# mgalardini/pyseer

Hardware: AMD Instinct MI355X
Metric: k-mer tests/sec at N=5000 samples (LMM), whole job (higher is better)
Workload: dtype int8 limbs x4 (exact int32 MFMA accumulation, fp64 recombination and statistics)

## Files before the change

### pyseer_amd/csrc/api.hip

```cpp
#include "common.h"
#include "route.h"
#include "host_pool.h"
#include <atomic>
#include <deque>
#include <mutex>
#include <condition_variable>
#include <functional>
#include <string>
#include <vector>
#include <thread>
#include <future>
#include <chrono>
#include <cmath>
#include <cstring>
#include <cstdlib>
#include <algorithm>

#include "lmm_params.h"
#include "vcf_kernels.h"
#include "vcf_reader.h"
#include "enet_params.h"
extern "C" {
hipError_t shk_sim_accumulate(hipStream_t st, const uint64_t *T, int64_t Vpad, int64_t V, int N, int NB64, double min_af, double max_af,
                              int af_on, uint64_t *keep, uint64_t *S, int NS, unsigned long long *Kacc);
hipError_t shk_sim_finish(hipStream_t st, const unsigned long long *Kacc, int NS, int N, double *K);
hipError_t shk_repack_bits(hipStream_t, const uint8_t *, int64_t, int64_t, int64_t, int, int, uint64_t *, uint8_t *);
hipError_t shk_lmm_linear(hipStream_t, int, const uint64_t *, int64_t, int, int, const double *, const double *,
                          const double *, const double *, const uint64_t *, const uint64_t *, int, const double *, LmmLinOut);
hipError_t shk_lmm_build_tab(hipStream_t, const double *, const double *, const double *, const double *, int, int, int, int, double *);
hipError_t shk_lmm_quadform(hipStream_t, int, const int8_t *, const uint64_t *, int64_t, int, int, int, double *, const int *, int, int64_t *);
hipError_t shk_lmm_refine(hipStream_t, int64_t, int64_t, int, int, int, int, const int8_t *, const uint64_t *, uint64_t *, double *, LmmLinOut,
                          const double *, LmmFinParams, double *, uint32_t *, LmmRefine);
hipError_t shk_af_compact(hipStream_t, int, int64_t, LmmLinOut, LmmFinParams, int *, int *, const uint64_t *, int64_t, uint64_t *,
                          int64_t, int, int, const double *, double *);
hipError_t shk_lmm_finalize(hipStream_t, int64_t, int64_t, int, LmmLinOut, const double *, LmmFinParams, double *, uint32_t *, LmmRefine);
hipError_t shk_spectral_bound(hipStream_t, const float *, int, int, double *, double *, int, double *, int *);
hipError_t shk_power_norm(hipStream_t, const float *, int, int, double *, double *, double *, int);
hipError_t shk_lmm_build_G(hipStream_t, const double *, const double *, int, int, int, int, int, int, double *, double *,
                           unsigned long long *, int8_t *, float *, double *, double *, double *, int);
hipError_t shk_dd_find(hipStream_t, const uint64_t *, int64_t, int64_t, int, uint64_t *, uint64_t, unsigned long long *, int *, int *, int *, int *);
hipError_t shk_af_rows(hipStream_t, int, const uint8_t *, int64_t, int64_t, int, double, double, int *, int *, int *);
hipError_t shk_pf_rows(hipStream_t, const uint8_t *, int64_t, int64_t, int, const uint64_t *, const uint64_t *, double, double, int, int, int,
                       double, int, int *, int *, int *, int *, int *, int *, double *, uint32_t *);
hipError_t shk_dd_gather(hipStream_t, const uint8_t *, int64_t, int64_t, const int *, const int *, uint8_t *);
hipError_t shk_dd_scatter(hipStream_t, int64_t, int64_t, int, const int *, const int *, const double *, const uint32_t *, double *, uint32_t *);
hipError_t shk_job_select(hipStream_t, const uint32_t *, const double *, int64_t, int, int, int, int *, long long *, long long *, int32_t *, uint32_t *, double *, int64_t, int32_t *);
int64_t sh_format_records(const char *, const int64_t *, const int32_t *, int, const int32_t *, int64_t, const double *const *, int, const double *, int64_t, int,
                          const uint8_t *, const int32_t *, const char *const *, int, const uint32_t *, const char **);
int64_t format_records_samples(const char *, const int64_t *, const int32_t *, int, const int32_t *, int64_t, const double *const *, int, const double *, int64_t, int,
                               const uint8_t *, const int32_t *, const char *const *, int, const uint32_t *, const char **, const uint8_t *, int64_t, const char *,
                               const int64_t *, const int32_t *);
hipError_t shk_job_patterns(hipStream_t, const uint64_t *, int64_t, int64_t, int, const uint32_t *, int *, long long *, uint32_t *, char *, char *);
#define JOB_ROWS_PER_BLOCK_HOST 1024
hipError_t shk_enet_store(hipStream_t, const uint8_t *, const uint8_t *, const uint8_t *, int64_t, int, int, uint64_t *);
hipError_t shk_enet_gather(hipStream_t, const uint64_t *, const int64_t *, int64_t, int, uint64_t *);
hipError_t shk_enet_ingest_count(hipStream_t, const uint64_t *, int64_t, int, int, int, int, int32_t *, int32_t *, int32_t *, int32_t *, int32_t *);
hipError_t shk_enet_ingest_scatter(hipStream_t, const uint64_t *, int64_t, int, int, const int32_t *, const int32_t *, uint64_t *);
hipError_t shk_enet_moments(hipStream_t, const uint64_t *, int64_t, int, int, const double *, double, double *);
hipError_t shk_enet_grad(hipStream_t, const uint64_t *, int64_t, int, const double *, int64_t, int, double *, int64_t);
size_t shk_enet_cd_lds_bytes(int, int);
hipError_t shk_enet_cd(hipStream_t, const struct EnetCdArgs *, int);
hipError_t shk_enet_predict(hipStream_t, const uint64_t *, const uint64_t *, const double *, const uint8_t *, int64_t, int, int, double *);
}
#include "glm_api.inc"

static thread_local std::string g_err;
static int fail(int code, const std::string &msg) { g_err = msg; return code; }
#define HIPCHK(x) do { hipError_t e_ = (x); if (e_ != hipSuccess) return fail(SH_EHIP, std::string(#x) + ": " + hipGetErrorString(e_)); } while (0)

#include <execinfo.h>
#include <signal.h>
static void sh_abort_backtrace(int sig)
{
    void *frames[64];
    const int n = backtrace(frames, 64);
    const char msg[] = "[seerhip] fatal signal; native backtrace of the signalled thread:\n";
    (void)!write(2, msg, sizeof(msg) - 1);
    backtrace_symbols_fd(frames, n, 2);
    signal(sig, SIG_DFL);
    raise(sig);
}
namespace { struct ShBacktraceInit { ShBacktraceInit() { if (sh_debug("backtrace")) { signal(SIGABRT, sh_abort_backtrace); signal(SIGSEGV, sh_abort_backtrace); signal(SIGBUS, sh_abort_backtrace); } } } sh_backtrace_init; }

template <typename T> static hipError_t dmalloc(T **p, size_t n)
{
    const hipError_t e = hipMalloc(reinterpret_cast<void **>(p), n * sizeof(T));
    if (e == hipSuccess && n && sh_debug("poison")) {
        const hipError_t m = hipMemset(*p, 0xFF, n * sizeof(T));
        return m != hipSuccess ? m : hipStreamSynchronize(nullptr);
    }
    return e;
}

struct sh_lanes;
struct EnetState;
struct PredictState;
struct GlmSetupArgs { std::vector<double> y, W; int q = 0, continuous = 0, force_firth = 0; double null_llf = 0, null_firth = 0, pret = 1, lrtt = 1;
                      std::string route; };
struct sh_ctx {
    int device = 0, N = 0;
    hipStream_t stream = nullptr;
    int *h_rb = nullptr;
    sh_lanes *lanes = nullptr; int n_lanes = 3; bool is_lane = false; GlmSetupArgs glm_args;
    double min_af = 0.0, max_af = 1.0; int af_on = 0;
    int NT = 0, Np = 0, NB64 = 0, NB64p = 0;
    bool lmm_ready = false;
    int k = 0, D = 0, L = 5, DP = 0;
    LmmFinParams fin{};
    double *d_vv = nullptr, *d_mdiag = nullptr, *d_yc = nullptr, *d_Qb = nullptr, *d_tab = nullptr;
    uint64_t *d_y1 = nullptr, *d_y0 = nullptr;
    int8_t *d_G = nullptr;
    double quant_scale = 0.0;
    size_t g_bytes = 0, tab_doubles = 0;
    int64_t macs_issued = 0;
    int E = 0;
    bool complement = false;
    double err_norm_ulp = 0.0, err_norm_est_ulp = 0.0, lmm_tol = 1e-8, trace_M = 0.0; int err_norm_squarings = 0;
    uint8_t *d_flip = nullptr; uint64_t *d_T3 = nullptr; double *d_q3 = nullptr; int *d_rlist = nullptr, *d_rcount = nullptr;
    unsigned long long *d_bmax = nullptr; int64_t cap_ref = 0;
    int qf_split = 1;
    int qf_variant = 4;
    GlmState glm;
    int64_t capV = 0;
    uint64_t *d_T = nullptr;
    int *d_t11 = nullptr, *d_t01 = nullptr, *d_m = nullptr;
    double *d_xky = nullptr, *d_dg = nullptr, *d_rss = nullptr, *d_s1 = nullptr, *d_q1 = nullptr, *d_q = nullptr;
    uint64_t *d_T2 = nullptr; double *d_q2 = nullptr; int *d_keep = nullptr, *d_nkeep = nullptr; int64_t cap_keep = 0;
    int af_compact = 1; int64_t last_kept = -1;
    int *h_nkeep = nullptr; hipEvent_t keep_ev = nullptr; bool keep_pending = false; int64_t keep_V = 0; double filtered_hint = 0.0;
    int timing = 0;
    int lin_tab = 1;
    std::vector<std::pair<hipEvent_t, hipEvent_t>> tev;
    int dedup = 0; int64_t dd_cap = 0, dd_capV = 0, dd_last_unique = -1;
    uint64_t *dd_h = nullptr; unsigned long long *dd_keys = nullptr; int *dd_idx = nullptr, *dd_rep = nullptr, *dd_slot = nullptr, *dd_n = nullptr;
    uint8_t *dd_bits = nullptr; double *dd_out = nullptr; uint32_t *dd_flags = nullptr; int64_t dd_cap_bits = 0, dd_cap_out = 0, dd_cap_flags = 0;
    int *af_rep = nullptr, *af_slot = nullptr, *af_cnt = nullptr, *h_af_cnt = nullptr; int64_t af_capV = 0;
    int *af_m = nullptr;
    uint8_t *af_bits = nullptr; double *af_out = nullptr; uint32_t *af_flags = nullptr; int64_t af_cap_bits = 0, af_cap_out = 0, af_cap_flags = 0;
    hipEvent_t af_ev = nullptr; bool af_pending = false; int64_t af_pending_V = 0; double af_hint = 0.0; int64_t af_last_rows = -1; unsigned af_tick = 0;
    unsigned long long *sim_K = nullptr; uint64_t *sim_S = nullptr, *sim_keep = nullptr; double *sim_out = nullptr; int64_t sim_capV = 0; int NS = 0;
    hipStream_t copy_stream = nullptr; hipEvent_t ev_h2d[2] = {nullptr, nullptr}, ev_done[2] = {nullptr, nullptr};
    uint8_t *hb_bits[2] = {nullptr, nullptr}; double *hb_out[2] = {nullptr, nullptr}; uint32_t *hb_flags[2] = {nullptr, nullptr};
    int64_t hb_cap_bits = 0, hb_cap_out = 0, hb_cap_flags = 0;
    uint8_t *hp_bits[2] = {nullptr, nullptr}; int64_t hp_cap = 0;
    struct HostPending { bool valid = false; int b = 0, q = 0; int64_t s = 0, n = 0; double *outs[5] = {nullptr, nullptr, nullptr, nullptr, nullptr};
                         double *betas = nullptr; uint32_t *flags = nullptr; } pend;
    uint64_t hb_seq = 0;
    const uint8_t *next_bits = nullptr; int64_t next_row_bytes = 0, next_V = 0;
    const uint8_t *pre_bits = nullptr; int64_t pre_row_bytes = 0, pre_n = 0; int pre_set = -1;
    int64_t cap_bits = 0, cap_out = 0, cap_flags = 0;
    uint8_t *d_bits = nullptr; double *d_out = nullptr; uint32_t *d_flags = nullptr;
    EnetState *enet = nullptr;
    PredictState *predict = nullptr;
};

__global__ void k_readback4(const int *__restrict__ a, const int *__restrict__ b, const int *__restrict__ c2, const int *__restrict__ d, int *__restrict__ out)
{
    if (threadIdx.x == 0) { out[0] = *a; if (b) out[1] = *b; if (c2) out[2] = *c2; if (d) out[3] = *d; __threadfence_system(); }
}
static hipError_t readback_launch(hipStream_t st, const int *a, const int *b, const int *c2, const int *d, int *host_mapped)
{
    hipLaunchKernelGGL(k_readback4, dim3(1), dim3(64), 0, st, a, b, c2, d, host_mapped);
    return hipGetLastError();
}
static int ensure_rb(sh_ctx *c);
static int readback_sync(sh_ctx *c, hipStream_t st, const int *a, const int *b, const int *c2, const int *d, int *dst);

static void lanes_destroy(sh_ctx *c);
static void enet_free(sh_ctx *c);
static void predict_free(sh_ctx *c);
static int lanes_wait(sh_ctx *c);
static void lanes_set_timing(sh_ctx *c, int on);
static int lanes_add_timing(sh_ctx *c, double *total_ms, int64_t *launches);
static void free_ws(sh_ctx *c)
{
    hipFree(c->d_T); hipFree(c->d_t11); hipFree(c->d_t01); hipFree(c->d_m); hipFree(c->d_xky); hipFree(c->d_dg);
    hipFree(c->d_rss); hipFree(c->d_s1); hipFree(c->d_q1); hipFree(c->d_q);
    c->d_T = nullptr; c->d_t11 = c->d_t01 = c->d_m = nullptr;
    c->d_xky = c->d_dg = c->d_rss = c->d_s1 = c->d_q1 = c->d_q = nullptr; c->capV = 0;
    hipFree(c->d_T2); hipFree(c->d_q2); hipFree(c->d_keep); hipFree(c->d_nkeep);
    c->d_T2 = nullptr; c->d_q2 = nullptr; c->d_keep = c->d_nkeep = nullptr; c->cap_keep = 0;
    hipFree(c->d_flip); hipFree(c->d_T3); hipFree(c->d_q3); hipFree(c->d_rlist);
    c->d_flip = nullptr; c->d_T3 = nullptr; c->d_q3 = nullptr; c->d_rlist = nullptr; c->cap_ref = 0;
}

static int ensure_rb(sh_ctx *c)
{
    if (!c->h_rb) HIPCHK(hipHostMalloc((void **)&c->h_rb, 16 * sizeof(int), hipHostMallocMapped));
    return SH_OK;
}
static int readback_sync(sh_ctx *c, hipStream_t st, const int *a, const int *b, const int *c2, const int *d, int *dst)
{
    int rc = ensure_rb(c); if (rc) return rc;
    HIPCHK(readback_launch(st, a, b, c2, d, c->h_rb));
    HIPCHK(hipStreamSynchronize(st));
    dst[0] = c->h_rb[0]; if (b) dst[1] = c->h_rb[1]; if (c2) dst[2] = c->h_rb[2]; if (d) dst[3] = c->h_rb[3];
    return SH_OK;
}

static int ensure_ws(sh_ctx *c, int64_t Vpad)
{
    if (Vpad <= c->capV) return SH_OK;
    free_ws(c);
    HIPCHK(dmalloc(&c->d_T, (size_t)Vpad * c->NB64p));
    HIPCHK(dmalloc(&c->d_t11, Vpad)); HIPCHK(dmalloc(&c->d_t01, Vpad)); HIPCHK(dmalloc(&c->d_m, Vpad));
    HIPCHK(dmalloc(&c->d_xky, Vpad)); HIPCHK(dmalloc(&c->d_dg, Vpad)); HIPCHK(dmalloc(&c->d_rss, Vpad));
    HIPCHK(dmalloc(&c->d_s1, Vpad)); HIPCHK(dmalloc(&c->d_q1, Vpad)); HIPCHK(dmalloc(&c->d_q, Vpad * 8));
    c->capV = Vpad;
    return SH_OK;
}

static int ensure_staging(sh_ctx *c, int64_t bits_bytes, int64_t out_doubles, int64_t V)
{
    if (bits_bytes > c->cap_bits) { hipFree(c->d_bits); c->d_bits = nullptr; HIPCHK(hipMalloc((void **)&c->d_bits, bits_bytes)); c->cap_bits = bits_bytes; }
    if (out_doubles > c->cap_out) { hipFree(c->d_out); c->d_out = nullptr; HIPCHK(dmalloc(&c->d_out, out_doubles)); c->cap_out = out_doubles; }
    if (V > c->cap_flags) { hipFree(c->d_flags); c->d_flags = nullptr; HIPCHK(dmalloc(&c->d_flags, V)); c->cap_flags = V; }
    return SH_OK;
}

static void parallel_copy(uint8_t *dst, const uint8_t *src, size_t n)
{
    shost::CpuScope cs(shost::ST_STAGE_COPY);
    const size_t piece = (size_t)4 << 20, np = (n + piece - 1) / piece;
    if (np <= 1) { std::memcpy(dst, src, n); return; }
    const std::function<void(int64_t)> cp = [&](int64_t i) { const size_t lo = (size_t)i * piece, hi = std::min(n, lo + piece); std::memcpy(dst + lo, src + lo, hi - lo); };
    shost::pool().run((int64_t)np, 1, cp, shost::ST_STAGE_COPY, shost::per_stream_cpus(2));
}

__global__ void k_betas_rows(const double *__restrict__ src, double *__restrict__ dst, int64_t n, int q)
{
    const int64_t i = (int64_t)blockIdx.x * blockDim.x + threadIdx.x;
    if (i >= n * q) return;
    const int64_t v = i / q; const int j = (int)(i - v * q);
    dst[i] = src[(size_t)j * n + v];
}

static void forget_announced(sh_ctx *c) { c->next_bits = nullptr; c->pre_bits = nullptr; c->pre_set = -1; }

static int drain_pending(sh_ctx *c)
{
    if (!c->pend.valid) return SH_OK;
    HIPCHK(hipSetDevice(c->device));
    const sh_ctx::HostPending p = c->pend;
    c->pend.valid = false;
    const int b = p.b;
    const int64_t s = p.s, n = p.n;
    HIPCHK(hipStreamWaitEvent(c->copy_stream, c->ev_done[b], 0));
    for (int a = 0; a < 5; ++a)
        HIPCHK(hipMemcpyAsync(p.outs[a] + s, c->hb_out[b] + (size_t)a * n, sizeof(double) * n, hipMemcpyDeviceToHost, c->copy_stream));
    if (p.q > 0)
        HIPCHK(hipMemcpyAsync(p.betas + (size_t)s * p.q, c->hb_out[b] + (size_t)(5 + p.q) * n, sizeof(double) * p.q * n, hipMemcpyDeviceToHost, c->copy_stream));
    HIPCHK(hipMemcpyAsync(p.flags + s, c->hb_flags[b], sizeof(uint32_t) * n, hipMemcpyDeviceToHost, c->copy_stream));
    HIPCHK(hipStreamSynchronize(c->copy_stream));
    return SH_OK;
}

template <typename F>
static int host_batch(sh_ctx *c, const uint8_t *bits, int64_t row_bytes, int64_t V, int nrow, double *const *outs, double *betas,
                      int q, uint32_t *flags, bool async, F inner_dev)
{
    const double t_entry = std::chrono::duration<double, std::milli>(std::chrono::steady_clock::now().time_since_epoch()).count();
    HIPCHK(hipSetDevice(c->device));
    const int64_t CH = 1 << 18;
    const int64_t cap = std::min(CH, V);
    if (!c->copy_stream) {
        HIPCHK(hipStreamCreateWithFlags(&c->copy_stream, hipStreamNonBlocking));
        for (int b = 0; b < 2; ++b) { HIPCHK(hipEventCreateWithFlags(&c->ev_h2d[b], hipEventDisableTiming)); HIPCHK(hipEventCreateWithFlags(&c->ev_done[b], hipEventDisableTiming)); }
    }
    if (cap * row_bytes > c->hb_cap_bits || cap * (nrow + q) > c->hb_cap_out || cap > c->hb_cap_flags) {
        int rc = drain_pending(c); if (rc) return rc;
        const int64_t nb = std::max(cap * row_bytes, c->hb_cap_bits), no = std::max(cap * (nrow + q), c->hb_cap_out), nf = std::max(cap, c->hb_cap_flags);
        for (int b = 0; b < 2; ++b) {
            hipFree(c->hb_bits[b]); hipFree(c->hb_out[b]); hipFree(c->hb_flags[b]);
            c->hb_bits[b] = nullptr; c->hb_out[b] = nullptr; c->hb_flags[b] = nullptr;
            HIPCHK(hipMalloc((void **)&c->hb_bits[b], nb)); HIPCHK(dmalloc(&c->hb_out[b], no)); HIPCHK(dmalloc(&c->hb_flags[b], nf));
        }
        c->hb_cap_bits = nb; c->hb_cap_out = no; c->hb_cap_flags = nf;
        c->pre_bits = nullptr; c->pre_set = -1;
    }
    if (cap * row_bytes > c->hp_cap) {
        int rc = drain_pending(c); if (rc) return rc;
        for (int b = 0; b < 2; ++b) { if (c->hp_bits[b]) hipHostFree(c->hp_bits[b]); c->hp_bits[b] = nullptr; HIPCHK(hipHostMalloc((void **)&c->hp_bits[b], cap * row_bytes, hipHostMallocDefault)); }
        c->hp_cap = cap * row_bytes;
        c->pre_bits = nullptr; c->pre_set = -1;
    }
    std::vector<int64_t> cut{0};
    for (int64_t step = 1 << 17; cut.back() < V; step = CH) cut.push_back(std::min(V, cut.back() + step));
    const int64_t nchunk = (int64_t)cut.size() - 1;
    const bool dbg = sh_debug("host");
    auto now = [] { return std::chrono::duration<double, std::milli>(std::chrono::steady_clock::now().time_since_epoch()).count(); };
    const uint8_t *const nb_bits = c->next_bits; const int64_t nb_rb = c->next_row_bytes, nb_V = c->next_V;
    c->next_bits = nullptr;
    const double t00 = now();
    auto upload = [&](int64_t i, int b) -> int {
        const int64_t s = cut[i], n = cut[i + 1] - s;
        parallel_copy(c->hp_bits[b], bits + s * row_bytes, (size_t)(n * row_bytes));
        HIPCHK(hipMemcpyAsync(c->hb_bits[b], c->hp_bits[b], n * row_bytes, hipMemcpyHostToDevice, c->copy_stream));
        HIPCHK(hipEventRecord(c->ev_h2d[b], c->copy_stream));
        return SH_OK;
    };
    for (int64_t i = 0; i < nchunk; ++i) {
        const int b = (int)(c->hb_seq++ & 1);
        const int64_t s = cut[i], n = cut[i + 1] - s;
        const double t0 = now();
        if (i == 0) {
            if (c->pend.valid && c->pend.b == b) { int rc = drain_pending(c); if (rc) return rc; }
            bool have = c->pre_bits == bits && c->pre_row_bytes == row_bytes && c->pre_n == n && c->pre_set == b;
            if (have) {
                const size_t nbytes = (size_t)(n * row_bytes), probe = std::min<size_t>(nbytes, 4096);
                have = std::memcmp(c->hp_bits[b], bits, probe) == 0 && std::memcmp(c->hp_bits[b] + nbytes - probe, bits + nbytes - probe, probe) == 0;
            }
            c->pre_bits = nullptr; c->pre_set = -1;
            if (!have) { int rc = upload(0, b); if (rc) return rc; }
        }
        const double t1 = now();
        HIPCHK(hipStreamWaitEvent(c->stream, c->ev_h2d[b], 0));
        std::string side_err;
        std::future<int> side = std::async(std::launch::async, [&]() -> int {
            if (hipSetDevice(c->device) != hipSuccess) { side_err = "hipSetDevice failed on the copy thread"; return SH_EHIP; }
            int rc = drain_pending(c);
            if (!rc && i + 1 < nchunk) rc = upload(i + 1, b ^ 1);
            else if (!rc && nb_bits && nb_bits != bits) {
                const int64_t n0 = std::min<int64_t>((int64_t)1 << 17, nb_V);
                if (n0 * nb_rb <= c->hp_cap && n0 * nb_rb <= c->hb_cap_bits) {
                    parallel_copy(c->hp_bits[b ^ 1], nb_bits, (size_t)(n0 * nb_rb));
                    if (hipMemcpyAsync(c->hb_bits[b ^ 1], c->hp_bits[b ^ 1], n0 * nb_rb, hipMemcpyHostToDevice, c->copy_stream) != hipSuccess ||
                        hipEventRecord(c->ev_h2d[b ^ 1], c->copy_stream) != hipSuccess) { g_err = "prefetch upload failed"; rc = SH_EHIP; }
                    else { c->pre_bits = nb_bits; c->pre_row_bytes = nb_rb; c->pre_n = n0; c->pre_set = b ^ 1; }
                }
            }
            if (rc) side_err = g_err;
            return rc;
        });
        int rc = inner_dev(c->hb_bits[b], n, c->hb_out[b], c->hb_flags[b]);
        if (!rc && q > 0) {
            hipLaunchKernelGGL(k_betas_rows, dim3((unsigned)((n * q + 255) / 256)), dim3(256), 0, c->stream, c->hb_out[b] + (size_t)5 * n,
                               c->hb_out[b] + (size_t)(5 + q) * n, n, q);
            if (hipGetLastError() != hipSuccess) rc = fail(SH_EHIP, "k_betas_rows launch failed");
        }
        if (!rc && hipEventRecord(c->ev_done[b], c->stream) != hipSuccess) rc = fail(SH_EHIP, "hipEventRecord failed");
        const double t2 = now();
        const int rc_side = side.get();
        if (rc) { c->pend.valid = false; return rc; }
        if (rc_side) { c->pend.valid = false; return fail(rc_side, side_err); }
        c->pend.valid = true; c->pend.b = b; c->pend.q = q; c->pend.s = s; c->pend.n = n; c->pend.betas = betas; c->pend.flags = flags;
        for (int a = 0; a < 5; ++a) c->pend.outs[a] = outs[a];
        if (dbg) fprintf(stderr, "[host_batch] chunk %lld n=%lld: first upload %.2f ms, kernels queued (fixed effects: run) %.2f ms, wait for the copy thread %.2f ms, t=%.2f\n", (long long)i, (long long)n, t1 - t0, t2 - t1, now() - t2, now() - t00);
    }
    const int rc_end = async ? SH_OK : drain_pending(c);
    if (dbg) fprintf(stderr, "[host_batch] call of %lld variants: %.2f ms in all (%.2f ms before the first chunk)\n", (long long)V, now() - t_entry, t00 - t_entry);
    return rc_end;
}

static int lmm_batch_dev_inner(sh_ctx *c, const void *d_bits, int64_t row_bytes, int64_t V, void *d_out, void *d_flags);
static int glm_batch_dev_inner(sh_ctx *c, const void *d_bits, int64_t row_bytes, int64_t V, void *d_out, void *d_flags);

template <typename F>
static int dedup_wrap(sh_ctx *c, const void *d_bits, int64_t row_bytes, int64_t V, void *d_out, void *d_flags, int nrow, F inner)
{
    HIPCHK(hipSetDevice(c->device));
    hipStream_t st = c->stream;
    const int64_t Vpad = (V + 511) / 512 * 512;
    int rc = ensure_ws(c, Vpad); if (rc) return rc;
    if (V > c->dd_capV) {
        hipFree(c->dd_h); hipFree(c->dd_keys); hipFree(c->dd_idx); hipFree(c->dd_rep); hipFree(c->dd_slot); hipFree(c->dd_n);
        c->dd_h = nullptr; c->dd_keys = nullptr; c->dd_idx = c->dd_rep = c->dd_slot = c->dd_n = nullptr;
        uint64_t cap = 1024; while (cap < (uint64_t)V * 2) cap <<= 1;
        HIPCHK(dmalloc(&c->dd_h, V)); HIPCHK(dmalloc(&c->dd_keys, cap)); HIPCHK(dmalloc(&c->dd_idx, cap));
        HIPCHK(dmalloc(&c->dd_rep, V)); HIPCHK(dmalloc(&c->dd_slot, V)); HIPCHK(dmalloc(&c->dd_n, 1));
        c->dd_cap = (int64_t)cap; c->dd_capV = V;
    }
    if (V * row_bytes > c->dd_cap_bits) { hipFree(c->dd_bits); c->dd_bits = nullptr; HIPCHK(hipMalloc((void **)&c->dd_bits, V * row_bytes)); c->dd_cap_bits = V * row_bytes; }
    if (V * nrow > c->dd_cap_out) { hipFree(c->dd_out); c->dd_out = nullptr; HIPCHK(dmalloc(&c->dd_out, V * nrow)); c->dd_cap_out = V * nrow; }
    if (V > c->dd_cap_flags) { hipFree(c->dd_flags); c->dd_flags = nullptr; HIPCHK(dmalloc(&c->dd_flags, V)); c->dd_cap_flags = V; }
    HIPCHK(shk_repack_bits(st, (const uint8_t *)d_bits, row_bytes, V, Vpad, c->N, c->NB64p, c->d_T, nullptr));
    HIPCHK(shk_dd_find(st, c->d_T, Vpad, V, c->NB64, c->dd_h, (uint64_t)c->dd_cap, c->dd_keys, c->dd_idx, c->dd_rep, c->dd_slot, c->dd_n));
    int nu = 0;
    { const int rcb = readback_sync(c, st, c->dd_n, nullptr, nullptr, nullptr, &nu); if (rcb) return rcb; }
    c->dd_last_unique = nu;
    HIPCHK(shk_dd_gather(st, (const uint8_t *)d_bits, row_bytes, V, c->dd_rep, c->dd_slot, c->dd_bits));
    rc = inner(c->dd_bits, (int64_t)nu, c->dd_out, c->dd_flags); if (rc) return rc;
    HIPCHK(shk_dd_scatter(st, V, nu, nrow, c->dd_rep, c->dd_slot, c->dd_out, c->dd_flags, (double *)d_out, (uint32_t *)d_flags));
    return SH_OK;
}

struct PrefilterRows { const uint64_t *y1 = nullptr, *y0 = nullptr; int n1 = 0, n0 = 0; double pret = 1.0; };
template <typename F>
static int af_wrap(sh_ctx *c, const void *d_bits, int64_t row_bytes, int64_t V, void *d_out, void *d_flags, int nrow, F inner,
                   PrefilterRows pf = PrefilterRows())
{
    c->af_last_rows = -1;
    const bool use_pf = pf.y1 != nullptr && pf.pret < 1.0;
    if (!((c->af_on || use_pf) && c->af_compact) || (V < 1024 && c->af_compact != 2)) return inner(d_bits, V, d_out, d_flags);
    HIPCHK(hipSetDevice(c->device));
    hipStream_t st = c->stream;
    if (V > c->af_capV) {
        hipFree(c->af_rep); hipFree(c->af_slot); hipFree(c->af_m); c->af_rep = c->af_slot = c->af_m = nullptr;
        HIPCHK(dmalloc(&c->af_rep, V)); HIPCHK(dmalloc(&c->af_slot, V)); HIPCHK(dmalloc(&c->af_m, 3 * V)); c->af_capV = V;
    }
    if (!c->af_cnt) {
        HIPCHK(dmalloc(&c->af_cnt, 2)); HIPCHK(hipHostMalloc((void **)&c->h_af_cnt, 2 * sizeof(int)));
        HIPCHK(hipEventCreateWithFlags(&c->af_ev, hipEventDisableTiming));
    }
    if (c->af_pending && hipEventQuery(c->af_ev) == hipSuccess) {
        c->af_hint = 1.0 - (double)c->h_af_cnt[0] / (double)c->af_pending_V; c->af_pending = false;
    }
    bool compact = false; int nk = 0, R = 0;
    if (!c->af_pending && (c->af_hint >= 0.10 || c->af_compact == 2 || (c->af_tick++ & 3) == 0)) {
        HIPCHK(hipMemsetD32Async((hipDeviceptr_t)c->af_cnt, 0, 1, st));
        HIPCHK(hipMemsetD32Async((hipDeviceptr_t)(c->af_cnt + 1), 2147483647, 1, st));
        if (use_pf)
            HIPCHK(shk_pf_rows(st, (const uint8_t *)d_bits, row_bytes, V, c->N, pf.y1, pf.y0, c->min_af, c->max_af, c->af_on, pf.n1, pf.n0, pf.pret, nrow,
                               c->af_m, c->af_m + c->af_capV, c->af_m + 2 * c->af_capV, c->af_rep, c->af_slot, c->af_cnt, (double *)d_out,
                               (uint32_t *)d_flags));
        else
            HIPCHK(shk_af_rows(st, 0, (const uint8_t *)d_bits, row_bytes, V, c->N, c->min_af, c->max_af, c->af_rep, c->af_slot, c->af_cnt));
        HIPCHK(readback_launch(st, c->af_cnt, c->af_cnt + 1, nullptr, nullptr, c->h_af_cnt));
        if (c->af_hint >= 0.10 || c->af_compact == 2) {
            HIPCHK(hipStreamSynchronize(st));
            nk = c->h_af_cnt[0]; R = c->h_af_cnt[1];
            c->af_hint = 1.0 - (double)nk / (double)V;
            compact = (int64_t)nk * 100 <= V * 90 || (c->af_compact == 2 && (int64_t)nk * 100 <= V * 97);
        } else {
            HIPCHK(hipEventRecord(c->af_ev, st)); c->af_pending = true; c->af_pending_V = V;
        }
    }
    if (!compact) return inner(d_bits, V, d_out, d_flags);
    const int64_t nu = (int64_t)nk + (R != 2147483647 ? 1 : 0);
    if (nu == 0) { c->af_last_rows = 0; return SH_OK; }
    if (nu * row_bytes > c->af_cap_bits) { hipFree(c->af_bits); c->af_bits = nullptr; HIPCHK(hipMalloc((void **)&c->af_bits, nu * row_bytes)); c->af_cap_bits = nu * row_bytes; }
    if (nu * nrow > c->af_cap_out) { hipFree(c->af_out); c->af_out = nullptr; HIPCHK(dmalloc(&c->af_out, nu * nrow)); c->af_cap_out = nu * nrow; }
    if (nu > c->af_cap_flags) { hipFree(c->af_flags); c->af_flags = nullptr; HIPCHK(dmalloc(&c->af_flags, nu)); c->af_cap_flags = nu; }
    HIPCHK(shk_af_rows(st, 1, nullptr, 0, V, 0, 0, 0, c->af_rep, c->af_slot, c->af_cnt));
    HIPCHK(shk_dd_gather(st, (const uint8_t *)d_bits, row_bytes, V, c->af_rep, c->af_slot, c->af_bits));
    c->af_last_rows = nu;
    int rc = inner(c->af_bits, nu, c->af_out, c->af_flags); if (rc) return rc;
    HIPCHK(shk_dd_scatter(st, V, nu, nrow, c->af_rep, c->af_slot, c->af_out, c->af_flags, (double *)d_out, (uint32_t *)d_flags));
    return SH_OK;
}

extern "C" {

int sh_abi_version(void) { return SH_ABI_VERSION; }
const char *sh_last_error(void) { return g_err.c_str(); }

int sh_device_count(void)
{
    int n = 0;
    if (hipGetDeviceCount(&n) != hipSuccess) return 0;
    return n;
}

__global__ void k_noop() {}

static std::atomic<int> g_wait_mode{0};
static std::atomic<uint64_t> g_wait_applied{0};
static void apply_wait_mode(int device)
{
    if (g_wait_mode.load() != 1 || device < 0 || device >= 64) return;
    const uint64_t bit = 1ull << device;
    if (g_wait_applied.fetch_or(bit) & bit) return;
    if (hipSetDeviceFlags(hipDeviceScheduleBlockingSync) != hipSuccess) (void)hipGetLastError();
}
void sh_set_wait_mode(int sleeping) { g_wait_mode.store(sleeping ? 1 : 0); }

int sh_warmup(int device)
{
    int n = 0;
    if (hipGetDeviceCount(&n) != hipSuccess || device < 0 || device >= n) return fail(SH_ENODEV, "no such HIP device");
    HIPCHK(hipSetDevice(device));
    apply_wait_mode(device);
    hipLaunchKernelGGL(k_noop, dim3(1), dim3(64), 0, 0);
    HIPCHK(hipGetLastError());
    HIPCHK(hipDeviceSynchronize());
    return SH_OK;
}

sh_ctx *sh_create(int device, int n_samples)
{
    int n = 0;
    if (const std::string bad = sh_route_unknown(); !bad.empty()) { g_err = "SEERHIP_ROUTE: unknown item '" + bad + "' (keys: csrc/route.h)"; return nullptr; }
    if (hipGetDeviceCount(&n) != hipSuccess || n <= 0) { g_err = "no HIP device: libseerhip has no CPU fallback"; return nullptr; }
    if (device < 0 || device >= n) { g_err = "bad device index"; return nullptr; }
    if (n_samples < 2) { g_err = "n_samples must be >= 2"; return nullptr; }
    hipDeviceProp_t prop;
    if (hipGetDeviceProperties(&prop, device) != hipSuccess) { g_err = "hipGetDeviceProperties failed"; return nullptr; }
    if (std::string(prop.gcnArchName).find("gfx950") == std::string::npos) {
        g_err = std::string("device is ") + prop.gcnArchName + ", libseerhip is built for gfx950 only"; return nullptr;
    }
    if (hipSetDevice(device) != hipSuccess) { g_err = "hipSetDevice failed"; return nullptr; }
    apply_wait_mode(device);
    sh_ctx *c = new sh_ctx();
    c->device = device; c->N = n_samples;
    if (const char *qv = sh_route("qf")) c->qf_variant = std::atoi(qv);
    if (const char *lv = sh_route("lanes")) c->n_lanes = std::max(1, std::min(8, std::atoi(lv)));
    if (const char *ac = sh_route("afcompact")) c->af_compact = std::atoi(ac);
    c->NT = (n_samples + 255) / 256; c->Np = c->NT * 256;
    c->NB64 = (n_samples + 63) / 64; c->NB64p = c->NT * 4;
    return c;
}

void sh_destroy(sh_ctx *c)
{
    if (!c) return;
    hipSetDevice(c->device);
    lanes_destroy(c);
    enet_free(c);
    predict_free(c);
    free_ws(c);
    if (c->h_nkeep) hipHostFree(c->h_nkeep);
    if (c->h_rb) hipHostFree(c->h_rb);
    if (c->h_af_cnt) hipHostFree(c->h_af_cnt);
    if (c->af_ev) hipEventDestroy(c->af_ev);
    hipFree(c->af_rep); hipFree(c->af_slot); hipFree(c->af_m); hipFree(c->af_cnt); hipFree(c->af_bits); hipFree(c->af_out); hipFree(c->af_flags);
    if (c->keep_ev) hipEventDestroy(c->keep_ev);
    hipFree(c->d_vv); hipFree(c->d_mdiag); hipFree(c->d_yc); hipFree(c->d_Qb); hipFree(c->d_y1); hipFree(c->d_y0); hipFree(c->d_tab);
    hipFree(c->d_G); hipFree(c->d_bits); hipFree(c->d_out); hipFree(c->d_flags); hipFree(c->d_rcount); hipFree(c->d_bmax);
    for (int b = 0; b < 2; ++b) { hipFree(c->hb_bits[b]); hipFree(c->hb_out[b]); hipFree(c->hb_flags[b]); if (c->ev_h2d[b]) hipEventDestroy(c->ev_h2d[b]); if (c->ev_done[b]) hipEventDestroy(c->ev_done[b]); }
    if (c->copy_stream) hipStreamDestroy(c->copy_stream);
    for (int b = 0; b < 2; ++b) if (c->hp_bits[b]) hipHostFree(c->hp_bits[b]);
    for (auto &p : c->tev) { hipEventDestroy(p.first); hipEventDestroy(p.second); }
    hipFree(c->dd_h); hipFree(c->dd_keys); hipFree(c->dd_idx); hipFree(c->dd_rep); hipFree(c->dd_slot); hipFree(c->dd_n); hipFree(c->dd_bits); hipFree(c->dd_out); hipFree(c->dd_flags);
    hipFree(c->sim_K); hipFree(c->sim_S); hipFree(c->sim_keep); hipFree(c->sim_out);
    glm_free(&c->glm);
    delete c;
}

int sh_set_stream(sh_ctx *c, void *s) { if (!c) return fail(SH_EINVAL, "null ctx"); forget_announced(c); c->stream = (hipStream_t)s; return SH_OK; }

int sh_synchronize(sh_ctx *c)
{
    if (!c) return fail(SH_EINVAL, "null ctx");
    HIPCHK(hipSetDevice(c->device));
    HIPCHK(hipStreamSynchronize(c->stream));
    return SH_OK;
}

int sh_set_timing(sh_ctx *c, int on)
{
    if (!c) return fail(SH_EINVAL, "null ctx");
    for (auto &p : c->tev) { hipEventDestroy(p.first); hipEventDestroy(p.second); }
    c->tev.clear(); c->timing = on;
    if (c->lanes) { const int rc = lanes_wait(c); if (rc) return rc; lanes_set_timing(c, on); }
    return SH_OK;
}

int sh_get_timing(sh_ctx *c, double *total_ms, int64_t *launches)
{
    if (!c) return fail(SH_EINVAL, "null ctx");
    HIPCHK(hipSetDevice(c->device));
    double tot = 0;
    for (auto &p : c->tev) { HIPCHK(hipEventSynchronize(p.second)); float ms = 0; HIPCHK(hipEventElapsedTime(&ms, p.first, p.second)); tot += ms; }
    int64_t nl = (int64_t)c->tev.size();
    if (c->lanes) { const int rc = lanes_wait(c); if (rc) return rc; const int r2 = lanes_add_timing(c, &tot, &nl); if (r2) return r2; }
    if (total_ms) *total_ms = tot;
    if (launches) *launches = nl;
    return SH_OK;
}

int sh_set_dedup(sh_ctx *c, int on) { if (!c) return fail(SH_EINVAL, "null ctx"); c->dedup = on; return SH_OK; }

int sh_dedup_info(sh_ctx *c, int64_t *unique_last_batch)
{
    if (!c) return fail(SH_EINVAL, "null ctx");
    if (unique_last_batch) *unique_last_batch = c->dd_last_unique;
    return SH_OK;
}

int sh_set_af_filter(sh_ctx *c, double min_af, double max_af)
{
    if (!c) return fail(SH_EINVAL, "null ctx");
    c->min_af = min_af; c->max_af = max_af; c->af_on = !(min_af <= 0.0 && max_af >= 1.0);
    return SH_OK;
}

static double spectral_bound_value(double f2, const int *e, int nsq)
{
    if (!(f2 > 0.0)) return 0.0;
    double lg = std::log2(f2) / std::ldexp(1.0, nsq + 1);
    for (int k = 0; k < nsq; ++k) lg -= (double)e[k] / std::ldexp(1.0, k);
    return std::exp2(lg);
}

int sh_lmm_setup(sh_ctx *c, const double *U, const double *S, int k, const double *y, const double *C, int D,
                 double h2, int continuous, double pret, double lrtt, int n_limbs)
{
    if (!c || !U || !S || !y || !C) return fail(SH_EINVAL, "null argument");
    if (k < 1 || D < 1) return fail(SH_ESHAPE, "k and D must be >= 1");
    if (h2 < 0.0 || h2 >= 1.0 || std::isnan(h2)) return fail(SH_EH2, "h2 outside [0,1): reference returns no 'beta' (KeyError)");
    { const int rc0 = drain_pending(c); if (rc0) return rc0; }
    forget_announced(c);
    if (n_limbs == 0) {
        const char *fe = sh_route("lmm_limbs");
        if (fe && std::atoi(fe) > 0) n_limbs = std::atoi(fe);
        else {
            const int rc4 = sh_lmm_setup(c, U, S, k, y, C, D, h2, continuous, pret, lrtt, 4);
            if (rc4 != SH_OK) return rc4;
            const double typ = c->trace_M > 0 ? c->fin.err_norm * (0.5 * c->N) / (0.25 * c->trace_M) : 0.0;
            if (c->E > 0 && typ <= 0.25 * c->lmm_tol) return SH_OK;
            n_limbs = 5;
        }
    }
    if (n_limbs < 3 || n_limbs > 7) return fail(SH_EINVAL, "n_limbs must be 3..7");
    if (c->N > 262143) return fail(SH_EINVAL, "more than 262143 samples: the int32 partial sums of k_lmm_quadform_i8 could overflow");
    HIPCHK(hipSetDevice(c->device));
    const int N = c->N, Np = c->Np;
    const int kp = (k + 3) & ~3;
    c->lmm_ready = false; c->macs_issued = 0;

    std::vector<double> Qb((size_t)N * D, 0.0);
    int r = 0;
    for (int d = 0; d < D; ++d) {
        const int src = (d == 0) ? D - 1 : d - 1;
        std::vector<double> col(N);
        double n0 = 0;
        for (int i = 0; i < N; ++i) { col[i] = C[(size_t)i * D + src]; n0 += col[i] * col[i]; }
        for (int pass = 0; pass < 2; ++pass)
            for (int e = 0; e < r; ++e) {
                double dot = 0; for (int i = 0; i < N; ++i) dot += Qb[(size_t)i * D + e] * col[i];
                for (int i = 0; i < N; ++i) col[i] -= dot * Qb[(size_t)i * D + e];
            }
        double n1 = 0; for (int i = 0; i < N; ++i) n1 += col[i] * col[i];
        if (!(n1 > 1e-24 * n0) || n0 == 0) continue;
        const double inv = 1.0 / std::sqrt(n1);
        for (int i = 0; i < N; ++i) Qb[(size_t)i * D + r] = col[i] * inv;
        ++r;
    }
    if (r < 1) return fail(SH_EINVAL, "covariate matrix has rank 0");
    bool ones_in_span;
    {
        std::vector<double> one(N, 1.0);
        for (int e = 0; e < r; ++e) { double dot = 0; for (int i = 0; i < N; ++i) dot += Qb[(size_t)i * D + e] * one[i]; for (int i = 0; i < N; ++i) one[i] -= dot * Qb[(size_t)i * D + e]; }
        double res = 0; for (int i = 0; i < N; ++i) res += one[i] * one[i];
        ones_in_span = res <= 1e-20 * (double)N;
    }
    bool intercept_only = (r == 1);
    if (intercept_only) { const double q0 = Qb[0]; for (int i = 0; i < N; ++i) if (std::fabs(Qb[(size_t)i * D] - q0) > 1e-12 * std::fabs(q0)) intercept_only = false; }
    int DP = 0;
    if (!intercept_only) { DP = 4; while (DP < r) DP *= 2; if (DP > 32) return fail(SH_EINVAL, "more than 32 independent covariates are not supported"); }

    std::vector<double> yt(N);
    {
        std::vector<double> cy(r, 0.0);
        for (int e = 0; e < r; ++e) { double s = 0; for (int i = 0; i < N; ++i) s += Qb[(size_t)i * D + e] * y[i]; cy[e] = s; }
        double mean = 0;
        for (int i = 0; i < N; ++i) { double s = y[i]; for (int e = 0; e < r; ++e) s -= Qb[(size_t)i * D + e] * cy[e]; yt[i] = s; mean += s; }
        mean /= N; double q = 0; for (int i = 0; i < N; ++i) q += (yt[i] - mean) * (yt[i] - mean);
        if (std::sqrt(q / N) <= 1e-10) std::fill(yt.begin(), yt.end(), 0.0);
    }
    std::vector<double> Sd(k), uy(k, 0.0), sgn(kp, 0.0);
    for (int rr = 0; rr < k; ++rr) Sd[rr] = h2 * S[rr] + (1.0 - h2);
    std::vector<double> W((size_t)Np * kp, 0.0);
    {
        std::vector<double> QtU((size_t)r * k, 0.0);
        for (int i = 0; i < N; ++i) {
            const double *u = U + (size_t)i * k;
            for (int e = 0; e < r; ++e) { const double q = Qb[(size_t)i * D + e]; double *o = &QtU[(size_t)e * k]; for (int rr = 0; rr < k; ++rr) o[rr] += q * u[rr]; }
        }
        for (int i = 0; i < N; ++i) {
            const double *u = U + (size_t)i * k; double *w = &W[(size_t)i * kp];
            for (int rr = 0; rr < k; ++rr) w[rr] = u[rr];
            for (int e = 0; e < r; ++e) { const double q = Qb[(size_t)i * D + e]; const double *o = &QtU[(size_t)e * k]; for (int rr = 0; rr < k; ++rr) w[rr] -= q * o[rr]; }
            const double yi = yt[i];
            if (yi != 0.0) for (int rr = 0; rr < k; ++rr) uy[rr] += w[rr] * yi;
        }
    }
    double yKy = 0;
    std::vector<double> uys(k);
    for (int rr = 0; rr < k; ++rr) { yKy += uy[rr] * uy[rr] / Sd[rr]; uys[rr] = uy[rr] / Sd[rr]; sgn[rr] = Sd[rr] < 0 ? -1.0 : 1.0; }
    std::vector<double> vv(N);
    for (int i = 0; i < N; ++i) {
        double *w = &W[(size_t)i * kp]; double s = 0;
        for (int rr = 0; rr < k; ++rr) s += w[rr] * uys[rr];
        vv[i] = s;
        for (int rr = 0; rr < k; ++rr) w[rr] *= 1.0 / std::sqrt(std::fabs(Sd[rr]));
    }
    std::vector<uint64_t> y1(c->NB64p, 0), y0(c->NB64p, 0);
    int n1 = 0, n0 = 0; double ymean = 0;
    for (int i = 0; i < N; ++i) { if (y[i] == 1.0) { y1[i >> 6] |= 1ull << (i & 63); ++n1; } else if (y[i] == 0.0) { y0[i >> 6] |= 1ull << (i & 63); ++n0; } ymean += y[i]; }
    ymean /= N;
    std::vector<double> yc(N); double ycs = 0, ycq = 0;
    for (int i = 0; i < N; ++i) { yc[i] = y[i] - ymean; ycs += yc[i]; ycq += yc[i] * yc[i]; }
    std::vector<double> Qbp;
    if (DP) { Qbp.assign((size_t)N * DP, 0.0); for (int i = 0; i < N; ++i) for (int e = 0; e < r; ++e) Qbp[(size_t)i * DP + e] = Qb[(size_t)i * D + e]; }

    hipFree(c->d_vv); hipFree(c->d_mdiag); hipFree(c->d_yc); hipFree(c->d_Qb); hipFree(c->d_y1); hipFree(c->d_y0); hipFree(c->d_G); hipFree(c->d_tab);
    c->d_vv = c->d_mdiag = c->d_yc = c->d_Qb = c->d_tab = nullptr; c->d_y1 = c->d_y0 = nullptr; c->d_G = nullptr;
    const int NT = c->NT, L = n_limbs;
    const int NR = 2 * NT;
    int E = std::min(2, 7 - L);
    const int Lt = L + E;
    const size_t gbytes = (size_t)Lt * NR * (NR + 1) * 8192;
    double *d_W = nullptr, *d_sgn = nullptr, *d_M = nullptr; unsigned long long *d_amax = nullptr;
    float *d_Ef = nullptr; double *d_px = nullptr, *d_py = nullptr, *d_nrm = nullptr;
    const int NPOW = 48;
    HIPCHK(dmalloc(&c->d_vv, N)); HIPCHK(dmalloc(&c->d_mdiag, N)); HIPCHK(dmalloc(&c->d_yc, N));
    HIPCHK(dmalloc(&c->d_y1, c->NB64p)); HIPCHK(dmalloc(&c->d_y0, c->NB64p));
    if (DP) HIPCHK(dmalloc(&c->d_Qb, (size_t)N * DP));
    HIPCHK(hipMalloc((void **)&c->d_G, gbytes + (256u << 10)));
    HIPCHK(dmalloc(&d_W, (size_t)Np * kp)); HIPCHK(dmalloc(&d_sgn, kp)); HIPCHK(dmalloc(&d_M, (size_t)Np * Np)); HIPCHK(dmalloc(&d_amax, 1));
    hipStream_t st = c->stream;
    HIPCHK(hipMemcpyAsync(d_W, W.data(), sizeof(double) * (size_t)Np * kp, hipMemcpyHostToDevice, st));
    HIPCHK(hipMemcpyAsync(d_sgn, sgn.data(), sizeof(double) * kp, hipMemcpyHostToDevice, st));
    HIPCHK(hipMemcpyAsync(c->d_vv, vv.data(), sizeof(double) * N, hipMemcpyHostToDevice, st));
    HIPCHK(hipMemcpyAsync(c->d_yc, yc.data(), sizeof(double) * N, hipMemcpyHostToDevice, st));
    HIPCHK(hipMemcpyAsync(c->d_y1, y1.data(), sizeof(uint64_t) * c->NB64p, hipMemcpyHostToDevice, st));
    HIPCHK(hipMemcpyAsync(c->d_y0, y0.data(), sizeof(uint64_t) * c->NB64p, hipMemcpyHostToDevice, st));
    if (DP) HIPCHK(hipMemcpyAsync(c->d_Qb, Qbp.data(), sizeof(double) * (size_t)N * DP, hipMemcpyHostToDevice, st));
    HIPCHK(hipMemsetAsync(d_M, 0, sizeof(double) * (size_t)Np * Np, st));
    HIPCHK(dmalloc(&d_Ef, (size_t)Np * Np)); HIPCHK(dmalloc(&d_px, Np)); HIPCHK(dmalloc(&d_py, Np)); HIPCHK(dmalloc(&d_nrm, NPOW));
    HIPCHK(shk_lmm_build_G(st, d_W, d_sgn, N, Np, kp, NR, Lt, E, d_M, c->d_mdiag, d_amax, c->d_G, d_Ef, d_px, d_py, d_nrm, NPOW));
    const int nsq = Np <= 16384 ? 5 : Np <= 32768 ? 4 : 3;
    double *d_X = nullptr, *d_work = nullptr; int *d_exps = nullptr;
    HIPCHK(dmalloc(&d_X, (size_t)Np * Np)); HIPCHK(dmalloc(&d_work, 2)); HIPCHK(dmalloc(&d_exps, 8));
    HIPCHK(shk_spectral_bound(st, d_Ef, N, Np, d_X, d_M, nsq, d_work, d_exps));
    double cert_f2 = 0.0; int cert_e[8] = {0, 0, 0, 0, 0, 0, 0, 0};
    HIPCHK(hipMemcpyAsync(&cert_f2, d_work + 1, sizeof(double), hipMemcpyDeviceToHost, st));
    HIPCHK(hipMemcpyAsync(cert_e, d_exps, sizeof(cert_e), hipMemcpyDeviceToHost, st));
    c->tab_doubles = (size_t)c->NB64 * 256 * (2 + 2 + 8); c->g_bytes = gbytes;
    HIPCHK(dmalloc(&c->d_tab, c->tab_doubles));
    HIPCHK(shk_lmm_build_tab(st, c->d_vv, c->d_mdiag, c->d_yc, c->d_Qb, DP, continuous, N, c->NB64, c->d_tab));
    unsigned long long amax_bits = 0;
    HIPCHK(hipMemcpyAsync(&amax_bits, d_amax, sizeof(amax_bits), hipMemcpyDeviceToHost, st));
    std::vector<double> nrm(NPOW, 0.0), mdiag_h(N, 0.0);
    HIPCHK(hipMemcpyAsync(nrm.data(), d_nrm, sizeof(double) * NPOW, hipMemcpyDeviceToHost, st));
    HIPCHK(hipMemcpyAsync(mdiag_h.data(), c->d_mdiag, sizeof(double) * N, hipMemcpyDeviceToHost, st));
    HIPCHK(hipStreamSynchronize(st));
    hipFree(d_W); hipFree(d_sgn); hipFree(d_M); hipFree(d_amax); hipFree(d_Ef); hipFree(d_px); hipFree(d_py); hipFree(d_nrm);
    hipFree(d_X); hipFree(d_work); hipFree(d_exps);
    double amax; std::memcpy(&amax, &amax_bits, sizeof(double));
    const double p256 = std::pow(256.0, L);
    c->quant_scale = amax > 0 ? 0.49 * p256 / amax : 0.0;
    c->err_norm_est_ulp = nrm[NPOW - 1];
    c->err_norm_squarings = nsq;
    c->err_norm_ulp = spectral_bound_value(cert_f2, cert_e, nsq) * (1.0 + 1e-6);
    if (!(c->err_norm_ulp >= c->err_norm_est_ulp * (1.0 - 1e-9)) || !std::isfinite(c->err_norm_ulp))
        return fail(SH_EHIP, "spectral-norm certificate below the power-iteration estimate");
    double sumv = 0; for (int i = 0; i < N; ++i) sumv += vv[i];
    c->trace_M = 0; for (int i = 0; i < N; ++i) c->trace_M += mdiag_h[i];

    c->k = k; c->D = D; c->L = L; c->DP = DP; c->E = E;
    c->complement = ones_in_span && !(sh_route("complement") && std::atoi(sh_route("complement")) == 0);
    if (const char *tv = sh_route("lmm_tol")) c->lmm_tol = std::atof(tv);
    LmmFinParams &P = c->fin;
    P.N = N; P.D = D; P.continuous = continuous; P.n1 = n1; P.n0 = n0; P.yc_sum = ycs; P.yc_sq = ycq;
    P.yKy = yKy; P.inv_scale = amax > 0 ? 1.0 / c->quant_scale : 0.0; P.pret = pret; P.lrtt = lrtt;
    P.sumv = sumv; P.err_norm = c->err_norm_ulp * P.inv_scale; P.tol = E > 0 ? c->lmm_tol : 0.0;
    P.inv_scale_low = P.inv_scale / std::pow(256.0, E);
    c->lmm_ready = true;
    return SH_OK;
}

int sh_lmm_info(sh_ctx *c, int *n_limbs, int64_t *macs, double *qscale)
{
    if (!c || !c->lmm_ready) return fail(SH_EINVAL, "sh_lmm_setup has not run");
    if (n_limbs) *n_limbs = c->L;
    if (macs) *macs = c->macs_issued > 0 ? c->macs_issued : (int64_t)c->L * (2 * c->NT) * (2 * c->NT + 1) * 128 * 64;
    if (qscale) *qscale = c->quant_scale;
    return SH_OK;
}

int sh_lmm_share(sh_ctx *dst, sh_ctx *src)
{
    if (!dst || !src || !src->lmm_ready) return fail(SH_EINVAL, "sh_lmm_share: the source context has no LMM set-up");
    if (dst == src) return SH_OK;
    if (dst->N != src->N) return fail(SH_ESHAPE, "sh_lmm_share: contexts of different sample counts");
    HIPCHK(hipSetDevice(src->device));
    HIPCHK(hipStreamSynchronize(src->stream));
    HIPCHK(hipSetDevice(dst->device));
    sh_ctx *c = dst;
    const int N = c->N;
    hipFree(c->d_vv); hipFree(c->d_mdiag); hipFree(c->d_yc); hipFree(c->d_Qb); hipFree(c->d_y1); hipFree(c->d_y0); hipFree(c->d_G); hipFree(c->d_tab);
    c->d_vv = c->d_mdiag = c->d_yc = c->d_Qb = c->d_tab = nullptr; c->d_y1 = c->d_y0 = nullptr; c->d_G = nullptr; c->lmm_ready = false;
    HIPCHK(dmalloc(&c->d_vv, N)); HIPCHK(dmalloc(&c->d_mdiag, N)); HIPCHK(dmalloc(&c->d_yc, N));
    HIPCHK(dmalloc(&c->d_y1, c->NB64p)); HIPCHK(dmalloc(&c->d_y0, c->NB64p));
    if (src->DP) HIPCHK(dmalloc(&c->d_Qb, (size_t)N * src->DP));
    HIPCHK(hipMalloc((void **)&c->d_G, src->g_bytes + (256u << 10))); HIPCHK(dmalloc(&c->d_tab, src->tab_doubles));
    auto cp = [&](void *d, const void *s_, size_t n) { return hipMemcpyPeerAsync(d, dst->device, s_, src->device, n, dst->stream); };
    HIPCHK(cp(c->d_vv, src->d_vv, sizeof(double) * N)); HIPCHK(cp(c->d_mdiag, src->d_mdiag, sizeof(double) * N));
    HIPCHK(cp(c->d_yc, src->d_yc, sizeof(double) * N));
    HIPCHK(cp(c->d_y1, src->d_y1, sizeof(uint64_t) * c->NB64p)); HIPCHK(cp(c->d_y0, src->d_y0, sizeof(uint64_t) * c->NB64p));
    if (src->DP) HIPCHK(cp(c->d_Qb, src->d_Qb, sizeof(double) * (size_t)N * src->DP));
    HIPCHK(cp(c->d_G, src->d_G, src->g_bytes)); HIPCHK(cp(c->d_tab, src->d_tab, sizeof(double) * src->tab_doubles));
    HIPCHK(hipStreamSynchronize(dst->stream));
    c->k = src->k; c->D = src->D; c->L = src->L; c->DP = src->DP; c->E = src->E; c->complement = src->complement;
    c->quant_scale = src->quant_scale; c->err_norm_ulp = src->err_norm_ulp; c->err_norm_est_ulp = src->err_norm_est_ulp; c->err_norm_squarings = src->err_norm_squarings; c->trace_M = src->trace_M; c->lmm_tol = src->lmm_tol;
    c->g_bytes = src->g_bytes; c->tab_doubles = src->tab_doubles; c->fin = src->fin;
    c->lmm_ready = true;
    return SH_OK;
}

int sh_set_lmm_tol(sh_ctx *c, double tol)
{
    if (!c) return fail(SH_EINVAL, "null ctx");
    if (!(tol >= 0.0)) return fail(SH_EINVAL, "tol must be >= 0 (0 = never refine)");
    c->lmm_tol = tol;
    if (c->lmm_ready) c->fin.tol = c->E > 0 ? tol : 0.0;
    return SH_OK;
}

int sh_lmm_bound(sh_ctx *c, double *err_norm_ulp, double *ulp, double *tol, int *extra_limbs, double *bound_typical,
                 double *bound_max_last, int64_t *refined_last)
{
    if (!c || !c->lmm_ready) return fail(SH_EINVAL, "sh_lmm_setup has not run");
    HIPCHK(hipSetDevice(c->device));
    if (err_norm_ulp) *err_norm_ulp = c->err_norm_ulp;
    if (ulp) *ulp = c->fin.inv_scale;
    if (tol) *tol = c->fin.tol;
    if (extra_limbs) *extra_limbs = c->E;
    if (bound_typical) *bound_typical = c->trace_M > 0 ? c->fin.err_norm * (0.5 * c->N) / (0.25 * c->trace_M) : 0.0;
    unsigned long long bm = 0; int nr = 0;
    if (c->d_bmax) {
        HIPCHK(hipMemcpyAsync(&bm, c->d_bmax, sizeof(bm), hipMemcpyDeviceToHost, c->stream));
        HIPCHK(hipMemcpyAsync(&nr, c->d_rcount, sizeof(nr), hipMemcpyDeviceToHost, c->stream));
        HIPCHK(hipStreamSynchronize(c->stream));
    }
    double b; std::memcpy(&b, &bm, sizeof(double));
    if (bound_max_last) *bound_max_last = b;
    if (refined_last) *refined_last = nr;
    return SH_OK;
}

int sh_lmm_bound_estimate(sh_ctx *c, double *power_iteration_ulp, int *squarings)
{
    if (!c || !c->lmm_ready) return fail(SH_EINVAL, "sh_lmm_setup has not run");
    if (power_iteration_ulp) *power_iteration_ulp = c->err_norm_est_ulp;
    if (squarings) *squarings = c->err_norm_squarings;
    return SH_OK;
}

int sh_spectral_bound_f32(sh_ctx *c, const float *A, int n, int squarings, double *upper, double *power_iteration)
{
    if (!c || !A || n < 1 || squarings < 1 || squarings > 6) return fail(SH_EINVAL, "bad argument");
    HIPCHK(hipSetDevice(c->device));
    const int Np = (n + 127) / 128 * 128, NPOW = 48;
    float *d_A = nullptr; double *d_X = nullptr, *d_Y = nullptr, *d_work = nullptr, *d_px = nullptr, *d_py = nullptr, *d_nrm = nullptr; int *d_exps = nullptr;
    HIPCHK(dmalloc(&d_A, (size_t)Np * Np)); HIPCHK(dmalloc(&d_X, (size_t)Np * Np)); HIPCHK(dmalloc(&d_Y, (size_t)Np * Np));
    HIPCHK(dmalloc(&d_work, 2)); HIPCHK(dmalloc(&d_exps, 8)); HIPCHK(dmalloc(&d_px, Np)); HIPCHK(dmalloc(&d_py, Np)); HIPCHK(dmalloc(&d_nrm, NPOW));
    hipStream_t st = c->stream;
    HIPCHK(hipMemsetAsync(d_A, 0, sizeof(float) * (size_t)Np * Np, st));
    HIPCHK(hipMemcpy2DAsync(d_A, sizeof(float) * Np, A, sizeof(float) * n, sizeof(float) * n, n, hipMemcpyHostToDevice, st));
    HIPCHK(shk_spectral_bound(st, d_A, n, Np, d_X, d_Y, squarings, d_work, d_exps));
    HIPCHK(shk_power_norm(st, d_A, n, Np, d_px, d_py, d_nrm, NPOW));
    double f2 = 0.0, nrm[48]; int e[8] = {0, 0, 0, 0, 0, 0, 0, 0};
    HIPCHK(hipMemcpyAsync(&f2, d_work + 1, sizeof(double), hipMemcpyDeviceToHost, st));
    HIPCHK(hipMemcpyAsync(e, d_exps, sizeof(e), hipMemcpyDeviceToHost, st));
    HIPCHK(hipMemcpyAsync(nrm, d_nrm, sizeof(nrm), hipMemcpyDeviceToHost, st));
    HIPCHK(hipStreamSynchronize(st));
    hipFree(d_A); hipFree(d_X); hipFree(d_Y); hipFree(d_work); hipFree(d_exps); hipFree(d_px); hipFree(d_py); hipFree(d_nrm);
    if (upper) *upper = spectral_bound_value(f2, e, squarings) * (1.0 + 1e-6);
    if (power_iteration) *power_iteration = nrm[NPOW - 1];
    return SH_OK;
}

int sh_lmm_batch_dev(sh_ctx *c, const void *d_bits, int64_t row_bytes, int64_t V, void *d_out, void *d_flags)
{
    if (!c || !c->lmm_ready) return fail(SH_EINVAL, "sh_lmm_setup has not run");
    if (V <= 0) return SH_OK;
    if (row_bytes * 8 < c->N) return fail(SH_ESHAPE, "row_bytes*8 < n_samples: shape mismatch between snps and Y");
    if (c->dedup)
        return dedup_wrap(c, d_bits, row_bytes, V, d_out, d_flags, 5,
                          [&](const void *b, int64_t n, void *o, void *f) { return lmm_batch_dev_inner(c, b, row_bytes, n, o, f); });
    return lmm_batch_dev_inner(c, d_bits, row_bytes, V, d_out, d_flags);
}

static int lmm_batch_dev_inner(sh_ctx *c, const void *d_bits, int64_t row_bytes, int64_t V, void *d_out, void *d_flags)
{
    if (V <= 0) return SH_OK;
    if (row_bytes * 8 < c->N) return fail(SH_ESHAPE, "row_bytes*8 < n_samples: shape mismatch between snps and Y");
    HIPCHK(hipSetDevice(c->device));
    const int64_t Vpad = (V + 511) / 512 * 512;
    int rc = ensure_ws(c, Vpad); if (rc) return rc;
    hipStream_t st = c->stream;
    if (Vpad > c->cap_ref || (c->E > 0 && !c->d_T3)) {
        hipFree(c->d_flip); hipFree(c->d_T3); hipFree(c->d_q3); hipFree(c->d_rlist);
        c->d_flip = nullptr; c->d_T3 = nullptr; c->d_q3 = nullptr; c->d_rlist = nullptr;
        HIPCHK(dmalloc(&c->d_flip, Vpad)); HIPCHK(dmalloc(&c->d_rlist, Vpad));
        if (c->E > 0) { HIPCHK(dmalloc(&c->d_T3, (size_t)Vpad * c->NB64p)); HIPCHK(dmalloc(&c->d_q3, Vpad * 2)); }
        c->cap_ref = Vpad;
    }
    if (!c->d_rcount) { HIPCHK(dmalloc(&c->d_rcount, 1)); HIPCHK(dmalloc(&c->d_bmax, 1)); }
    LmmLinOut lo{c->d_t11, c->d_t01, c->d_m, c->d_xky, c->d_dg, c->d_rss, c->d_s1, c->d_q1, c->complement ? c->d_flip : nullptr};
    HIPCHK(shk_repack_bits(st, (const uint8_t *)d_bits, row_bytes, V, Vpad, c->N, c->NB64p, c->d_T, c->complement ? c->d_flip : nullptr));
    HIPCHK(shk_lmm_linear(st, c->DP, c->d_T, Vpad, c->N, c->NB64, c->d_vv, c->d_mdiag, c->d_yc, c->d_Qb, c->d_y1, c->d_y0,
                          c->fin.continuous, c->lin_tab ? c->d_tab : nullptr, lo));
    hipEvent_t e0 = nullptr, e1 = nullptr;
    if (c->timing) { HIPCHK(hipEventCreate(&e0)); HIPCHK(hipEventCreate(&e1)); HIPCHK(hipEventRecord(e0, st)); }
    const int lsplit = c->qf_split ? c->L : 1;
    const int8_t *Gmain = c->d_G + (size_t)c->E * (2 * c->NT) * (2 * c->NT + 1) * 8192;
    int64_t nk = V;
    bool compact = false;
    LmmFinParams KP = c->fin; KP.min_af = c->min_af; KP.max_af = c->max_af; KP.af_on = c->af_on;
    if ((c->af_on || KP.pret < 1.0) && c->af_compact) {
        if (Vpad > c->cap_keep) {
            hipFree(c->d_T2); hipFree(c->d_q2); hipFree(c->d_keep); hipFree(c->d_nkeep);
            c->d_T2 = nullptr; c->d_q2 = nullptr; c->d_keep = c->d_nkeep = nullptr;
            HIPCHK(dmalloc(&c->d_T2, (size_t)Vpad * c->NB64p)); HIPCHK(dmalloc(&c->d_q2, Vpad * 8)); HIPCHK(dmalloc(&c->d_keep, Vpad));
            HIPCHK(dmalloc(&c->d_nkeep, 1)); c->cap_keep = Vpad;
        }
        if (!c->h_nkeep) { HIPCHK(hipHostMalloc((void **)&c->h_nkeep, sizeof(int))); HIPCHK(hipEventCreateWithFlags(&c->keep_ev, hipEventDisableTiming)); }
        if (c->keep_pending && hipEventQuery(c->keep_ev) == hipSuccess) {
            c->filtered_hint = 1.0 - (double)*c->h_nkeep / (double)c->keep_V; c->keep_pending = false;
        }
        if (!c->keep_pending) {
            HIPCHK(hipMemsetAsync(c->d_nkeep, 0, sizeof(int), st));
            HIPCHK(shk_af_compact(st, 0, V, lo, KP, c->d_keep, c->d_nkeep, nullptr, 0, nullptr, 0, 0, 0, nullptr, nullptr));
            HIPCHK(readback_launch(st, c->d_nkeep, nullptr, nullptr, nullptr, c->h_nkeep));
            if (c->filtered_hint >= 0.03 || c->af_compact == 2) {
                HIPCHK(hipStreamSynchronize(st));
                nk = *c->h_nkeep; c->filtered_hint = 1.0 - (double)nk / (double)V;
                compact = nk * 100 <= V * 97;
            } else {
                HIPCHK(hipEventRecord(c->keep_ev, st)); c->keep_pending = true; c->keep_V = V;
            }
        }
    }
    c->last_kept = compact ? nk : -1;
    if (compact && nk > 0) {
        const int64_t Vpad2 = (nk + 511) / 512 * 512;
        HIPCHK(shk_af_compact(st, 1, V, lo, KP, c->d_keep, nullptr, c->d_T, Vpad, c->d_T2, Vpad2, c->NB64p, (int)nk, nullptr, nullptr));
        HIPCHK(shk_lmm_quadform(st, c->qf_variant, Gmain, c->d_T2, Vpad2, 2 * c->NT, c->L, lsplit, c->d_q2, nullptr, c->N - (2 * c->NT - 1) * 128, &c->macs_issued));
        HIPCHK(shk_af_compact(st, 2, V, lo, KP, c->d_keep, nullptr, nullptr, Vpad, nullptr, Vpad2, lsplit, (int)nk, c->d_q2, c->d_q));
    } else if (!compact) {
        HIPCHK(shk_lmm_quadform(st, c->qf_variant, Gmain, c->d_T, Vpad, 2 * c->NT, c->L, lsplit, c->d_q, nullptr, c->N - (2 * c->NT - 1) * 128, &c->macs_issued));
    }
    if (c->timing) { HIPCHK(hipEventRecord(e1, st)); c->tev.emplace_back(e0, e1); }
    LmmFinParams P = c->fin; P.min_af = c->min_af; P.max_af = c->max_af; P.af_on = c->af_on;
    const bool refine = c->E > 0 && P.tol > 0.0;
    LmmRefine R{refine ? c->d_rlist : nullptr, c->d_rcount, c->d_bmax};
    HIPCHK(hipMemsetAsync(c->d_rcount, 0, sizeof(int), st));
    HIPCHK(hipMemsetAsync(c->d_bmax, 0, sizeof(unsigned long long), st));
    HIPCHK(shk_lmm_finalize(st, V, Vpad, lsplit, lo, c->d_q, P, (double *)d_out, (uint32_t *)d_flags, R));
    if (refine)
        HIPCHK(shk_lmm_refine(st, V, Vpad, lsplit, c->E, 2 * c->NT, c->NB64p, c->d_G, c->d_T, c->d_T3, c->d_q3, lo, c->d_q, P, (double *)d_out,
                              (uint32_t *)d_flags, R));
    return SH_OK;
}

static int lmm_batch_host(sh_ctx *c, const uint8_t *bits, int64_t row_bytes, int64_t V, double *prep, double *pvalue,
                          double *beta, double *bse, double *frac_h2, uint32_t *flags, bool async)
{
    if (!c || !c->lmm_ready) return fail(SH_EINVAL, "sh_lmm_setup has not run");
    if (!bits || !prep || !pvalue || !beta || !bse || !frac_h2 || !flags) return fail(SH_EINVAL, "null argument");
    if (V <= 0) { HIPCHK(hipSetDevice(c->device)); return drain_pending(c); }
    double *outs[5] = {prep, pvalue, beta, bse, frac_h2};
    return host_batch(c, bits, row_bytes, V, 5, outs, nullptr, 0, flags, async,
                      [&](const void *b, int64_t n, void *o, void *f) { return sh_lmm_batch_dev(c, b, row_bytes, n, o, f); });
}

int sh_lmm_batch(sh_ctx *c, const uint8_t *bits, int64_t row_bytes, int64_t V, double *prep, double *pvalue,
                 double *beta, double *bse, double *frac_h2, uint32_t *flags)
{
    return lmm_batch_host(c, bits, row_bytes, V, prep, pvalue, beta, bse, frac_h2, flags, false);
}

int sh_lmm_batch_async(sh_ctx *c, const uint8_t *bits, int64_t row_bytes, int64_t V, double *prep, double *pvalue,
                       double *beta, double *bse, double *frac_h2, uint32_t *flags)
{
    return lmm_batch_host(c, bits, row_bytes, V, prep, pvalue, beta, bse, frac_h2, flags, true);
}

int sh_prefetch_rows(sh_ctx *c, const uint8_t *bits, int64_t row_bytes, int64_t V)
{
    if (!c) return fail(SH_EINVAL, "null ctx");
    if (!bits || V <= 0 || row_bytes <= 0) { c->next_bits = nullptr; return SH_OK; }
    c->next_bits = bits; c->next_row_bytes = row_bytes; c->next_V = V;
    return SH_OK;
}

int sh_wait(sh_ctx *c)
{
    if (!c) return fail(SH_EINVAL, "null ctx");
    HIPCHK(hipSetDevice(c->device));
    const int rc = drain_pending(c);
    const int rl = lanes_wait(c);
    return rc ? rc : rl;
}

int sh_sim_begin(sh_ctx *c)
{
    if (!c) return fail(SH_EINVAL, "null ctx");
    HIPCHK(hipSetDevice(c->device));
    c->NS = (c->N + 127) / 128 * 128;
    if (!c->sim_K) HIPCHK(dmalloc(&c->sim_K, (size_t)c->NS * c->NS));
    HIPCHK(hipMemsetAsync(c->sim_K, 0, sizeof(unsigned long long) * (size_t)c->NS * c->NS, c->stream));
    return SH_OK;
}

int sh_sim_accumulate_dev(sh_ctx *c, const void *d_bits, int64_t row_bytes, int64_t V)
{
    if (!c || !c->sim_K) return fail(SH_EINVAL, "sh_sim_begin has not run");
    if (!d_bits) return fail(SH_EINVAL, "null argument");
    if (row_bytes * 8 < c->N) return fail(SH_ESHAPE, "row_bytes too small for n_samples");
    if (V <= 0) return SH_OK;
    if (V > ((int64_t)1 << 31)) return fail(SH_EINVAL, "at most 2^31 variants per call (32-bit partial counts)");
    HIPCHK(hipSetDevice(c->device));
    const int64_t Vpad = (V + 511) / 512 * 512;
    int rc = ensure_ws(c, Vpad); if (rc) return rc;
    if (Vpad > c->sim_capV) {
        hipFree(c->sim_S); hipFree(c->sim_keep); c->sim_S = nullptr; c->sim_keep = nullptr;
        const int64_t VWp = (Vpad / 64 + 15) / 16 * 16;
        HIPCHK(dmalloc(&c->sim_S, (size_t)VWp * c->NS)); HIPCHK(dmalloc(&c->sim_keep, (size_t)VWp));
        c->sim_capV = Vpad;
    }
    HIPCHK(shk_repack_bits(c->stream, (const uint8_t *)d_bits, row_bytes, V, Vpad, c->N, c->NB64p, c->d_T, nullptr));
    HIPCHK(shk_sim_accumulate(c->stream, c->d_T, Vpad, V, c->N, c->NB64, c->min_af, c->max_af, c->af_on, c->sim_keep, c->sim_S, c->NS, c->sim_K));
    return SH_OK;
}

int sh_sim_accumulate(sh_ctx *c, const uint8_t *bits, int64_t row_bytes, int64_t V)
{
    if (!c || !c->sim_K) return fail(SH_EINVAL, "sh_sim_begin has not run");
    if (!bits) return fail(SH_EINVAL, "null argument");
    HIPCHK(hipSetDevice(c->device));
    const int64_t CH = 1 << 20;
    for (int64_t s = 0; s < V; s += CH) {
        const int64_t n = std::min(CH, V - s);
        int rc = ensure_staging(c, n * row_bytes, 0, 0); if (rc) return rc;
        HIPCHK(hipMemcpyAsync(c->d_bits, bits + s * row_bytes, n * row_bytes, hipMemcpyHostToDevice, c->stream));
        rc = sh_sim_accumulate_dev(c, c->d_bits, row_bytes, n); if (rc) return rc;
        HIPCHK(hipStreamSynchronize(c->stream));
    }
    return SH_OK;
}

int sh_sim_finish(sh_ctx *c, double *K)
{
    if (!c || !c->sim_K) return fail(SH_EINVAL, "sh_sim_begin has not run");
    if (!K) return fail(SH_EINVAL, "null argument");
    HIPCHK(hipSetDevice(c->device));
    const size_t n = (size_t)c->N * c->N;
    if (!c->sim_out) HIPCHK(dmalloc(&c->sim_out, n));
    HIPCHK(shk_sim_finish(c->stream, c->sim_K, c->NS, c->N, c->sim_out));
    HIPCHK(hipMemcpyAsync(K, c->sim_out, sizeof(double) * n, hipMemcpyDeviceToHost, c->stream));
    HIPCHK(hipStreamSynchronize(c->stream));
    return SH_OK;
}

#include "glm_api_impl.inc"
#include "lanes_api.inc"
#include "job_api.inc"
#include "job_run.inc"
#include "vcf_api.inc"
#include "enet_api.inc"

}
```

### pyseer_amd/csrc/lmm_kernels.hip

```cpp
#include <utility>
#include "common.h"
#include "lmm_params.h"

typedef int v4i __attribute__((ext_vector_type(4)));
typedef int v16i __attribute__((ext_vector_type(16)));
typedef double v4d __attribute__((ext_vector_type(4)));


__global__ __launch_bounds__(256) void k_row_flip(const uint8_t *__restrict__ bits, int64_t row_bytes, int64_t V, int N, uint8_t *__restrict__ flip)
{
    const int64_t v = (int64_t)blockIdx.x * 4 + (threadIdx.x >> 6);
    const int lane = threadIdx.x & 63;
    if (v >= V) return;
    const uint8_t *p = bits + v * row_bytes;
    const int nb = N >> 3;
    int m = 0;
    for (int b = lane; b < nb; b += 64) m += __popc((unsigned)p[b]);
    if (lane == 0 && (N & 7)) m += __popc((unsigned)p[nb] & ((1u << (N & 7)) - 1u));
    for (int o = 32; o > 0; o >>= 1) m += __shfl_xor(m, o, 64);
    if (lane == 0) flip[v] = (2 * m > N) ? 1 : 0;
}

__global__ __launch_bounds__(256) void k_repack_bits_gather(const uint8_t *__restrict__ bits, int64_t row_bytes, int64_t V,
                                                            int64_t Vpad, int N, uint64_t *__restrict__ T, const uint8_t *__restrict__ flip)
{
    const int64_t v = (int64_t)blockIdx.x * 256 + threadIdx.x;
    const int sb = blockIdx.y;
    uint64_t w = 0;
    if (v < V) {
        const int64_t off = (int64_t)sb * 8;
        const uint8_t *p = bits + v * row_bytes + off;
        int64_t nbytes = row_bytes - off; if (nbytes > 8) nbytes = 8;
        if (nbytes == 8 && ((reinterpret_cast<uintptr_t>(p) & 7) == 0)) w = *reinterpret_cast<const uint64_t *>(p);
        else for (int b = 0; b < nbytes; b++) w |= (uint64_t)p[b] << (8 * b);
        if (flip && flip[v]) w = ~w;
        const int valid = N - sb * 64;
        if (valid <= 0) w = 0; else if (valid < 64) w &= ((1ull << valid) - 1ull);
    }
    T[(int64_t)sb * Vpad + v] = w;
}

__global__ __launch_bounds__(256) void k_repack_bits(const uint8_t *__restrict__ bits, int64_t row_bytes, int64_t V,
                                                     int64_t Vpad, int N, int NB64p, uint64_t *__restrict__ T, uint8_t *__restrict__ flip)
{
    extern __shared__ __attribute__((aligned(16))) uint8_t rp_rows[];
    __shared__ int rp_cnt[4][64];
    const int64_t v0 = (int64_t)blockIdx.x * 64;
    const int tid = threadIdx.x, lane = tid & 63, wave = tid >> 6;
    const int64_t nrows = min((int64_t)64, V - v0);
    const int64_t span = nrows > 0 ? nrows * row_bytes : 0;
    const uint8_t *src = bits + v0 * row_bytes;
    if ((reinterpret_cast<uintptr_t>(src) & 15) == 0) {
        const int64_t n16 = span >> 4;
        for (int64_t i = tid; i < n16; i += 256) reinterpret_cast<uint4 *>(rp_rows)[i] = reinterpret_cast<const uint4 *>(src)[i];
        for (int64_t i = (n16 << 4) + tid; i < span; i += 256) rp_rows[i] = src[i];
    } else {
        for (int64_t i = tid; i < span; i += 256) rp_rows[i] = src[i];
    }
    __syncthreads();
    auto word = [&](int sb) -> uint64_t {
        uint64_t w = 0;
        const int64_t off = (int64_t)sb * 8;
        if (lane < nrows && off < row_bytes) {
            const uint8_t *p = rp_rows + lane * row_bytes + off;
            int64_t nbytes = row_bytes - off; if (nbytes > 8) nbytes = 8;
            if (nbytes == 8 && ((row_bytes & 7) == 0)) w = *reinterpret_cast<const uint64_t *>(p);
            else for (int b = 0; b < nbytes; b++) w |= (uint64_t)p[b] << (8 * b);
            const int valid = N - sb * 64;
            if (valid <= 0) w = 0; else if (valid < 64) w &= ((1ull << valid) - 1ull);
        }
        return w;
    };
    bool fl = false;
    if (flip) {
        int m = 0;
        for (int sb = wave; sb < NB64p; sb += 4) m += __popcll(word(sb));
        rp_cnt[wave][lane] = m;
        __syncthreads();
        m = rp_cnt[0][lane] + rp_cnt[1][lane] + rp_cnt[2][lane] + rp_cnt[3][lane];
        fl = lane < nrows && 2 * m > N;
        if (wave == 0 && lane < nrows) flip[v0 + lane] = fl ? 1 : 0;
    }
    for (int sb = wave; sb < NB64p; sb += 4) {
        uint64_t w = word(sb);
        if (fl) {
            const int valid = N - sb * 64;
            w = ~w;
            if (valid <= 0) w = 0; else if (valid < 64) w &= ((1ull << valid) - 1ull);
        }
        T[(int64_t)sb * Vpad + v0 + lane] = w;
    }
}


template <int DP>
__global__ __launch_bounds__(256) void k_lmm_linear(const uint64_t *__restrict__ T, int64_t Vpad, int N, int NB64,
                                                    const double *__restrict__ vv, const double *__restrict__ mdiag,
                                                    const double *__restrict__ yc, const double *__restrict__ Qb,
                                                    const uint64_t *__restrict__ y1, const uint64_t *__restrict__ y0,
                                                    int continuous, LmmLinOut o)
{
    const int64_t v = (int64_t)blockIdx.x * 256 + threadIdx.x;
    double xky = 0, dg = 0, s1 = 0, q1 = 0;
    double c[DP > 0 ? DP : 1];
#pragma unroll
    for (int d = 0; d < DP; d++) c[d] = 0;
    int t11 = 0, t01 = 0, m = 0;
    for (int sb = 0; sb < NB64; sb++) {
        const uint64_t w = T[(int64_t)sb * Vpad + v];
        m += __popcll(w); t11 += __popcll(w & y1[sb]); t01 += __popcll(w & y0[sb]);
        const int nb = min(64, N - sb * 64);
        for (int b = 0; b < nb; b++) {
            const int i = sb * 64 + b;
            const double xd = (double)(unsigned)((w >> b) & 1ull);
            xky = fma(xd, vv[i], xky);
            dg = fma(xd, mdiag[i], dg);
            if (continuous) { const double t = yc[i]; s1 = fma(xd, t, s1); q1 = fma(xd, t * t, q1); }
#pragma unroll
            for (int d = 0; d < DP; d++) c[d] = fma(xd, Qb[(int64_t)i * DP + d], c[d]);
        }
    }
    double rss;
    if (DP > 0) {
        rss = 0;
        for (int sb = 0; sb < NB64; sb++) {
            const uint64_t w = T[(int64_t)sb * Vpad + v];
            const int nb = min(64, N - sb * 64);
            for (int b = 0; b < nb; b++) {
                const int i = sb * 64 + b;
                double r = (double)(unsigned)((w >> b) & 1ull);
#pragma unroll
                for (int d = 0; d < DP; d++) r = fma(-Qb[(int64_t)i * DP + d], c[d], r);
                rss = fma(r, r, rss);
            }
        }
    } else {
        rss = (double)m * (double)(N - m) / (double)N;
    }
    o.t11[v] = t11; o.t01[v] = t01; o.m[v] = m;
    o.xky[v] = xky; o.dg[v] = dg; o.rss[v] = rss; o.s1[v] = s1; o.q1[v] = q1;
}

__global__ __launch_bounds__(256) void k_lmm_build_tab(const double *__restrict__ vv, const double *__restrict__ mdiag, int N, int NB64,
                                                       double2 *__restrict__ tab)
{
    const int e = blockIdx.x * 256 + threadIdx.x;
    if (e >= NB64 * 256) return;
    const int value = e & 15, base = (e >> 4) * 4;
    double a = 0.0, b = 0.0;
    for (int k = 0; k < 4; ++k)
        if (((value >> k) & 1) && base + k < N) { a += vv[base + k]; b += mdiag[base + k]; }
    tab[e] = make_double2(a, b);
}

__global__ __launch_bounds__(256) void k_lmm_linear_tab(const uint64_t *__restrict__ T, int64_t Vpad, int N, int NB64,
                                                        const double2 *__restrict__ tab, const uint64_t *__restrict__ y1,
                                                        const uint64_t *__restrict__ y0, LmmLinOut o)
{
    __shared__ double2 lt[2][256];
    const int tid = threadIdx.x;
    const int64_t v = (int64_t)blockIdx.x * 256 + tid;
    double xky = 0, dg = 0;
    int t11 = 0, t01 = 0, m = 0;
    lt[0][tid] = tab[tid];
    for (int sb = 0; sb < NB64; sb++) {
        const double2 nxt = (sb + 1 < NB64) ? tab[(sb + 1) * 256 + tid] : make_double2(0.0, 0.0);
        const uint64_t w = T[(int64_t)sb * Vpad + v];
        __syncthreads();
        m += __popcll(w); t11 += __popcll(w & y1[sb]); t01 += __popcll(w & y0[sb]);
        const double2 *cur = lt[sb & 1];
        const uint32_t lo = (uint32_t)w, hi = (uint32_t)(w >> 32);
#pragma unroll
        for (int nib = 0; nib < 8; ++nib) {
            const double2 e0 = cur[nib * 16 + ((lo >> (4 * nib)) & 15u)];
            const double2 e1 = cur[(8 + nib) * 16 + ((hi >> (4 * nib)) & 15u)];
            xky += e0.x; dg += e0.y; xky += e1.x; dg += e1.y;
        }
        lt[(sb + 1) & 1][tid] = nxt;
    }
    o.t11[v] = t11; o.t01[v] = t01; o.m[v] = m;
    o.xky[v] = xky; o.dg[v] = dg; o.rss[v] = (double)m * (double)(N - m) / (double)N; o.s1[v] = 0.0; o.q1[v] = 0.0;
}

template <int NE>
__global__ __launch_bounds__(256) void k_lmm_build_tabn(const double *__restrict__ vv, const double *__restrict__ mdiag,
                                                        const double *__restrict__ yc, const double *__restrict__ Qb, int DP, int cont,
                                                        int N, int NB64, double *__restrict__ tab)
{
    const int e = blockIdx.x * 256 + threadIdx.x;
    if (e >= NB64 * 256) return;
    const int value = e & 15, base = (e >> 4) * 4;
    for (int c = 0; c < NE; ++c) {
        double a = 0.0;
        for (int k = 0; k < 4; ++k) {
            const int i = base + k;
            if (!((value >> k) & 1) || i >= N) continue;
            double x;
            if (c == 0) x = vv[i]; else if (c == 1) x = mdiag[i];
            else if (cont && c == 2) x = yc[i]; else if (cont && c == 3) x = yc[i] * yc[i];
            else x = Qb[(int64_t)i * DP + (c - 2 - 2 * cont)];
            a += x;
        }
        tab[(int64_t)e * NE + c] = a;
    }
}

template <int NE>
__global__ __launch_bounds__(256) void k_lmm_linear_tabn(const uint64_t *__restrict__ T, int64_t Vpad, int N, int NB64,
                                                         const double *__restrict__ tab, const uint64_t *__restrict__ y1,
                                                         const uint64_t *__restrict__ y0, const double *__restrict__ Qb, int DP,
                                                         int cont, LmmLinOut o)
{
    __shared__ __attribute__((aligned(16))) double lt[2][256 * NE];
    const int tid = threadIdx.x;
    const int64_t v = (int64_t)blockIdx.x * 256 + tid;
    double acc[NE];
#pragma unroll
    for (int c = 0; c < NE; ++c) acc[c] = 0.0;
    int t11 = 0, t01 = 0, m = 0;
#pragma unroll
    for (int c = 0; c < NE; ++c) lt[0][tid * NE + c] = tab[(int64_t)tid * NE + c];
    for (int sb = 0; sb < NB64; sb++) {
        double nxt[NE];
        const bool more = sb + 1 < NB64;
#pragma unroll
        for (int c = 0; c < NE; ++c) nxt[c] = more ? tab[((int64_t)(sb + 1) * 256 + tid) * NE + c] : 0.0;
        const uint64_t w = T[(int64_t)sb * Vpad + v];
        __syncthreads();
        m += __popcll(w); t11 += __popcll(w & y1[sb]); t01 += __popcll(w & y0[sb]);
        const double *cur = lt[sb & 1];
#pragma unroll 4
        for (int nib = 0; nib < 16; ++nib) {
            const double *e = cur + (nib * 16 + (int)((w >> (4 * nib)) & 15ull)) * NE;
#pragma unroll
            for (int c = 0; c < NE; ++c) acc[c] += e[c];
        }
#pragma unroll
        for (int c = 0; c < NE; ++c) lt[(sb + 1) & 1][tid * NE + c] = nxt[c];
    }
    const int c0 = 2 + 2 * cont;
    double rss;
    if (DP > 0) {
        double sc = 0.0;
        for (int d = 0; d < NE - c0; ++d) sc = fma(acc[c0 + d], acc[c0 + d], sc);
        rss = (double)m - sc;
        const bool susp = rss <= 1e-8 * fmax((double)m, 1.0);
        if (__any(susp)) {
            double ex = 0.0;
            for (int sb = 0; sb < NB64; sb++) {
                const uint64_t w = T[(int64_t)sb * Vpad + v];
                const int nb = min(64, N - sb * 64);
                for (int b = 0; b < nb; b++) {
                    const int i = sb * 64 + b;
                    double r = (double)(unsigned)((w >> b) & 1ull);
                    for (int d = 0; d < NE - c0; ++d) r = fma(-Qb[(int64_t)i * DP + d], acc[c0 + d], r);
                    ex = fma(r, r, ex);
                }
            }
            if (susp) rss = ex;
        }
    } else {
        rss = (double)m * (double)(N - m) / (double)N;
    }
    o.t11[v] = t11; o.t01[v] = t01; o.m[v] = m;
    o.xky[v] = acc[0]; o.dg[v] = acc[1]; o.rss[v] = rss;
    o.s1[v] = cont ? acc[2] : 0.0; o.q1[v] = cont ? acc[3] : 0.0;
}

template __global__ void k_lmm_linear<0>(const uint64_t *, int64_t, int, int, const double *, const double *, const double *, const double *, const uint64_t *, const uint64_t *, int, LmmLinOut);
template __global__ void k_lmm_linear<4>(const uint64_t *, int64_t, int, int, const double *, const double *, const double *, const double *, const uint64_t *, const uint64_t *, int, LmmLinOut);
template __global__ void k_lmm_linear<8>(const uint64_t *, int64_t, int, int, const double *, const double *, const double *, const double *, const uint64_t *, const uint64_t *, int, LmmLinOut);
template __global__ void k_lmm_linear<16>(const uint64_t *, int64_t, int, int, const double *, const double *, const double *, const double *, const uint64_t *, const uint64_t *, int, LmmLinOut);
template __global__ void k_lmm_linear<32>(const uint64_t *, int64_t, int, int, const double *, const double *, const double *, const double *, const uint64_t *, const uint64_t *, int, LmmLinOut);

#define QF_TILE_BYTES 8192
#define QF_BN 512

__device__ __forceinline__ int qf_off(int row, int chunk) { return row * 64 + ((chunk ^ ((row >> 2) & 3)) << 4); }

__device__ __forceinline__ uint4 qf_expand16(uint32_t bits16)
{
    uint4 r;
    r.x = (((bits16) & 0xFu) * 0x00204081u) & 0x01010101u;
    r.y = (((bits16 >> 4) & 0xFu) * 0x00204081u) & 0x01010101u;
    r.z = (((bits16 >> 8) & 0xFu) * 0x00204081u) & 0x01010101u;
    r.w = (((bits16 >> 12) & 0xFu) * 0x00204081u) & 0x01010101u;
    return r;
}

#ifndef QF_G_AUX
#define QF_G_AUX 0
#endif
#ifndef QF_JT
#define QF_JT 2
#endif
#define QF_WAVES (16 / QF_JT)
#define QF_DMA_PER_WAVE (24 / QF_WAVES)
#ifndef QF_DIAG_TRIM
#define QF_DIAG_TRIM 0
#endif
#ifndef QF_NST
#define QF_NST 5
#endif
#define QF_AHEAD (QF_NST - 1)
#define QF_STAGE_BYTES (2 * QF_TILE_BYTES + 2 * QF_BN * 8)

__device__ __forceinline__ void qf_dma_stage(const int8_t *gsrc, const uint64_t *tsrc, int64_t Vpad, char *slot, int wave, int lane)
{
#pragma unroll
    for (int j = 0; j < 16 / QF_WAVES; ++j) {
        const int piece = wave * (16 / QF_WAVES) + j;
        __builtin_amdgcn_global_load_lds((const __attribute__((address_space(1))) void *)(gsrc + piece * 1024 + lane * 16),
                                         (__attribute__((address_space(3))) void *)(slot + piece * 1024), 16, 0, QF_G_AUX);
    }
#pragma unroll
    for (int j = 0; j < 8 / QF_WAVES; ++j) {
        const int pb = wave * (8 / QF_WAVES) + j;
        const uint64_t *src = tsrc + (int64_t)(pb >> 2) * Vpad + (pb & 3) * 128 + lane * 2;
        __builtin_amdgcn_global_load_lds((const __attribute__((address_space(1))) void *)src,
                                         (__attribute__((address_space(3))) void *)(slot + 2 * QF_TILE_BYTES + pb * 1024), 16, 0, 0);
    }
}

template <int N> __device__ __forceinline__ void qf_wait_vm() { asm volatile("s_waitcnt vmcnt(%0)" ::"n"(N) : "memory"); }

template <int ABL>
__global__ __launch_bounds__(64 * QF_WAVES, QF_JT == 2 ? 2 : 1) void k_lmm_quadform_i8(const int8_t *__restrict__ G, const uint64_t *__restrict__ T,
                                                            int64_t Vpad, int NR, int L, int lsplit, double *__restrict__ qout,
                                                            const int *__restrict__ nlimit)
{
    extern __shared__ __attribute__((aligned(16))) char smem[];
    const int tid = threadIdx.x, lane = tid & 63, wave = tid >> 6;
    const int l31 = lane & 31, lh = lane >> 5;
    const int ntiles = (int)(Vpad / QF_BN);
    int tile, lgrp;
    if ((ntiles & 7) == 0) { const int xcd = blockIdx.x & 7, w = blockIdx.x >> 3; tile = (w / lsplit) * 8 + xcd; lgrp = w % lsplit; }
    else { tile = blockIdx.x / lsplit; lgrp = blockIdx.x % lsplit; }
    const int nl = (L - lgrp + lsplit - 1) / lsplit;
    const int64_t v0 = (int64_t)tile * QF_BN;
    if (nlimit && v0 >= (int64_t)*nlimit) return;
    const bool big = NR * 128 > 65535;
    const int64_t TL = (int64_t)NR * (NR + 1);
    const int total = nl * (NR * (NR + 1) / 2);
    int aoff[4][2];
#pragma unroll
    for (int it = 0; it < 4; ++it) { aoff[it][0] = qf_off(it * 32 + l31, lh); aoff[it][1] = qf_off(it * 32 + l31, 2 + lh); }
    const int boff = 2 * QF_TILE_BYTES + (wave * (32 * QF_JT) + l31) * 8;

    double tot[QF_JT];
#pragma unroll
    for (int jt = 0; jt < QF_JT; ++jt) tot[jt] = 0.0;
    v16i acc[4][QF_JT];
    int pI = 0, pl = 0, pst = 0, pslot = 0;
    int cI = 0, cl = 0, cst = 0;
    double scale0 = 1.0, step = 1.0;
    for (int i = 0; i < lgrp; ++i) scale0 *= 256.0;
    for (int i = 0; i < lsplit; ++i) step *= 256.0;
    double scale_l = scale0;

    auto fetch = [&]() {
        const int8_t *g = G + ((int64_t)(lgrp + pl * lsplit) * TL + (int64_t)pI * (pI + 1) + 2 * pst) * QF_TILE_BYTES;
        const uint64_t *t = T + (int64_t)(2 * pst) * Vpad + v0;
        if (ABL & 8) { g = G; t = T + v0; }
        if (!(ABL & 1)) qf_dma_stage(g, t, Vpad, smem + pslot * QF_STAGE_BYTES, wave, lane);
        if (++pslot == QF_NST) pslot = 0;
        if (++pst == pI + 1) { pst = 0; if (++pl == nl) { pl = 0; ++pI; } }
    };

#pragma unroll 1
    for (int s = 0; s < QF_AHEAD && s < total; ++s) fetch();

    auto sync_refill = [&](int s) {
        const int newer = max(0, min(total - 2 - s, QF_AHEAD - 2));
        if (!(ABL & 1)) {
            if (newer >= 3) qf_wait_vm<3 * QF_DMA_PER_WAVE>(); else if (newer == 2) qf_wait_vm<2 * QF_DMA_PER_WAVE>();
            else if (newer == 1) qf_wait_vm<QF_DMA_PER_WAVE>(); else qf_wait_vm<0>();
        }
        if (!(ABL & 16)) __builtin_amdgcn_s_barrier();
        __builtin_amdgcn_sched_barrier(0);
        if (s + QF_AHEAD < total) fetch();
    };
    auto read_bits = [&](const char *base, uint64_t (&w)[2][QF_JT]) {
#pragma unroll
        for (int jt = 0; jt < QF_JT; ++jt) {
            w[0][jt] = *reinterpret_cast<const uint64_t *>(base + boff + 256 * jt);
            w[1][jt] = *reinterpret_cast<const uint64_t *>(base + boff + QF_BN * 8 + 256 * jt);
        }
    };
    auto expand = [&](const uint64_t (&w)[2][QF_JT], int sub, v4i (&b)[QF_JT]) {
        const int tl = sub >> 1, kh = sub & 1;
#pragma unroll
        for (int jt = 0; jt < QF_JT; ++jt) {
            const uint32_t h = lh ? (uint32_t)(w[tl][jt] >> 32) : (uint32_t)w[tl][jt];
            uint4 e;
            if (ABL & 4) e = make_uint4(h, kh, jt, 1);
            else e = make_uint4((h >> (4 * kh)) & 0x01010101u, (h >> (4 * kh + 1)) & 0x01010101u,
                                (h >> (4 * kh + 2)) & 0x01010101u, (h >> (4 * kh + 3)) & 0x01010101u);
            b[jt] = (v4i){(int)e.x, (int)e.y, (int)e.z, (int)e.w};
        }
    };

    uint64_t wb[2][QF_JT], wbn[2][QF_JT];
    v4i a_cur[4], a_nxt[4], b_cur[QF_JT], b_nxt[QF_JT];
    sync_refill(0);
    read_bits(smem, wb);
#pragma unroll
    for (int it = 0; it < 4; ++it) a_cur[it] = (ABL & 2) ? (v4i){it, lane, 0, 1} : *reinterpret_cast<const v4i *>(smem + aoff[it][0]);
    expand(wb, 0, b_cur);

    int slot = 0;
#pragma unroll 1
    for (int s = 0; s < total; ++s) {
        if (s > 0) sync_refill(s);
        if ((ABL & 256) ? s == 0 : cst == 0) {
#pragma unroll
            for (int it = 0; it < 4; ++it)
#pragma unroll
                for (int jt = 0; jt < QF_JT; ++jt)
#pragma unroll
                    for (int r = 0; r < 16; ++r) acc[it][jt][r] = 0;
        }
        const char *a_base = smem + slot * QF_STAGE_BYTES;
        const char *n_base = smem + (slot + 1 == QF_NST ? 0 : slot + 1) * QF_STAGE_BYTES;
        const bool diag = (cst == cI);
        __builtin_amdgcn_sched_barrier(0);
#pragma unroll
        for (int sub = 0; sub < 4; ++sub) {
            if (sub < 3) {
                const int nt = (sub + 1) >> 1, nk = (sub + 1) & 1;
#pragma unroll
                for (int it = 0; it < 4; ++it)
                    a_nxt[it] = (ABL & 2) ? (v4i){it, lane, nt, nk}
                                          : *reinterpret_cast<const v4i *>(a_base + nt * QF_TILE_BYTES + aoff[it][nk]);
                if (sub == 2) read_bits(n_base, wbn);
            } else {
#pragma unroll
                for (int it = 0; it < 4; ++it)
                    a_nxt[it] = (ABL & 2) ? (v4i){it, lane, s, 1} : *reinterpret_cast<const v4i *>(n_base + aoff[it][0]);
            }
#pragma unroll
            for (int it = 0; it < 4; ++it) {
                if (QF_DIAG_TRIM && sub >= 2 && it < 2 && diag) continue;
#pragma unroll
                for (int jt = 0; jt < QF_JT; ++jt)
                    acc[it][jt] = __builtin_amdgcn_mfma_i32_32x32x32_i8(a_cur[it], b_cur[jt], acc[it][jt], 0, 0, 0);
            }
            if (sub < 3) expand(wb, sub + 1, b_nxt); else expand(wbn, 0, b_nxt);
            __builtin_amdgcn_sched_barrier(0);
#pragma unroll
            for (int it = 0; it < 4; ++it) a_cur[it] = a_nxt[it];
#pragma unroll
            for (int jt = 0; jt < QF_JT; ++jt) b_cur[jt] = b_nxt[jt];
        }
        if (++slot == QF_NST) slot = 0;
        if (++cst == cI + 1) {
#pragma unroll
            for (int jt = 0; jt < QF_JT; ++jt) {
                int part[4];
                if (ABL & 128) { tot[jt] += (double)(acc[0][jt][0] + acc[1][jt][1] + acc[2][jt][2] + acc[3][jt][3]); continue; }
#pragma unroll
                for (int it = 0; it < 4; ++it) {
                    const uint32_t w = (uint32_t)(wb[it >> 1][jt] >> ((it & 1) * 32 + 4 * lh));
                    part[it] = 0;
                    if (!big) {
#pragma unroll
                        for (int r = 0; r < 16; ++r) {
                            const int row = (r & 3) + 8 * (r >> 2);
                            const int bit = (int)__builtin_amdgcn_ubfe(w, row, 1);
                            asm("v_mad_i32_i24 %0, %1, %2, %0" : "+v"(part[it]) : "v"(acc[it][jt][r]), "v"(bit));
                        }
                    } else {
#pragma unroll
                        for (int r = 0; r < 16; ++r) {
                            const int row = (r & 3) + 8 * (r >> 2);
                            part[it] += ((w >> row) & 1u) ? acc[it][jt][r] : 0;
                        }
                    }
                }
                tot[jt] = fma((double)((part[0] + part[1]) + (part[2] + part[3])), scale_l, tot[jt]);
            }
            cst = 0; scale_l *= step;
            if (++cl == nl) { cl = 0; scale_l = scale0; ++cI; }
        }
#pragma unroll
        for (int jt = 0; jt < QF_JT; ++jt) { wb[0][jt] = wbn[0][jt]; wb[1][jt] = wbn[1][jt]; }
    }
#pragma unroll
    for (int jt = 0; jt < QF_JT; ++jt) tot[jt] += __shfl_xor(tot[jt], 32, 64);
    if (lh == 0) {
        double *qo = qout + (int64_t)lgrp * Vpad + v0 + wave * (32 * QF_JT) + l31;
#pragma unroll
        for (int jt = 0; jt < QF_JT; ++jt) qo[32 * jt] = tot[jt];
    }
}

#include "lmm_quadform_wide.inc"


struct LinV { int m, t11, t01, mst; double xky, dg, rss, s1, q1; };
__device__ __forceinline__ LinV lin_load(const LmmLinOut &li, const LmmFinParams &P, int64_t v)
{
    LinV r;
    r.mst = li.m[v]; r.m = r.mst; r.t11 = li.t11[v]; r.t01 = li.t01[v];
    r.xky = li.xky[v]; r.dg = li.dg[v]; r.rss = li.rss[v]; r.s1 = li.s1[v]; r.q1 = li.q1[v];
    if (li.flip && li.flip[v]) {
        r.m = P.N - r.mst; r.t11 = P.n1 - r.t11; r.t01 = P.n0 - r.t01;
        r.xky = P.sumv - r.xky; r.s1 = P.yc_sum - r.s1; r.q1 = P.yc_sq - r.q1;
    }
    return r;
}

__device__ __forceinline__ double lmm_fin_one(int64_t v, int64_t V, int64_t Vpad, int nq, const LmmLinOut &li, const double *__restrict__ q,
                                              const LmmFinParams &P, double q_extra, bool refined, double *__restrict__ out,
                                              uint32_t *__restrict__ flags, bool *want_refine)
{
    const double nanv = NAN;
    double prep = nanv, pval = nanv, beta = nanv, bse = nanv, frac = nanv, bound = 0.0;
    uint32_t fl = 0;
    const LinV L = lin_load(li, P, v);
    const int m = L.m;
    bool go = true;
    *want_refine = false;
    if (P.af_on) {
        const double af = (double)m / (double)P.N;
        if (!(P.min_af <= af && af <= P.max_af)) { fl = SH_NOTE_AF_FILTER | SH_FLAG_PREFILTER; go = false; }
    }
    if (go) {
        bool bad = false;
        if (P.continuous) {
            const double n1 = (double)m, n0 = (double)(P.N - m);
            prep = sh_prefilter_welch(n1, L.s1, L.q1, n0, P.yc_sum - L.s1, P.yc_sq - L.q1);
        } else {
            prep = sh_prefilter_binary(L.t11, P.n1 - L.t11, L.t01, P.n0 - L.t01, &bad);
        }
        if (bad) fl |= SH_NOTE_BAD_CHISQ;
        if (prep >= P.pret || !isfinite(prep)) fl |= SH_NOTE_PRE_FILTER | SH_FLAG_PREFILTER;
    }
    if (go && !((fl & SH_FLAG_PREFILTER) && P.pret < 1.0)) {
        const bool zeroed = sqrt(L.rss / (double)P.N) <= 1e-10;
        double qs = 0.0;
        for (int a = 0; a < nq; ++a) qs += q[(int64_t)a * Vpad + v];
        const double xKx = zeroed ? 0.0 : (L.dg + (qs * P.inv_scale + q_extra));
        const double xKy = zeroed ? 0.0 : L.xky;
        if (!zeroed && xKx > 0.0) {
            bound = (refined ? P.err_norm * (P.inv_scale_low / P.inv_scale) : P.err_norm) * (double)L.mst / xKx;
            if (!refined && P.tol > 0.0 && bound > P.tol) *want_refine = true;
        }
        double b = xKy / xKx;
        if (isnan(b) && xKy == 0.0) b = 0.0;
        const double veb = xKy * b, r2 = P.yKy - veb;
        const double var = r2 / ((double)(P.N - P.D) - 1.0) / xKx;
        const double chi2 = b * b / var;
        pval = sh_f_sf_1(chi2, (double)(P.N - (P.D + 1)));
        beta = b; bse = sqrt(var); frac = sqrt(veb / P.yKy);
        if (!(fl & SH_FLAG_PREFILTER)) {
            if (pval >= P.lrtt || !isfinite(pval)) fl |= SH_NOTE_LRT_FILTER | SH_FLAG_FILTER;
        }
    }
    out[v] = prep; out[V + v] = pval; out[2 * V + v] = beta; out[3 * V + v] = bse; out[4 * V + v] = frac;
    flags[v] = fl;
    return bound;
}

__device__ __forceinline__ void lmm_bound_max(double bound, unsigned long long *bound_max)
{
    for (int o = 32; o > 0; o >>= 1) bound = fmax(bound, __shfl_xor(bound, o, 64));
    if ((threadIdx.x & 63) == 0 && bound > 0.0 && bound_max) atomicMax(bound_max, (unsigned long long)__double_as_longlong(bound));
}

__global__ __launch_bounds__(256) void k_lmm_finalize(int64_t V, int64_t Vpad, int nq, LmmLinOut li, const double *__restrict__ q,
                                                      LmmFinParams P, double *__restrict__ out, uint32_t *__restrict__ flags, LmmRefine R)
{
    const int64_t v = (int64_t)blockIdx.x * 256 + threadIdx.x;
    const int lane = threadIdx.x & 63;
    bool ref = false;
    double bound = 0.0;
    if (v < V) bound = lmm_fin_one(v, V, Vpad, nq, li, q, P, 0.0, false, out, flags, &ref);
    const unsigned long long rm = __ballot(ref);
    if (rm && R.list) {
        int base = 0;
        if (lane == 0) base = atomicAdd(R.count, __popcll(rm));
        base = __shfl(base, 0);
        if (ref) R.list[base + __popcll(rm & ((1ull << lane) - 1ull))] = (int)v;
    }
    lmm_bound_max((ref && R.list) ? 0.0 : bound, R.bound_max);
}

__global__ __launch_bounds__(256) void k_lmm_refine_fix(int64_t V, int64_t Vpad, int nq, int nq3, LmmLinOut li, const double *__restrict__ q,
                                                        const double *__restrict__ q3, LmmFinParams P, double *__restrict__ out,
                                                        uint32_t *__restrict__ flags, LmmRefine R)
{
    const int n = *R.count;
    for (int64_t j0 = (int64_t)blockIdx.x * 256; j0 < n; j0 += (int64_t)gridDim.x * 256) {
        const int64_t j = j0 + threadIdx.x;
        double bound = 0.0;
        if (j < n) {
            const int64_t v = R.list[j];
            double qe = 0.0;
            for (int a = 0; a < nq3; ++a) qe += q3[(int64_t)a * Vpad + j];
            bool dummy;
            bound = lmm_fin_one(v, V, Vpad, nq, li, q, P, qe * P.inv_scale_low, true, out, flags, &dummy);
        }
        lmm_bound_max(bound, R.bound_max);
    }
}

__global__ __launch_bounds__(256) void k_gather_T_list(const uint64_t *__restrict__ T, int64_t Vpad, uint64_t *__restrict__ T3, LmmRefine R)
{
    const int n = *R.count;
    const int64_t npad = ((int64_t)n + 511) / 512 * 512;
    const int64_t sb = blockIdx.y;
    for (int64_t j = (int64_t)blockIdx.x * 256 + threadIdx.x; j < npad; j += (int64_t)gridDim.x * 256)
        T3[sb * Vpad + j] = j < n ? T[sb * Vpad + R.list[j]] : 0ull;
}

__global__ __launch_bounds__(256) void k_af_keep(int64_t V, LmmLinOut li, LmmFinParams P, int *__restrict__ idx, int *__restrict__ n)
{
    const int64_t v = (int64_t)blockIdx.x * 256 + threadIdx.x;
    const int lane = threadIdx.x & 63;
    bool keep = false;
    if (v < V) {
        const LinV L = lin_load(li, P, v);
        const int m = L.m;
        keep = true;
        if (P.af_on) { const double af = (double)m / (double)P.N; keep = (P.min_af <= af && af <= P.max_af); }
        if (keep && P.pret < 1.0) {
            bool bad = false; double prep;
            if (P.continuous) prep = sh_prefilter_welch((double)m, L.s1, L.q1, (double)(P.N - m), P.yc_sum - L.s1, P.yc_sq - L.q1);
            else prep = sh_prefilter_binary(L.t11, P.n1 - L.t11, L.t01, P.n0 - L.t01, &bad);
            keep = !(prep >= P.pret || !isfinite(prep));
        }
    }
    const unsigned long long km = __ballot(keep);
    int base = 0;
    if (lane == 0 && km) base = atomicAdd(n, __popcll(km));
    base = __shfl(base, 0);
    if (keep) idx[base + __popcll(km & ((1ull << lane) - 1ull))] = (int)v;
}

__global__ __launch_bounds__(256) void k_gather_T(const uint64_t *__restrict__ T, int64_t Vpad, uint64_t *__restrict__ T2, int64_t Vpad2,
                                                  const int *__restrict__ idx, int nk)
{
    const int64_t j = (int64_t)blockIdx.x * 256 + threadIdx.x;
    if (j >= Vpad2) return;
    const int64_t sb = blockIdx.y;
    T2[sb * Vpad2 + j] = j < nk ? T[sb * Vpad + idx[j]] : 0ull;
}

__global__ __launch_bounds__(256) void k_scatter_q(const double *__restrict__ q2, int64_t Vpad2, double *__restrict__ q, int64_t Vpad,
                                                   const int *__restrict__ idx, int nk)
{
    const int64_t j = (int64_t)blockIdx.x * 256 + threadIdx.x;
    if (j >= nk) return;
    q[(int64_t)blockIdx.y * Vpad + idx[j]] = q2[(int64_t)blockIdx.y * Vpad2 + j];
}

extern "C" hipError_t shk_af_compact(hipStream_t st, int which, int64_t V, LmmLinOut li, LmmFinParams P, int *idx, int *n,
                                     const uint64_t *T, int64_t Vpad, uint64_t *T2, int64_t Vpad2, int rows, int nk,
                                     const double *q2, double *q)
{
    if (which == 0) hipLaunchKernelGGL(k_af_keep, dim3((unsigned)((V + 255) / 256)), dim3(256), 0, st, V, li, P, idx, n);
    else if (which == 1) hipLaunchKernelGGL(k_gather_T, dim3((unsigned)((Vpad2 + 255) / 256), (unsigned)rows), dim3(256), 0, st, T, Vpad, T2, Vpad2, idx, nk);
    else hipLaunchKernelGGL(k_scatter_q, dim3((unsigned)((nk + 255) / 256), (unsigned)rows), dim3(256), 0, st, q2, Vpad2, q, Vpad, idx, nk);
    return hipGetLastError();
}


__global__ __launch_bounds__(256) void k_syrk_f64(const double *__restrict__ W, const double *__restrict__ sgn,
                                                  int Np, int kp, double *__restrict__ M, int mirror = 0)
{
    int t = blockIdx.x, bi = 0;
    while ((bi + 1) * (bi + 2) / 2 <= t) ++bi;
    const int bj = t - bi * (bi + 1) / 2;
    const int lane = threadIdx.x & 63, wave = threadIdx.x >> 6;
    const int i0 = bi * 128 + (wave >> 1) * 64, j0 = bj * 128 + (wave & 1) * 64;
    const int lr = lane & 15, lk = lane >> 4;
    v4d acc[4][4];
#pragma unroll
    for (int a = 0; a < 4; ++a)
#pragma unroll
        for (int b = 0; b < 4; ++b) acc[a][b] = (v4d){0, 0, 0, 0};
    const double *Ai = W + (int64_t)(i0 + lr) * kp + lk;
    const double *Bj = W + (int64_t)(j0 + lr) * kp + lk;
    for (int kk = 0; kk < kp; kk += 4) {
        const double sg = sgn ? sgn[kk + lk] : 1.0;
        double a[4], b[4];
#pragma unroll
        for (int x = 0; x < 4; ++x) { a[x] = Ai[(int64_t)x * 16 * kp + kk] * sg; b[x] = Bj[(int64_t)x * 16 * kp + kk]; }
#pragma unroll
        for (int x = 0; x < 4; ++x)
#pragma unroll
            for (int y = 0; y < 4; ++y)
                acc[x][y] = __builtin_amdgcn_mfma_f64_16x16x4f64(a[x], b[y], acc[x][y], 0, 0, 0);
    }
#pragma unroll
    for (int x = 0; x < 4; ++x)
#pragma unroll
        for (int y = 0; y < 4; ++y)
#pragma unroll
            for (int r = 0; r < 4; ++r) {
                M[(int64_t)(i0 + x * 16 + lk + 4 * r) * Np + (j0 + y * 16 + lr)] = acc[x][y][r];
                if (mirror && bi != bj) M[(int64_t)(j0 + y * 16 + lr) * Np + (i0 + x * 16 + lk + 4 * r)] = acc[x][y][r];
            }
}

__global__ __launch_bounds__(256) void k_lower_absmax(const double *__restrict__ M, int N, int Np,
                                                      unsigned long long *__restrict__ amax)
{
    const int i = blockIdx.x;
    double mx = 0;
    for (int j = threadIdx.x; j < i; j += 256) mx = fmax(mx, fabs(2.0 * M[(int64_t)i * Np + j]));
    for (int o = 32; o > 0; o >>= 1) mx = fmax(mx, __shfl_xor(mx, o, 64));
    if ((threadIdx.x & 63) == 0 && mx > 0) atomicMax(amax, (unsigned long long)__double_as_longlong(mx));
}

__global__ void k_extract_diag(const double *__restrict__ M, int N, int Np, double *__restrict__ mdiag)
{
    const int i = blockIdx.x * blockDim.x + threadIdx.x;
    if (i < N) mdiag[i] = M[(int64_t)i * Np + i];
}

__global__ __launch_bounds__(128) void k_lmm_quantize(const double *__restrict__ M, int N, int Np, int NR, int Lt, int E,
                                                      const unsigned long long *__restrict__ amax_bits,
                                                      int8_t *__restrict__ G, float *__restrict__ Ef)
{
    int t = blockIdx.x, I = 0;
    while ((I + 1) * (I + 2) <= t) ++I;
    const int ks = t - I * (I + 1);
    const int r = threadIdx.x;
    const int i = I * 128 + r;
    const double amax = __longlong_as_double((long long)*amax_bits);
    double p256 = 1.0;
    for (int l = 0; l < Lt; ++l) p256 *= 256.0;
    const double scale = amax > 0 ? 0.49 * p256 / amax : 0.0;
    const int64_t TL = (int64_t)NR * (NR + 1);
    for (int ch = 0; ch < 4; ++ch) {
        long long qv[16];
        double fr[16];
        int jj[16];
#pragma unroll
        for (int c = 0; c < 16; ++c) {
            const int j = ks * 64 + 32 * (ch & 1) + 8 * (c & 3) + 4 * (ch >> 1) + (c >> 2);
            double g = 0.0;
            if (i < N && j < i) g = 2.0 * M[(int64_t)i * Np + j];
            const double gs = g * scale;
            qv[c] = llrint(gs); fr[c] = gs - (double)qv[c]; jj[c] = j;
        }
        for (int l = 0; l < Lt; ++l) {
            if (l == E && Ef) {
#pragma unroll
                for (int c = 0; c < 16; ++c) {
                    const int j = jj[c];
                    if (i < N && j < i) {
                        const float e = (float)(fr[c] * 0.5);
                        Ef[(int64_t)i * Np + j] = e; Ef[(int64_t)j * Np + i] = e;
                    }
                }
            }
            uint32_t pk[4] = {0, 0, 0, 0};
#pragma unroll
            for (int c = 0; c < 16; ++c) {
                long long d = ((qv[c] + 128) & 255) - 128;
                qv[c] = (qv[c] - d) >> 8;
                if (l < E) fr[c] = (fr[c] + (double)d) * (1.0 / 256.0);
                pk[c >> 2] |= ((uint32_t)(d & 255)) << (8 * (c & 3));
            }
            uint4 o; o.x = pk[0]; o.y = pk[1]; o.z = pk[2]; o.w = pk[3];
            *reinterpret_cast<uint4 *>(G + ((int64_t)l * TL + t) * QF_TILE_BYTES + qf_off(r, ch)) = o;
        }
    }
}

__global__ __launch_bounds__(256) void k_symv_f32(const float *__restrict__ A, int N, int Np, const double *__restrict__ x, double *__restrict__ y)
{
    __shared__ double red[4];
    const int i = blockIdx.x;
    double s = 0.0;
    for (int j = threadIdx.x; j < N; j += 256) s = fma((double)A[(int64_t)i * Np + j], x[j], s);
    for (int o = 32; o > 0; o >>= 1) s += __shfl_xor(s, o, 64);
    if ((threadIdx.x & 63) == 0) red[threadIdx.x >> 6] = s;
    __syncthreads();
    if (threadIdx.x == 0) y[i] = (red[0] + red[1]) + (red[2] + red[3]);
}

__global__ __launch_bounds__(256) void k_f32_to_f64_sq(const float *__restrict__ A, int N, int Np, double *__restrict__ X)
{
    const int64_t i = (int64_t)blockIdx.x * 256 + threadIdx.x;
    if (i >= (int64_t)Np * Np) return;
    const int r = (int)(i / Np), c = (int)(i % Np);
    X[i] = (r < N && c < N) ? (double)A[i] : 0.0;
}

__global__ __launch_bounds__(256) void k_frob2(const double *__restrict__ X, int64_t n, double *__restrict__ out)
{
    __shared__ double red[4];
    double s = 0.0;
    for (int64_t i = (int64_t)blockIdx.x * 256 + threadIdx.x; i < n; i += (int64_t)gridDim.x * 256) s = fma(X[i], X[i], s);
    for (int o = 32; o > 0; o >>= 1) s += __shfl_xor(s, o, 64);
    if ((threadIdx.x & 63) == 0) red[threadIdx.x >> 6] = s;
    __syncthreads();
    if (threadIdx.x == 0) atomicAdd(out, (red[0] + red[1]) + (red[2] + red[3]));
}

__global__ __launch_bounds__(256) void k_scale_pow2(double *__restrict__ X, int64_t n, const double *__restrict__ frob2, int *__restrict__ exps, int step)
{
    int e2; (void)frexp(sqrt(*frob2), &e2);
    const int e = -(e2 - 1);
    if (blockIdx.x == 0 && threadIdx.x == 0) exps[step] = e;
    for (int64_t i = (int64_t)blockIdx.x * 256 + threadIdx.x; i < n; i += (int64_t)gridDim.x * 256) X[i] = ldexp(X[i], e);
}

__global__ __launch_bounds__(1024) void k_pow_norm(const double *__restrict__ y, double *__restrict__ x, int N, double *__restrict__ nrm, int it)
{
    __shared__ double red[16];
    __shared__ double tot;
    double s = 0.0;
    for (int j = threadIdx.x; j < N; j += 1024) s = fma(y[j], y[j], s);
    for (int o = 32; o > 0; o >>= 1) s += __shfl_xor(s, o, 64);
    if ((threadIdx.x & 63) == 0) red[threadIdx.x >> 6] = s;
    __syncthreads();
    if (threadIdx.x == 0) { double t = 0; for (int w = 0; w < 16; ++w) t += red[w]; tot = sqrt(t); nrm[it] = tot; }
    __syncthreads();
    const double inv = tot > 0.0 ? 1.0 / tot : 0.0;
    for (int j = threadIdx.x; j < N; j += 1024) x[j] = y[j] * inv;
}

__global__ void k_pow_init(double *__restrict__ x, int N)
{
    const int i = blockIdx.x * blockDim.x + threadIdx.x;
    if (i < N) { unsigned h = (unsigned)i * 2654435761u; h ^= h >> 15; h *= 2246822519u; h ^= h >> 13; x[i] = ((double)(h & 0xFFFF) - 32767.5) / 32768.0; }
}

extern "C" {

hipError_t shk_repack_bits(hipStream_t st, const uint8_t *bits, int64_t row_bytes, int64_t V, int64_t Vpad, int N,
                           int NB64, uint64_t *T, uint8_t *flip)
{
    const size_t lds = (size_t)64 * row_bytes;
    if (lds > 64 * 1024) {
        if (Vpad & 255) return hipErrorInvalidValue;
        if (flip) hipLaunchKernelGGL(k_row_flip, dim3((unsigned)((V + 3) / 4)), dim3(256), 0, st, bits, row_bytes, V, N, flip);
        hipLaunchKernelGGL(k_repack_bits_gather, dim3((unsigned)(Vpad / 256), (unsigned)NB64), dim3(256), 0, st, bits, row_bytes, V, Vpad, N, T, flip);
        return hipGetLastError();
    }
    static bool attr_set = false;
    if (!attr_set) { (void)hipFuncSetAttribute(reinterpret_cast<const void *>(k_repack_bits), hipFuncAttributeMaxDynamicSharedMemorySize, 64 * 1024); attr_set = true; }
    hipLaunchKernelGGL(k_repack_bits, dim3((unsigned)(Vpad / 64)), dim3(256), lds, st, bits, row_bytes, V, Vpad, N, NB64, T, flip);
    return hipGetLastError();
}

static int lin_tab_ne(int DP, int continuous) { return (DP == 0 || DP == 4 || DP == 8) ? 2 + 2 * (continuous ? 1 : 0) + DP : 0; }

hipError_t shk_lmm_build_tab(hipStream_t st, const double *vv, const double *mdiag, const double *yc, const double *Qb, int DP,
                             int continuous, int N, int NB64, double *tab)
{
    const dim3 g((unsigned)NB64), b(256);
    const int cont = continuous ? 1 : 0;
    switch (lin_tab_ne(DP, continuous)) {
    case 2: hipLaunchKernelGGL(k_lmm_build_tab, g, b, 0, st, vv, mdiag, N, NB64, reinterpret_cast<double2 *>(tab)); break;
    case 4: hipLaunchKernelGGL(k_lmm_build_tabn<4>, g, b, 0, st, vv, mdiag, yc, Qb, DP, cont, N, NB64, tab); break;
    case 6: hipLaunchKernelGGL(k_lmm_build_tabn<6>, g, b, 0, st, vv, mdiag, yc, Qb, DP, cont, N, NB64, tab); break;
    case 8: hipLaunchKernelGGL(k_lmm_build_tabn<8>, g, b, 0, st, vv, mdiag, yc, Qb, DP, cont, N, NB64, tab); break;
    case 10: hipLaunchKernelGGL(k_lmm_build_tabn<10>, g, b, 0, st, vv, mdiag, yc, Qb, DP, cont, N, NB64, tab); break;
    case 12: hipLaunchKernelGGL(k_lmm_build_tabn<12>, g, b, 0, st, vv, mdiag, yc, Qb, DP, cont, N, NB64, tab); break;
    default: return hipSuccess;
    }
    return hipGetLastError();
}

hipError_t shk_lmm_linear(hipStream_t st, int DP, const uint64_t *T, int64_t Vpad, int N, int NB64, const double *vv,
                          const double *mdiag, const double *yc, const double *Qb, const uint64_t *y1,
                          const uint64_t *y0, int continuous, const double *tab, LmmLinOut o)
{
    dim3 grid((unsigned)(Vpad / 256)), blk(256);
    const int cont = continuous ? 1 : 0;
    if (tab) {
        switch (lin_tab_ne(DP, continuous)) {
        case 2: hipLaunchKernelGGL(k_lmm_linear_tab, grid, blk, 0, st, T, Vpad, N, NB64, reinterpret_cast<const double2 *>(tab), y1, y0, o); return hipGetLastError();
        case 4: hipLaunchKernelGGL(k_lmm_linear_tabn<4>, grid, blk, 0, st, T, Vpad, N, NB64, tab, y1, y0, Qb, DP, cont, o); return hipGetLastError();
        case 6: hipLaunchKernelGGL(k_lmm_linear_tabn<6>, grid, blk, 0, st, T, Vpad, N, NB64, tab, y1, y0, Qb, DP, cont, o); return hipGetLastError();
        case 8: hipLaunchKernelGGL(k_lmm_linear_tabn<8>, grid, blk, 0, st, T, Vpad, N, NB64, tab, y1, y0, Qb, DP, cont, o); return hipGetLastError();
        case 10: hipLaunchKernelGGL(k_lmm_linear_tabn<10>, grid, blk, 0, st, T, Vpad, N, NB64, tab, y1, y0, Qb, DP, cont, o); return hipGetLastError();
        case 12: hipLaunchKernelGGL(k_lmm_linear_tabn<12>, grid, blk, 0, st, T, Vpad, N, NB64, tab, y1, y0, Qb, DP, cont, o); return hipGetLastError();
        default: break;
        }
    }
    switch (DP) {
    case 0: hipLaunchKernelGGL(k_lmm_linear<0>, grid, blk, 0, st, T, Vpad, N, NB64, vv, mdiag, yc, Qb, y1, y0, continuous, o); break;
    case 4: hipLaunchKernelGGL(k_lmm_linear<4>, grid, blk, 0, st, T, Vpad, N, NB64, vv, mdiag, yc, Qb, y1, y0, continuous, o); break;
    case 8: hipLaunchKernelGGL(k_lmm_linear<8>, grid, blk, 0, st, T, Vpad, N, NB64, vv, mdiag, yc, Qb, y1, y0, continuous, o); break;
    case 16: hipLaunchKernelGGL(k_lmm_linear<16>, grid, blk, 0, st, T, Vpad, N, NB64, vv, mdiag, yc, Qb, y1, y0, continuous, o); break;
    case 32: hipLaunchKernelGGL(k_lmm_linear<32>, grid, blk, 0, st, T, Vpad, N, NB64, vv, mdiag, yc, Qb, y1, y0, continuous, o); break;
    default: return hipErrorInvalidValue;
    }
    return hipGetLastError();
}

hipError_t shk_lmm_quadform(hipStream_t st, int variant, const int8_t *G, const uint64_t *T, int64_t Vpad, int NR, int L, int lsplit, double *q,
                            const int *nlimit, int rows_last, int64_t *macs_per_variant)
{
    const bool wide_ok = lsplit == L && NR >= 4 && (uint64_t)NR * 2 * (uint64_t)Vpad * 8 < (1ull << 32) && (uint64_t)(L + 1) * NR * (NR + 1) * QF_TILE_BYTES < (1ull << 32);
    const bool wide_var = variant == 4 || variant == 6 || variant == 7 || variant == 8 || variant == 9 || variant == 50 || variant == 441 || variant == 162 || variant == 35;
    if (wide_var && !wide_ok) variant = 0;
    const bool refine_wide = true;
    if (variant == 64 && wide_ok && refine_wide) variant = 464;
    const bool wide = (wide_var && wide_ok) || variant == 464;
    const int nit_last = !wide ? 4 : rows_last <= 0 ? 0 : rows_last <= 32 ? 1 : rows_last <= 64 ? 2 : 4;
    if (macs_per_variant)
        *macs_per_variant = (int64_t)L * ((int64_t)(NR - 1) * NR * 128 * 64 + (int64_t)2 * NR * 32 * nit_last * 64);
    const dim3 g((unsigned)(Vpad / QF_BN * lsplit)), b(wide ? 256 : 64 * QF_WAVES);
    const size_t lds = QF_NST * QF_STAGE_BYTES;
    static bool attr_set = false;
    if (!attr_set) {
        (void)hipFuncSetAttribute(reinterpret_cast<const void *>(k_lmm_quadform_i8<0>), hipFuncAttributeMaxDynamicSharedMemorySize, (int)lds);
        (void)hipFuncSetAttribute(reinterpret_cast<const void *>(k_lmm_quadform_i8<1>), hipFuncAttributeMaxDynamicSharedMemorySize, (int)lds);
        (void)hipFuncSetAttribute(reinterpret_cast<const void *>(k_lmm_quadform_i8<2>), hipFuncAttributeMaxDynamicSharedMemorySize, (int)lds);
        (void)hipFuncSetAttribute(reinterpret_cast<const void *>(k_lmm_quadform_i8<4>), hipFuncAttributeMaxDynamicSharedMemorySize, (int)lds);
        (void)hipFuncSetAttribute(reinterpret_cast<const void *>(k_lmm_quadform_i8<7>), hipFuncAttributeMaxDynamicSharedMemorySize, (int)lds);
        (void)hipFuncSetAttribute(reinterpret_cast<const void *>(k_lmm_quadform_i8<8>), hipFuncAttributeMaxDynamicSharedMemorySize, (int)lds);
        (void)hipFuncSetAttribute(reinterpret_cast<const void *>(k_lmm_quadform_i8<16>), hipFuncAttributeMaxDynamicSharedMemorySize, (int)lds);
        (void)hipFuncSetAttribute(reinterpret_cast<const void *>(k_lmm_quadform_i8<23>), hipFuncAttributeMaxDynamicSharedMemorySize, (int)lds);
        (void)hipFuncSetAttribute(reinterpret_cast<const void *>(k_lmm_quadform_i8<64>), hipFuncAttributeMaxDynamicSharedMemorySize, (int)lds);
        (void)hipFuncSetAttribute(reinterpret_cast<const void *>(k_lmm_quadform_i8<128>), hipFuncAttributeMaxDynamicSharedMemorySize, (int)lds);
        (void)hipFuncSetAttribute(reinterpret_cast<const void *>(k_lmm_quadform_i8<256>), hipFuncAttributeMaxDynamicSharedMemorySize, (int)lds);
        (void)hipFuncSetAttribute(reinterpret_cast<const void *>(k_lmm_quadform_i8<384>), hipFuncAttributeMaxDynamicSharedMemorySize, (int)lds);
        (void)hipFuncSetAttribute(reinterpret_cast<const void *>(k_lmm_quadform_i8<407>), hipFuncAttributeMaxDynamicSharedMemorySize, (int)lds);
        (void)hipFuncSetAttribute(reinterpret_cast<const void *>(k_lmm_quadform_i8w<0>), hipFuncAttributeMaxDynamicSharedMemorySize, (int)lds);
        (void)hipFuncSetAttribute(reinterpret_cast<const void *>(k_lmm_quadform_i8w<0, 3>), hipFuncAttributeMaxDynamicSharedMemorySize, (int)lds);
        (void)hipFuncSetAttribute(reinterpret_cast<const void *>(k_lmm_quadform_i8w<0, 0, 1>), hipFuncAttributeMaxDynamicSharedMemorySize, (int)lds);
        (void)hipFuncSetAttribute(reinterpret_cast<const void *>(k_lmm_quadform_i8w<0, 0, 2>), hipFuncAttributeMaxDynamicSharedMemorySize, (int)lds);
        (void)hipFuncSetAttribute(reinterpret_cast<const void *>(k_lmm_quadform_i8w<16, 0, 1>), hipFuncAttributeMaxDynamicSharedMemorySize, (int)lds);
        (void)hipFuncSetAttribute(reinterpret_cast<const void *>(k_lmm_quadform_i8w<1, 0, 1>), hipFuncAttributeMaxDynamicSharedMemorySize, (int)lds);
        (void)hipFuncSetAttribute(reinterpret_cast<const void *>(k_lmm_quadform_i8w<16>), hipFuncAttributeMaxDynamicSharedMemorySize, (int)lds);
        (void)hipFuncSetAttribute(reinterpret_cast<const void *>(k_lmm_quadform_i8w<1>), hipFuncAttributeMaxDynamicSharedMemorySize, (int)lds);
        (void)hipFuncSetAttribute(reinterpret_cast<const void *>(k_lmm_quadform_i8w<128>), hipFuncAttributeMaxDynamicSharedMemorySize, (int)lds);
        (void)hipFuncSetAttribute(reinterpret_cast<const void *>(k_lmm_quadform_i8w<407>), hipFuncAttributeMaxDynamicSharedMemorySize, (int)lds);
        attr_set = true;
    }
    switch (variant) {
    case 31: hipLaunchKernelGGL(k_lmm_quadform_i8<1>, g, b, lds, st, G, T, Vpad, NR, L, lsplit, q, nlimit); break;
    case 32: hipLaunchKernelGGL(k_lmm_quadform_i8<2>, g, b, lds, st, G, T, Vpad, NR, L, lsplit, q, nlimit); break;
    case 34: hipLaunchKernelGGL(k_lmm_quadform_i8<4>, g, b, lds, st, G, T, Vpad, NR, L, lsplit, q, nlimit); break;
    case 53: hipLaunchKernelGGL(k_lmm_quadform_i8<23>, g, b, lds, st, G, T, Vpad, NR, L, lsplit, q, nlimit); break;
    case 46: hipLaunchKernelGGL(k_lmm_quadform_i8<16>, g, b, lds, st, G, T, Vpad, NR, L, lsplit, q, nlimit); break;
    case 38: hipLaunchKernelGGL(k_lmm_quadform_i8<8>, g, b, lds, st, G, T, Vpad, NR, L, lsplit, q, nlimit); break;
    case 37: hipLaunchKernelGGL(k_lmm_quadform_i8<7>, g, b, lds, st, G, T, Vpad, NR, L, lsplit, q, nlimit); break;
    case 64: hipLaunchKernelGGL(k_lmm_quadform_i8<64>, g, b, lds, st, G, T, Vpad, NR, L, lsplit, q, nlimit); break;
    case 158: hipLaunchKernelGGL(k_lmm_quadform_i8<128>, g, b, lds, st, G, T, Vpad, NR, L, lsplit, q, nlimit); break;
    case 286: hipLaunchKernelGGL(k_lmm_quadform_i8<256>, g, b, lds, st, G, T, Vpad, NR, L, lsplit, q, nlimit); break;
    case 414: hipLaunchKernelGGL(k_lmm_quadform_i8<384>, g, b, lds, st, G, T, Vpad, NR, L, lsplit, q, nlimit); break;
    case 464: hipLaunchKernelGGL((k_lmm_quadform_i8w<0, 3>), g, b, lds, st, G, T, Vpad, NR, L, lsplit, q, nlimit, nit_last); break;
    case 4: hipLaunchKernelGGL(k_lmm_quadform_i8w<0>, g, b, lds, st, G, T, Vpad, NR, L, lsplit, q, nlimit, nit_last); break;
    case 6: hipLaunchKernelGGL((k_lmm_quadform_i8w<0, 0, 1>), g, b, lds, st, G, T, Vpad, NR, L, lsplit, q, nlimit, nit_last); break;
    case 7: hipLaunchKernelGGL((k_lmm_quadform_i8w<0, 0, 2>), g, b, lds, st, G, T, Vpad, NR, L, lsplit, q, nlimit, nit_last); break;
    case 8: hipLaunchKernelGGL((k_lmm_quadform_i8w<16, 0, 1>), g, b, lds, st, G, T, Vpad, NR, L, lsplit, q, nlimit, nit_last); break;
    case 9: hipLaunchKernelGGL((k_lmm_quadform_i8w<1, 0, 1>), g, b, lds, st, G, T, Vpad, NR, L, lsplit, q, nlimit, nit_last); break;
    case 50: hipLaunchKernelGGL(k_lmm_quadform_i8w<16>, g, b, lds, st, G, T, Vpad, NR, L, lsplit, q, nlimit, nit_last); break;
    case 35: hipLaunchKernelGGL(k_lmm_quadform_i8w<1>, g, b, lds, st, G, T, Vpad, NR, L, lsplit, q, nlimit, nit_last); break;
    case 162: hipLaunchKernelGGL(k_lmm_quadform_i8w<128>, g, b, lds, st, G, T, Vpad, NR, L, lsplit, q, nlimit, nit_last); break;
    case 441: hipLaunchKernelGGL(k_lmm_quadform_i8w<407>, g, b, lds, st, G, T, Vpad, NR, L, lsplit, q, nlimit, nit_last); break;
    case 437: hipLaunchKernelGGL(k_lmm_quadform_i8<407>, g, b, lds, st, G, T, Vpad, NR, L, lsplit, q, nlimit); break;
    default: hipLaunchKernelGGL(k_lmm_quadform_i8<0>, g, b, lds, st, G, T, Vpad, NR, L, lsplit, q, nlimit); break;
    }
    return hipGetLastError();
}

hipError_t shk_lmm_finalize(hipStream_t st, int64_t V, int64_t Vpad, int nq, LmmLinOut li, const double *q, LmmFinParams P, double *out,
                            uint32_t *flags, LmmRefine R)
{
    hipLaunchKernelGGL(k_lmm_finalize, dim3((unsigned)((V + 255) / 256)), dim3(256), 0, st, V, Vpad, nq, li, q, P, out, flags, R);
    return hipGetLastError();
}

hipError_t shk_lmm_refine(hipStream_t st, int64_t V, int64_t Vpad, int nq, int E, int NR, int NB64p, const int8_t *Glow, const uint64_t *T,
                          uint64_t *T3, double *q3, LmmLinOut li, const double *q, LmmFinParams P, double *out, uint32_t *flags, LmmRefine R)
{
    hipLaunchKernelGGL(k_gather_T_list, dim3(64, (unsigned)NB64p), dim3(256), 0, st, T, Vpad, T3, R);
    hipError_t e = shk_lmm_quadform(st, 64, Glow, T3, Vpad, NR, E, E, q3, R.count, 128, nullptr);
    if (e != hipSuccess) return e;
    hipLaunchKernelGGL(k_lmm_refine_fix, dim3(64), dim3(256), 0, st, V, Vpad, nq, E, li, q, q3, P, out, flags, R);
    return hipGetLastError();
}

hipError_t shk_lmm_build_G(hipStream_t st, const double *W, const double *sgn, int N, int Np, int kp, int NR, int Lt, int E,
                           double *M, double *mdiag, unsigned long long *amax, int8_t *G, float *Ef, double *px, double *py, double *nrm, int npow)
{
    const int nb = Np / 128;
    (void)hipMemsetAsync(amax, 0, sizeof(unsigned long long), st);
    hipLaunchKernelGGL(k_syrk_f64, dim3((unsigned)(nb * (nb + 1) / 2)), dim3(256), 0, st, W, sgn, Np, kp, M);
    hipLaunchKernelGGL(k_lower_absmax, dim3((unsigned)N), dim3(256), 0, st, M, N, Np, amax);
    hipLaunchKernelGGL(k_extract_diag, dim3((unsigned)((N + 255) / 256)), dim3(256), 0, st, M, N, Np, mdiag);
    if (Ef) (void)hipMemsetAsync(Ef, 0, sizeof(float) * (size_t)Np * Np, st);
    hipLaunchKernelGGL(k_lmm_quantize, dim3((unsigned)(NR * (NR + 1))), dim3(128), 0, st, M, N, Np, NR, Lt, E, amax, G, Ef);
    if (Ef) {
        hipLaunchKernelGGL(k_pow_init, dim3((unsigned)((N + 255) / 256)), dim3(256), 0, st, px, N);
        for (int it = 0; it < npow; ++it) {
            hipLaunchKernelGGL(k_symv_f32, dim3((unsigned)N), dim3(256), 0, st, Ef, N, Np, px, py);
            hipLaunchKernelGGL(k_pow_norm, dim3(1), dim3(1024), 0, st, py, px, N, nrm, it);
        }
    }
    return hipGetLastError();
}

hipError_t shk_power_norm(hipStream_t st, const float *A, int N, int Np, double *px, double *py, double *nrm, int npow)
{
    hipLaunchKernelGGL(k_pow_init, dim3((unsigned)((N + 255) / 256)), dim3(256), 0, st, px, N);
    for (int it = 0; it < npow; ++it) {
        hipLaunchKernelGGL(k_symv_f32, dim3((unsigned)N), dim3(256), 0, st, A, N, Np, px, py);
        hipLaunchKernelGGL(k_pow_norm, dim3(1), dim3(1024), 0, st, py, px, N, nrm, it);
    }
    return hipGetLastError();
}

hipError_t shk_spectral_bound(hipStream_t st, const float *A, int N, int Np, double *X, double *Y, int nsq, double *work, int *exps)
{
    const int nb = Np / 128;
    const int64_t n2 = (int64_t)Np * Np;
    hipLaunchKernelGGL(k_f32_to_f64_sq, dim3((unsigned)((n2 + 255) / 256)), dim3(256), 0, st, A, N, Np, X);
    double *cur = X, *nxt = Y;
    for (int k = 0; k <= nsq; ++k) {
        (void)hipMemsetAsync(work, 0, sizeof(double), st);
        hipLaunchKernelGGL(k_frob2, dim3(1024), dim3(256), 0, st, cur, n2, work);
        if (k == nsq) break;
        hipLaunchKernelGGL(k_scale_pow2, dim3(1024), dim3(256), 0, st, cur, n2, work, exps, k);
        hipLaunchKernelGGL(k_syrk_f64, dim3((unsigned)(nb * (nb + 1) / 2)), dim3(256), 0, st, cur, (const double *)nullptr, Np, Np, nxt, 1);
        std::swap(cur, nxt);
    }
    (void)hipMemcpyAsync(work + 1, work, sizeof(double), hipMemcpyDeviceToDevice, st);
    return hipGetLastError();
}

}
```

### pyseer_amd/csrc/lmm_params.h

```cpp
#pragma once

struct LmmLinOut {
    int *t11, *t01, *m;
    double *xky, *dg, *rss, *s1, *q1;
    const unsigned char *flip;
};

struct LmmFinParams {
    int N, D, continuous;
    int n1, n0;
    double yc_sum, yc_sq;
    double yKy, inv_scale;
    double pret, lrtt;
    double min_af, max_af; int af_on;
    double sumv;
    double err_norm;
    double tol;
    double inv_scale_low;
};

struct LmmRefine {
    int *list, *count;
    unsigned long long *bound_max;
};
```

### pyseer_amd/csrc/lmm_quadform_wide.inc

```
#define QW_ALL_AGPRS "a0","a1","a2","a3","a4","a5","a6","a7","a8","a9","a10","a11","a12","a13","a14","a15","a16","a17","a18","a19","a20","a21","a22","a23","a24","a25","a26","a27","a28","a29","a30","a31","a32","a33","a34","a35","a36","a37","a38","a39","a40","a41","a42","a43","a44","a45","a46","a47","a48","a49","a50","a51","a52","a53","a54","a55","a56","a57","a58","a59","a60","a61","a62","a63","a64","a65","a66","a67","a68","a69","a70","a71","a72","a73","a74","a75","a76","a77","a78","a79","a80","a81","a82","a83","a84","a85","a86","a87","a88","a89","a90","a91","a92","a93","a94","a95","a96","a97","a98","a99","a100","a101","a102","a103","a104","a105","a106","a107","a108","a109","a110","a111","a112","a113","a114","a115","a116","a117","a118","a119","a120","a121","a122","a123","a124","a125","a126","a127","a128","a129","a130","a131","a132","a133","a134","a135","a136","a137","a138","a139","a140","a141","a142","a143","a144","a145","a146","a147","a148","a149","a150","a151","a152","a153","a154","a155","a156","a157","a158","a159","a160","a161","a162","a163","a164","a165","a166","a167","a168","a169","a170","a171","a172","a173","a174","a175","a176","a177","a178","a179","a180","a181","a182","a183","a184","a185","a186","a187","a188","a189","a190","a191","a192","a193","a194","a195","a196","a197","a198","a199","a200","a201","a202","a203","a204","a205","a206","a207","a208","a209","a210","a211","a212","a213","a214","a215","a216","a217","a218","a219","a220","a221","a222","a223","a224","a225","a226","a227","a228","a229","a230","a231","a232","a233","a234","a235","a236","a237","a238","a239","a240","a241","a242","a243","a244","a245","a246","a247","a248","a249","a250","a251","a252","a253","a254","a255"

typedef int v2i_t __attribute__((ext_vector_type(2)));

#define QW_SREGS "s84", "s85", "s86", "s87", "s88", "s89", "s90", "s91", "s92", "s93", "s94", "s95", "s96", "s97", "s98", "s99", "scc"

__device__ __forceinline__ void qw_read_bits(v2i_t (&H)[2][2], int h_addr)
{
    asm volatile("ds_read2st64_b32 %0, %4 offset1:1\n\tds_read2st64_b32 %1, %4 offset0:2 offset1:3\n\t"
                 "ds_read2st64_b32 %2, %4 offset0:16 offset1:17\n\tds_read2st64_b32 %3, %4 offset0:18 offset1:19"
                 : "+v"(H[0][0]), "+v"(H[0][1]), "+v"(H[1][0]), "+v"(H[1][1]) : "v"(h_addr) : "memory");
}

#include "lmm_quadform_wide_substeps.inc"

template <int ABL, int DM = 0, int PROF = 0>
__global__ __launch_bounds__(256, 1) void k_lmm_quadform_i8w(const int8_t *__restrict__ G, const uint64_t *__restrict__ T,
                                                              int64_t Vpad, int NR, int L, int lsplit, double *__restrict__ qout,
                                                              const int *__restrict__ nlimit, int nit_last)
{
    constexpr int JT = 4, DMA_PER_WAVE = 6;
    extern __shared__ __attribute__((aligned(16))) char smem[];
    const int tid = threadIdx.x, lane = tid & 63;
    const int wave = __builtin_amdgcn_readfirstlane(tid >> 6);
    const int l31 = lane & 31, lh = lane >> 5;
    const int ntiles = (int)(Vpad / QF_BN);
    int tile, lgrp;
    if ((ntiles & 7) == 0) { const int xcd = blockIdx.x & 7, w = blockIdx.x >> 3; tile = (w / lsplit) * 8 + xcd; lgrp = w % lsplit; }
    else { tile = blockIdx.x / lsplit; lgrp = blockIdx.x % lsplit; }
    const int nl = (L - lgrp + lsplit - 1) / lsplit;
    const int64_t v0 = (int64_t)tile * QF_BN;
    if (nlimit && v0 >= (int64_t)*nlimit) return;
    asm volatile("" ::: QW_ALL_AGPRS);
    const int64_t TL = (int64_t)NR * (NR + 1);
    const uint32_t smem_base = (uint32_t)(uintptr_t)smem;
    const int aoff0 = qf_off(l31, lh), aoff1 = qf_off(l31, 2 + lh);
    const int boff = 2 * QF_TILE_BYTES + (wave * (32 * JT) + l31) * 8;
    auto make_rsrc = [](const void *p) -> v4i {
        const uint64_t a = (uint64_t)(uintptr_t)p;
        return (v4i){__builtin_amdgcn_readfirstlane((int)(uint32_t)a), __builtin_amdgcn_readfirstlane((int)(uint32_t)((a >> 32) & 0xffffu)), -1, 0x00020000};
    };
    const v4i rsG = make_rsrc(G), rsT = make_rsrc(T + v0);
    uint32_t gvoff[4], tvoff[2];
#pragma unroll
    for (int j = 0; j < 4; ++j) gvoff[j] = (uint32_t)((wave * 4 + j) * 1024 + lane * 16);
#pragma unroll
    for (int j = 0; j < 2; ++j) { const int pb = wave * 2 + j; tvoff[j] = (uint32_t)(((int64_t)(pb >> 2) * Vpad + (pb & 3) * 128 + lane * 2) * 8); }

    double tot[JT];
#pragma unroll
    for (int jt = 0; jt < JT; ++jt) tot[jt] = 0.0;
    double scale0 = 1.0;
    for (int i = 0; i < lgrp; ++i) scale0 *= 256.0;

    uint32_t gso = (uint32_t)((int64_t)lgrp * TL * QF_TILE_BYTES), tso = 0, prem = 1, plen = 2;
    const uint32_t tinc = (uint32_t)(2 * Vpad * 8);
    auto dma1 = [&](uint32_t lds_dst, uint32_t voff, const v4i &rs, uint32_t so) {
        if (!(ABL & 1)) asm volatile("s_mov_b32 m0, %0\n\ts_nop 0\n\tbuffer_load_dwordx4 %1, %2, %3 offen lds" ::"s"(lds_dst), "v"(voff), "s"(rs), "s"(so) : "memory");
    };
#pragma unroll 1
    for (int s = 0; s < QF_AHEAD; ++s) {
        const uint32_t dslot = smem_base + s * QF_STAGE_BYTES;
#pragma unroll
        for (int j = 0; j < 4; ++j) dma1(dslot + (wave * 4 + j) * 1024, gvoff[j], rsG, gso);
#pragma unroll
        for (int j = 0; j < 2; ++j) dma1(dslot + 2 * QF_TILE_BYTES + (wave * 2 + j) * 1024, tvoff[j], rsT, tso);
        gso += 2 * QF_TILE_BYTES; tso += tinc;
        if (--prem == 0) { tso = 0; prem = plen; ++plen; }
    }
    if (!(ABL & 1)) qf_wait_vm<(QF_AHEAD - 2) * DMA_PER_WAVE>();
    __builtin_amdgcn_s_barrier();

    v4i AP[4], AQ[4], BP[4], BQ[4];
    v2i_t HC[2][2], HN[2][2];
#pragma unroll
    for (int it = 0; it < 4; ++it) { AP[it] = (v4i){0, 0, 0, 0}; AQ[it] = (v4i){0, 0, 0, 0}; }
#pragma unroll
    for (int a = 0; a < 2; ++a)
#pragma unroll
        for (int b = 0; b < 2; ++b) { HC[a][b] = (v2i_t){0, 0}; HN[a][b] = (v2i_t){0, 0}; }
    {
        const int a0 = (int)smem_base + aoff0;
#pragma unroll
        for (int it = 0; it < 4; ++it) asm volatile("ds_read_b128 %0, %1 offset:%c2" : "+v"(AP[it]) : "v"(a0), "i"(it * 2048) : "memory");
        qw_read_bits(HC, (int)smem_base + boff + 4 * lh);
        asm volatile("s_waitcnt lgkmcnt(0)" : "+v"(AP[0]), "+v"(AP[1]), "+v"(AP[2]), "+v"(AP[3]), "+v"(HC[0][0]), "+v"(HC[0][1]), "+v"(HC[1][0]), "+v"(HC[1][1]));
#pragma unroll
        for (int jt = 0; jt < JT; ++jt) {
            const uint32_t h = (uint32_t)HC[0][jt >> 1][jt & 1];
            BP[jt] = (v4i){(int)(h & 0x01010101u), (int)((h >> 1) & 0x01010101u), (int)((h >> 2) & 0x01010101u), (int)((h >> 3) & 0x01010101u)};
        }
    }

    const int boffl = boff + 4 * lh;
    int a0c = (int)smem_base + aoff0, a1c = (int)smem_base + aoff1;
    int a0n = a0c + QF_STAGE_BYTES, a1n = a1c + QF_STAGE_BYTES, hbn = (int)smem_base + QF_STAGE_BYTES + boffl;
    asm volatile("s_mov_b32 s84, %0\n\ts_mov_b32 s85, %1\n\ts_add_u32 s86, %1, 0x6000\n\ts_mov_b32 s87, %1\n\t"
                 "s_add_u32 s88, %2, %3\n\ts_add_u32 s89, %2, %4\n\ts_mov_b32 s90, %5\n\ts_mov_b32 s91, %6\n\ts_mov_b32 s92, %7\n\ts_mov_b32 s93, %8\n\t"
                 "s_add_u32 s94, %1, %9\n\ts_mov_b32 s95, %1\n\ts_mov_b32 s96, %3\n\ts_mov_b32 s97, %4\n\ts_mov_b32 s98, 0x01010101\n\ts_mov_b32 s99, 0x6000"
                 ::"s"(prem), "s"(smem_base), "s"(smem_base + QF_AHEAD * QF_STAGE_BYTES), "s"(wave * 4096), "s"(2 * QF_TILE_BYTES + wave * 2048), "s"(gso),
                   "s"(tso), "s"(plen), "s"(tinc), "s"(QF_NST * QF_STAGE_BYTES) : QW_SREGS);
    uint64_t pt_wait = 0, pt_sub[4] = {0, 0, 0, 0}, pt_epi = 0, pt_tail = 0, pt0 = 0, pt1 = 0;
#define QW_STAMP(ACCU) if (PROF) { pt1 = __builtin_amdgcn_s_memtime(); ACCU += pt1 - pt0; pt0 = pt1; }
    if (PROF) pt0 = __builtin_amdgcn_s_memtime();

    auto stage = [&](auto zc, auto nc) {
        constexpr bool Z = decltype(zc)::value; constexpr int NIT = decltype(nc)::value;
#define QW_H(HH, TLX, JTX) ((uint32_t)HH[TLX][(JTX) >> 1][(JTX) & 1])
#define QW_BIND(AF, BF, RF, TLX, HH, ADDR, OFFV)                                                                                          \
        v4i(&A)[4] = AF; v4i(&B)[4] = BF; v4i(&R)[4] = RF; int N[4][4];                                                                    \
        const uint32_t H0 = QW_H(HH, TLX, 0), H1 = QW_H(HH, TLX, 1), H2 = QW_H(HH, TLX, 2), H3 = QW_H(HH, TLX, 3);                            \
        const int AA = ADDR; constexpr int OFF = OFFV;
#define QW_NEXT(BN) _Pragma("unroll") for (int it = 0; it < 4; ++it) BN[it] = (v4i){N[it][0], N[it][1], N[it][2], N[it][3]};
        const uint32_t(&GV)[4] = gvoff; const uint32_t(&TV)[2] = tvoff; const v4i &RSG = rsG, &RST = rsT;
        {
            QW_BIND(AP, BP, AQ, 0, HC, a1c, 0)
            if (NIT == 4) {
                if (Z) { if (ABL & 1) QW_SUB0Z_NODMA(); else if (ABL & 16) QW_SUB0Z_NOBAR(); else QW_SUB0Z(); }
                else { if (ABL & 1) QW_SUB0_NODMA(); else if (ABL & 16) QW_SUB0_NOBAR(); else QW_SUB0(); }
            } else if (NIT == 2) {
                if (Z) { if (ABL & 1) QW_SUB0Z_NODMA_N2(); else if (ABL & 16) QW_SUB0Z_NOBAR_N2(); else QW_SUB0Z_N2(); }
                else { if (ABL & 1) QW_SUB0_NODMA_N2(); else if (ABL & 16) QW_SUB0_NOBAR_N2(); else QW_SUB0_N2(); }
            } else {
                if (Z) { if (ABL & 1) QW_SUB0Z_NODMA_N1(); else if (ABL & 16) QW_SUB0Z_NOBAR_N1(); else QW_SUB0Z_N1(); }
                else { if (ABL & 1) QW_SUB0_NODMA_N1(); else if (ABL & 16) QW_SUB0_NOBAR_N1(); else QW_SUB0_N1(); }
            }
            QW_NEXT(BQ)
        }
        QW_STAMP(pt_sub[0])
        {
            QW_BIND(AQ, BQ, AP, 1, HC, a0c, 8192)
            if (NIT == 4) { if (ABL & 1) QW_SUB1_NODMA(); else QW_SUB1(); }
            else if (NIT == 2) { if (ABL & 1) QW_SUB1_NODMA_N2(); else QW_SUB1_N2(); }
            else { if (ABL & 1) QW_SUB1_NODMA_N1(); else QW_SUB1_N1(); }
            QW_NEXT(BP)
        }
        QW_STAMP(pt_sub[1])
        int a0n_n, a1n_n, hbn_n;
        {
            QW_BIND(AP, BP, AQ, 1, HC, a1c, 8192)
            const int HB = hbn, Y1 = aoff0; int X0;
            if (NIT == 4) QW_SUB2(); else if (NIT == 2) QW_SUB2_N2(); else QW_SUB2_N1();
            a0n_n = X0;
            QW_NEXT(BQ)
        }
        QW_STAMP(pt_sub[2])
        {
            QW_BIND(AQ, BQ, AP, 0, HN, a0n, 0)
            const int Y2 = aoff1, Y3 = boffl; int X1, X2;
            if (NIT == 4) QW_SUB3(); else if (NIT == 2) QW_SUB3_N2(); else QW_SUB3_N1();
            a1n_n = X1; hbn_n = X2;
            QW_NEXT(BP)
        }
#undef QW_H
        QW_STAMP(pt_sub[3])
        a0c = a0n; a1c = a1n; a0n = a0n_n; a1n = a1n_n; hbn = hbn_n;
    };

    auto segment = [&](auto nc, int cI, double scale_l) {
        constexpr int NIT = decltype(nc)::value;
        if (ABL & 256) { if (cI == 0) stage(std::true_type{}, nc); else stage(std::false_type{}, nc); }
        else stage(std::true_type{}, nc);
#pragma unroll 1
        for (int k = 1; k <= cI; ++k) stage(std::false_type{}, nc);
            v4i W[2][2];
#pragma unroll
        for (int a = 0; a < 2; ++a)
#pragma unroll
            for (int b = 0; b < 2; ++b) W[a][b] = (v4i){0, 0, 0, 0};
        int wa;
        asm volatile("s_cmp_eq_u32 s85, s95\n\ts_cselect_b32 s87, s94, s85\n\ts_sub_u32 s87, s87, s99\n\tv_add_u32 %0, s87, %1" : "=v"(wa) : "v"(boff) : QW_SREGS);
        asm volatile("ds_read2_b64 %[w0], %[p0] offset1:32\n\tds_read2_b64 %[w1], %[p0] offset0:64 offset1:96\n\t"
                     "ds_read2_b64 %[w2], %[p1] offset1:32\n\tds_read2_b64 %[w3], %[p1] offset0:64 offset1:96\n\t"
                     "s_waitcnt lgkmcnt(0)\n\ts_nop 7"
                     : [w0] "+v"(W[0][0]), [w1] "+v"(W[0][1]), [w2] "+v"(W[1][0]), [w3] "+v"(W[1][1]),
                       "+v"(AP[0]), "+v"(AP[1]), "+v"(AP[2]), "+v"(AP[3])
                     : [p0] "v"(wa), [p1] "v"(wa + QF_BN * 8) : "memory");
        if (ABL & 128) {
            int t0; asm volatile("v_accvgpr_read_b32 %0, a0" : "=v"(t0)); tot[0] += (double)(t0 + W[0][0][0]);
        } else {
#pragma unroll
            for (int jt = 0; jt < JT; ++jt) {
                int part[4] = {0, 0, 0, 0};
                uint32_t w[4];
#pragma unroll
                for (int it = 0; it < 4; ++it)
                    w[it] = (uint32_t)W[it >> 1][jt >> 1][(jt & 1) * 2 + (it & 1)] >> (4 * lh);
#pragma unroll
                for (int r = 0; r < 16; ++r) {
                    const int row = (r & 3) + 8 * (r >> 2);
                    int t0, t1, t2, t3, b0, b1, b2, b3;
                    if (NIT == 4)
                        asm volatile("v_accvgpr_read_b32 %[t0], a%c[i0]\n\tv_accvgpr_read_b32 %[t1], a%c[i1]\n\t"
                                         "v_accvgpr_read_b32 %[t2], a%c[i2]\n\tv_accvgpr_read_b32 %[t3], a%c[i3]\n\t"
                                         "v_bfe_u32 %[b0], %[w0], %c[row], 1\n\tv_bfe_u32 %[b1], %[w1], %c[row], 1\n\t"
                                         "v_bfe_u32 %[b2], %[w2], %c[row], 1\n\tv_bfe_u32 %[b3], %[w3], %c[row], 1\n\t"
                                         "v_mad_i32_i24 %[p0], %[t0], %[b0], %[p0]\n\tv_mad_i32_i24 %[p1], %[t1], %[b1], %[p1]\n\t"
                                         "v_mad_i32_i24 %[p2], %[t2], %[b2], %[p2]\n\tv_mad_i32_i24 %[p3], %[t3], %[b3], %[p3]"
                                         : [p0] "+v"(part[0]), [p1] "+v"(part[1]), [p2] "+v"(part[2]), [p3] "+v"(part[3]), [t0] "=&v"(t0), [t1] "=&v"(t1),
                                           [t2] "=&v"(t2), [t3] "=&v"(t3), [b0] "=&v"(b0), [b1] "=&v"(b1), [b2] "=&v"(b2), [b3] "=&v"(b3)
                                         : [w0] "v"(w[0]), [w1] "v"(w[1]), [w2] "v"(w[2]), [w3] "v"(w[3]), [row] "i"(row), [i0] "i"((0 * 4 + jt) * 16 + r),
                                           [i1] "i"((1 * 4 + jt) * 16 + r), [i2] "i"((2 * 4 + jt) * 16 + r), [i3] "i"((3 * 4 + jt) * 16 + r));
                    else {
#pragma unroll
                        for (int it = 0; it < NIT; ++it) {
                            int t, bb;
                            if (it == 0) asm volatile("v_accvgpr_read_b32 %[t], a%c[i]\n\tv_bfe_u32 %[b], %[w], %c[row], 1\n\tv_mad_i32_i24 %[p], %[t], %[b], %[p]"
                                                      : [p] "+v"(part[0]), [t] "=&v"(t), [b] "=&v"(bb) : [w] "v"(w[0]), [row] "i"(row), [i] "i"((0 * 4 + jt) * 16 + r));
                            else asm volatile("v_accvgpr_read_b32 %[t], a%c[i]\n\tv_bfe_u32 %[b], %[w], %c[row], 1\n\tv_mad_i32_i24 %[p], %[t], %[b], %[p]"
                                              : [p] "+v"(part[1]), [t] "=&v"(t), [b] "=&v"(bb) : [w] "v"(w[1]), [row] "i"(row), [i] "i"((1 * 4 + jt) * 16 + r));
                        }
                    }
                }
                tot[jt] = fma((double)((part[0] + part[1]) + (part[2] + part[3])), scale_l, tot[jt]);
            }
        }
        QW_STAMP(pt_epi)
    };
    const int NRfull = (nit_last == 4) ? NR : NR - 1;
#pragma unroll 1
    for (int cI = 0; cI < NRfull; ++cI) segment(std::integral_constant<int, 4>{}, cI, scale0);
    if (nit_last == 2) segment(std::integral_constant<int, 2>{}, NR - 1, scale0);
    else if (nit_last == 1) segment(std::integral_constant<int, 1>{}, NR - 1, scale0);
    const int total = nl * (NR * (NR + 1) / 2);
    asm volatile("s_waitcnt vmcnt(0) lgkmcnt(0)" ::: "memory");
    if (PROF && blockIdx.x == 0 && tid == 0)
        printf("wide prof (block 0, wave 0): stages %d  wait %llu  sub0 %llu  sub1 %llu  sub2 %llu  sub3 %llu  tail %llu  epilogue %llu  (cycles)\n", total,
               (unsigned long long)pt_wait, (unsigned long long)pt_sub[0], (unsigned long long)pt_sub[1], (unsigned long long)pt_sub[2],
               (unsigned long long)pt_sub[3], (unsigned long long)pt_tail, (unsigned long long)pt_epi);
#pragma unroll
    for (int jt = 0; jt < JT; ++jt) tot[jt] += __shfl_xor(tot[jt], 32, 64);
    if (lh == 0) {
        double *qo = qout + (int64_t)lgrp * Vpad + v0 + wave * (32 * JT) + l31;
#pragma unroll
        for (int jt = 0; jt < JT; ++jt) qo[32 * jt] = tot[jt];
    }
}
```

### pyseer_amd/csrc/route.h

```cpp
#pragma once
#include <cstdlib>
#include <cstring>
#include <string>

static inline const char *const *sh_route_keys()
{
    static const char *const keys[] = {"chord", "chord_n32", "chord_enter", "bitdot", "first_bordered", "pk", "warm", "fin_rounds", "ll_first", "newton",
                                       "firth_last", "firth_first32", "afcompact", "complement", "reader_slab", "reader_pad", "reader_chunk", "reader_workers", "reader_depth", "reader_helpers", "reader_target",
                                       "firth_literal", "firth_strict", "firth_fast", "firth_w", "lmm_limbs", "lmm_tol", "qf", "lanes", "reader", "reader_threads", "wait", "job", "dma", "procs", "dma_window", nullptr};
    return keys;
}
static inline const char *&sh_route_override() { static thread_local const char *p = nullptr; return p; }
static inline const char *sh_route_string() { const char *o = sh_route_override(); return o ? o : std::getenv("SEERHIP_ROUTE"); }
static inline const char *sh_route(const char *key)
{
    const char *e = sh_route_string();
    if (!e) return nullptr;
    static thread_local std::string val;
    const size_t kl = std::strlen(key);
    for (const char *p = e; *p;) {
        const char *end = std::strchr(p, ','); if (!end) end = p + std::strlen(p);
        const char *eq = (const char *)std::memchr(p, '=', (size_t)(end - p));
        if (eq && (size_t)(eq - p) == kl && std::memcmp(p, key, kl) == 0) { val.assign(eq + 1, end); return val.c_str(); }
        p = *end ? end + 1 : end;
    }
    return nullptr;
}
static inline std::string sh_route_unknown()
{
    const char *e = sh_route_string();
    if (!e) return std::string();
    for (const char *p = e; *p;) {
        const char *end = std::strchr(p, ','); if (!end) end = p + std::strlen(p);
        const char *eq = (const char *)std::memchr(p, '=', (size_t)(end - p));
        bool ok = false;
        if (eq) for (const char *const *k = sh_route_keys(); *k; ++k) if (std::strlen(*k) == (size_t)(eq - p) && std::memcmp(*k, p, (size_t)(eq - p)) == 0) ok = true;
        if (!ok && end > p) return std::string(p, end);
        p = *end ? end + 1 : end;
    }
    return std::string();
}

static inline bool sh_debug(const char *item)
{
    const char *e = std::getenv("SEERHIP_DEBUG");
    if (!e) return false;
    const size_t kl = std::strlen(item);
    for (const char *p = e; *p;) {
        const char *end = std::strchr(p, ','); if (!end) end = p + std::strlen(p);
        if ((size_t)(end - p) == kl && std::memcmp(p, item, kl) == 0) return true;
        p = *end ? end + 1 : end;
    }
    return false;
}
```

Baseline: 34.40 million.

## Handle ragged sample tail with a packed multi-limb MFMA kernel

When N leaves only a few rows (up to 8) beyond a multiple of 128, the wide quadform kernel now stops at the last full segment. A new kernel handles the leftover rows for all limbs at once, packing each limb's few rows into a shared 32-row MFMA tile. This avoids running a partial 32-row segment per limb that is mostly padding. The cost is a second kernel launch, a small extra device image built once at setup, and a read-modify-write of q with per-limb scaling.

After: 34.88 million, median of 6. 1.01x the previous value.

```diff
diff --git a/pyseer_amd/csrc/api.hip b/pyseer_amd/csrc/api.hip
--- a/pyseer_amd/csrc/api.hip
+++ b/pyseer_amd/csrc/api.hip
@@ -28,7 +28,8 @@
 hipError_t shk_lmm_linear(hipStream_t, int, const uint64_t *, int64_t, int, int, const double *, const double *,
                           const double *, const double *, const uint64_t *, const uint64_t *, int, const double *, LmmLinOut);
 hipError_t shk_lmm_build_tab(hipStream_t, const double *, const double *, const double *, const double *, int, int, int, int, double *);
-hipError_t shk_lmm_quadform(hipStream_t, int, const int8_t *, const uint64_t *, int64_t, int, int, int, double *, const int *, int, int64_t *);
+hipError_t shk_lmm_quadform(hipStream_t, int, const int8_t *, const uint64_t *, int64_t, int, int, int, double *, const int *, int, int64_t *, const int8_t *);
+hipError_t shk_lmm_ragged_image(hipStream_t, const int8_t *, int, int, int, int8_t *);
 hipError_t shk_lmm_refine(hipStream_t, int64_t, int64_t, int, int, int, int, const int8_t *, const uint64_t *, uint64_t *, double *, LmmLinOut,
                           const double *, LmmFinParams, double *, uint32_t *, LmmRefine);
 hipError_t shk_af_compact(hipStream_t, int, int64_t, LmmLinOut, LmmFinParams, int *, int *, const uint64_t *, int64_t, uint64_t *,
@@ -110,6 +111,8 @@
     double *d_vv = nullptr, *d_mdiag = nullptr, *d_yc = nullptr, *d_Qb = nullptr, *d_tab = nullptr;
     uint64_t *d_y1 = nullptr, *d_y0 = nullptr;
     int8_t *d_G = nullptr;
+    int8_t *d_ragA = nullptr; size_t rag_bytes = 0;
+    int ragged = 1;
     double quant_scale = 0.0;
     size_t g_bytes = 0, tab_doubles = 0;
     int64_t macs_issued = 0;
@@ -493,6 +496,7 @@
     sh_ctx *c = new sh_ctx();
     c->device = device; c->N = n_samples;
     if (const char *qv = sh_route("qf")) c->qf_variant = std::atoi(qv);
+    if (const char *rv = sh_route("ragged")) c->ragged = std::atoi(rv);
     if (const char *lv = sh_route("lanes")) c->n_lanes = std::max(1, std::min(8, std::atoi(lv)));
     if (const char *ac = sh_route("afcompact")) c->af_compact = std::atoi(ac);
     c->NT = (n_samples + 255) / 256; c->Np = c->NT * 256;
@@ -515,7 +519,7 @@
     hipFree(c->af_rep); hipFree(c->af_slot); hipFree(c->af_m); hipFree(c->af_cnt); hipFree(c->af_bits); hipFree(c->af_out); hipFree(c->af_flags);
     if (c->keep_ev) hipEventDestroy(c->keep_ev);
     hipFree(c->d_vv); hipFree(c->d_mdiag); hipFree(c->d_yc); hipFree(c->d_Qb); hipFree(c->d_y1); hipFree(c->d_y0); hipFree(c->d_tab);
-    hipFree(c->d_G); hipFree(c->d_bits); hipFree(c->d_out); hipFree(c->d_flags); hipFree(c->d_rcount); hipFree(c->d_bmax);
+    hipFree(c->d_G); hipFree(c->d_ragA); hipFree(c->d_bits); hipFree(c->d_out); hipFree(c->d_flags); hipFree(c->d_rcount); hipFree(c->d_bmax);
     for (int b = 0; b < 2; ++b) { hipFree(c->hb_bits[b]); hipFree(c->hb_out[b]); hipFree(c->hb_flags[b]); if (c->ev_h2d[b]) hipEventDestroy(c->ev_h2d[b]); if (c->ev_done[b]) hipEventDestroy(c->ev_done[b]); }
     if (c->copy_stream) hipStreamDestroy(c->copy_stream);
     for (int b = 0; b < 2; ++b) if (c->hp_bits[b]) hipHostFree(c->hp_bits[b]);
@@ -684,8 +688,8 @@
     std::vector<double> Qbp;
     if (DP) { Qbp.assign((size_t)N * DP, 0.0); for (int i = 0; i < N; ++i) for (int e = 0; e < r; ++e) Qbp[(size_t)i * DP + e] = Qb[(size_t)i * D + e]; }
 
-    hipFree(c->d_vv); hipFree(c->d_mdiag); hipFree(c->d_yc); hipFree(c->d_Qb); hipFree(c->d_y1); hipFree(c->d_y0); hipFree(c->d_G); hipFree(c->d_tab);
-    c->d_vv = c->d_mdiag = c->d_yc = c->d_Qb = c->d_tab = nullptr; c->d_y1 = c->d_y0 = nullptr; c->d_G = nullptr;
+    hipFree(c->d_vv); hipFree(c->d_mdiag); hipFree(c->d_yc); hipFree(c->d_Qb); hipFree(c->d_y1); hipFree(c->d_y0); hipFree(c->d_G); hipFree(c->d_tab); hipFree(c->d_ragA);
+    c->d_vv = c->d_mdiag = c->d_yc = c->d_Qb = c->d_tab = nullptr; c->d_y1 = c->d_y0 = nullptr; c->d_G = nullptr; c->d_ragA = nullptr; c->rag_bytes = 0;
     const int NT = c->NT, L = n_limbs;
     const int NR = 2 * NT;
     int E = std::min(2, 7 - L);
@@ -710,6 +714,11 @@
     HIPCHK(hipMemsetAsync(d_M, 0, sizeof(double) * (size_t)Np * Np, st));
     HIPCHK(dmalloc(&d_Ef, (size_t)Np * Np)); HIPCHK(dmalloc(&d_px, Np)); HIPCHK(dmalloc(&d_py, Np)); HIPCHK(dmalloc(&d_nrm, NPOW));
     HIPCHK(shk_lmm_build_G(st, d_W, d_sgn, N, Np, kp, NR, Lt, E, d_M, c->d_mdiag, d_amax, c->d_G, d_Ef, d_px, d_py, d_nrm, NPOW));
+    if (LmmRagged rg; c->ragged && lmm_ragged_shape(N, L, &rg)) {
+        c->rag_bytes = lmm_ragged_bytes(rg);
+        HIPCHK(hipMalloc((void **)&c->d_ragA, c->rag_bytes));
+        HIPCHK(shk_lmm_ragged_image(st, c->d_G + (size_t)E * NR * (NR + 1) * 8192, N, NR, L, c->d_ragA));
+    }
     const int nsq = Np <= 16384 ? 5 : Np <= 32768 ? 4 : 3;
     double *d_X = nullptr, *d_work = nullptr; int *d_exps = nullptr;
     HIPCHK(dmalloc(&d_X, (size_t)Np * Np)); HIPCHK(dmalloc(&d_work, 2)); HIPCHK(dmalloc(&d_exps, 8));
@@ -770,8 +779,8 @@
     HIPCHK(hipSetDevice(dst->device));
     sh_ctx *c = dst;
     const int N = c->N;
-    hipFree(c->d_vv); hipFree(c->d_mdiag); hipFree(c->d_yc); hipFree(c->d_Qb); hipFree(c->d_y1); hipFree(c->d_y0); hipFree(c->d_G); hipFree(c->d_tab);
-    c->d_vv = c->d_mdiag = c->d_yc = c->d_Qb = c->d_tab = nullptr; c->d_y1 = c->d_y0 = nullptr; c->d_G = nullptr; c->lmm_ready = false;
+    hipFree(c->d_vv); hipFree(c->d_mdiag); hipFree(c->d_yc); hipFree(c->d_Qb); hipFree(c->d_y1); hipFree(c->d_y0); hipFree(c->d_G); hipFree(c->d_tab); hipFree(c->d_ragA);
+    c->d_vv = c->d_mdiag = c->d_yc = c->d_Qb = c->d_tab = nullptr; c->d_y1 = c->d_y0 = nullptr; c->d_G = nullptr; c->d_ragA = nullptr; c->rag_bytes = 0; c->lmm_ready = false;
     HIPCHK(dmalloc(&c->d_vv, N)); HIPCHK(dmalloc(&c->d_mdiag, N)); HIPCHK(dmalloc(&c->d_yc, N));
     HIPCHK(dmalloc(&c->d_y1, c->NB64p)); HIPCHK(dmalloc(&c->d_y0, c->NB64p));
     if (src->DP) HIPCHK(dmalloc(&c->d_Qb, (size_t)N * src->DP));
@@ -782,6 +791,7 @@
     HIPCHK(cp(c->d_y1, src->d_y1, sizeof(uint64_t) * c->NB64p)); HIPCHK(cp(c->d_y0, src->d_y0, sizeof(uint64_t) * c->NB64p));
     if (src->DP) HIPCHK(cp(c->d_Qb, src->d_Qb, sizeof(double) * (size_t)N * src->DP));
     HIPCHK(cp(c->d_G, src->d_G, src->g_bytes)); HIPCHK(cp(c->d_tab, src->d_tab, sizeof(double) * src->tab_doubles));
+    if (src->d_ragA) { HIPCHK(hipMalloc((void **)&c->d_ragA, src->rag_bytes)); HIPCHK(cp(c->d_ragA, src->d_ragA, src->rag_bytes)); c->rag_bytes = src->rag_bytes; }
     HIPCHK(hipStreamSynchronize(dst->stream));
     c->k = src->k; c->D = src->D; c->L = src->L; c->DP = src->DP; c->E = src->E; c->complement = src->complement;
     c->quant_scale = src->quant_scale; c->err_norm_ulp = src->err_norm_ulp; c->err_norm_est_ulp = src->err_norm_est_ulp; c->err_norm_squarings = src->err_norm_squarings; c->trace_M = src->trace_M; c->lmm_tol = src->lmm_tol;
@@ -919,10 +929,10 @@
     if (compact && nk > 0) {
         const int64_t Vpad2 = (nk + 511) / 512 * 512;
         HIPCHK(shk_af_compact(st, 1, V, lo, KP, c->d_keep, nullptr, c->d_T, Vpad, c->d_T2, Vpad2, c->NB64p, (int)nk, nullptr, nullptr));
-        HIPCHK(shk_lmm_quadform(st, c->qf_variant, Gmain, c->d_T2, Vpad2, 2 * c->NT, c->L, lsplit, c->d_q2, nullptr, c->N - (2 * c->NT - 1) * 128, &c->macs_issued));
+        HIPCHK(shk_lmm_quadform(st, c->qf_variant, Gmain, c->d_T2, Vpad2, 2 * c->NT, c->L, lsplit, c->d_q2, nullptr, c->N - (2 * c->NT - 1) * 128, &c->macs_issued, c->d_ragA));
         HIPCHK(shk_af_compact(st, 2, V, lo, KP, c->d_keep, nullptr, nullptr, Vpad, nullptr, Vpad2, lsplit, (int)nk, c->d_q2, c->d_q));
     } else if (!compact) {
-        HIPCHK(shk_lmm_quadform(st, c->qf_variant, Gmain, c->d_T, Vpad, 2 * c->NT, c->L, lsplit, c->d_q, nullptr, c->N - (2 * c->NT - 1) * 128, &c->macs_issued));
+        HIPCHK(shk_lmm_quadform(st, c->qf_variant, Gmain, c->d_T, Vpad, 2 * c->NT, c->L, lsplit, c->d_q, nullptr, c->N - (2 * c->NT - 1) * 128, &c->macs_issued, c->d_ragA));
     }
     if (c->timing) { HIPCHK(hipEventRecord(e1, st)); c->tev.emplace_back(e0, e1); }
     LmmFinParams P = c->fin; P.min_af = c->min_af; P.max_af = c->max_af; P.af_on = c->af_on;
diff --git a/pyseer_amd/csrc/lmm_kernels.hip b/pyseer_amd/csrc/lmm_kernels.hip
--- a/pyseer_amd/csrc/lmm_kernels.hip
+++ b/pyseer_amd/csrc/lmm_kernels.hip
@@ -496,6 +496,103 @@
 
 #include "lmm_quadform_wide.inc"
 
+#define RG_LMAX 7
+
+__global__ __launch_bounds__(128) void k_lmm_ragged_image(const int8_t *__restrict__ G, int NR, int L, int nf, int rp, int nsb, int8_t *__restrict__ A)
+{
+    const int mt = blockIdx.y, sb = blockIdx.x;
+    const int kh = threadIdx.x >> 6, lane = threadIdx.x & 63, l31 = lane & 31, lh = lane >> 5;
+    const int R = mt * 32 + l31, l = R / rp, s = R - l * rp;
+    const int64_t TL = (int64_t)NR * (NR + 1);
+    uint4 o = make_uint4(0, 0, 0, 0);
+    if (l < L) o = *reinterpret_cast<const uint4 *>(G + ((int64_t)l * TL + (int64_t)nf * (nf + 1) + sb) * QF_TILE_BYTES + qf_off(s, lh + 2 * kh));
+    *reinterpret_cast<uint4 *>(A + (((int64_t)mt * nsb + sb) * 2 + kh) * 1024 + lane * 16) = o;
+}
+
+template <int MT>
+__global__ __launch_bounds__(256) void k_lmm_ragged_i8(const int8_t *__restrict__ A, const uint64_t *__restrict__ T, int64_t Vpad, int nsb, int nf,
+                                                       int rp, int mtot, int L, double *__restrict__ q)
+{
+    const int lane = threadIdx.x & 63, wave = threadIdx.x >> 6, l31 = lane & 31, lh = lane >> 5;
+    const int64_t v0 = (int64_t)blockIdx.x * QF_BN + wave * 128 + l31;
+    const uint32_t *th = reinterpret_cast<const uint32_t *>(T) + 2 * v0 + lh;
+    uint64_t wm[4];
+#pragma unroll
+    for (int jt = 0; jt < 4; ++jt) wm[jt] = T[(int64_t)(2 * nf) * Vpad + v0 + 32 * jt];
+    int ls[4][RG_LMAX];
+#pragma unroll
+    for (int jt = 0; jt < 4; ++jt)
+#pragma unroll
+        for (int l = 0; l < RG_LMAX; ++l) ls[jt][l] = 0;
+#pragma unroll 1
+    for (int mt0 = 0; mt0 < mtot; mt0 += MT) {
+        const v4i *ap = reinterpret_cast<const v4i *>(A) + (int64_t)mt0 * nsb * 128 + lane;
+        v16i acc[MT][4];
+#pragma unroll
+        for (int mt = 0; mt < MT; ++mt)
+#pragma unroll
+            for (int jt = 0; jt < 4; ++jt)
+#pragma unroll
+                for (int r = 0; r < 16; ++r) acc[mt][jt][r] = 0;
+        constexpr int D = MT == 1 ? 4 : 2;
+        uint32_t h[D][4];
+        v4i a[D][MT][2];
+        auto load = [&](int sb, uint32_t (&hh)[4], v4i (&aa)[MT][2]) {
+#pragma unroll
+            for (int jt = 0; jt < 4; ++jt) hh[jt] = th[2 * ((int64_t)sb * Vpad + 32 * jt)];
+#pragma unroll
+            for (int mt = 0; mt < MT; ++mt) { aa[mt][0] = ap[((int64_t)mt * nsb + sb) * 128]; aa[mt][1] = ap[((int64_t)mt * nsb + sb) * 128 + 64]; }
+        };
+#pragma unroll
+        for (int d = 0; d < D - 1; ++d) load(min(d, nsb - 1), h[d], a[d]);
+#pragma unroll 1
+        for (int sb0 = 0; sb0 < nsb; sb0 += D) {
+#pragma unroll
+            for (int u = 0; u < D; ++u) {
+                load(min(sb0 + u + D - 1, nsb - 1), h[(u + D - 1) % D], a[(u + D - 1) % D]);
+                __builtin_amdgcn_sched_barrier(0);
+                if (sb0 + u < nsb) {
+#pragma unroll
+                    for (int kh = 0; kh < 2; ++kh)
+#pragma unroll
+                        for (int jt = 0; jt < 4; ++jt) {
+                            const uint32_t x = h[u][jt] >> (4 * kh);
+                            const v4i b = (v4i){(int)(x & 0x01010101u), (int)((x >> 1) & 0x01010101u), (int)((x >> 2) & 0x01010101u), (int)((x >> 3) & 0x01010101u)};
+#pragma unroll
+                            for (int mt = 0; mt < MT; ++mt) acc[mt][jt] = __builtin_amdgcn_mfma_i32_32x32x32_i8(a[u][mt][kh], b, acc[mt][jt], 0, 0, 0);
+                        }
+                }
+                __builtin_amdgcn_sched_barrier(0);
+            }
+        }
+#pragma unroll
+        for (int mt = 0; mt < MT; ++mt)
+#pragma unroll
+            for (int g = 0; g < 4; ++g) {
+                const int R = (mt0 + mt) * 32 + 8 * g + 4 * lh, l = R / rp, s = R - l * rp;
+#pragma unroll
+                for (int jt = 0; jt < 4; ++jt) {
+                    const uint32_t m4 = (uint32_t)(wm[jt] >> s);
+                    int sg = 0;
+#pragma unroll
+                    for (int k = 0; k < 4; ++k) sg += ((m4 >> k) & 1u) ? acc[mt][jt][4 * g + k] : 0;
+#pragma unroll
+                    for (int x = 0; x < RG_LMAX; ++x) ls[jt][x] += (x == l) ? sg : 0;
+                }
+            }
+    }
+    double scale = 1.0;
+#pragma unroll
+    for (int l = 0; l < RG_LMAX; ++l) {
+#pragma unroll
+        for (int jt = 0; jt < 4; ++jt) {
+            const int t = ls[jt][l] + __shfl_xor(ls[jt][l], 32, 64);
+            if (lh == 0 && l < L) { double *qo = q + (int64_t)l * Vpad + v0 + 32 * jt; *qo = fma((double)t, scale, *qo); }
+        }
+        scale *= 256.0;
+    }
+}
+
 
 struct LinV { int m, t11, t01, mst; double xky, dg, rss, s1, q1; };
 __device__ __forceinline__ LinV lin_load(const LmmLinOut &li, const LmmFinParams &P, int64_t v)
@@ -897,7 +994,7 @@
 }
 
 hipError_t shk_lmm_quadform(hipStream_t st, int variant, const int8_t *G, const uint64_t *T, int64_t Vpad, int NR, int L, int lsplit, double *q,
-                            const int *nlimit, int rows_last, int64_t *macs_per_variant)
+                            const int *nlimit, int rows_last, int64_t *macs_per_variant, const int8_t *ragA)
 {
     const bool wide_ok = lsplit == L && NR >= 4 && (uint64_t)NR * 2 * (uint64_t)Vpad * 8 < (1ull << 32) && (uint64_t)(L + 1) * NR * (NR + 1) * QF_TILE_BYTES < (1ull << 32);
     const bool wide_var = variant == 4 || variant == 6 || variant == 7 || variant == 8 || variant == 9 || variant == 50 || variant == 441 || variant == 162 || variant == 35;
@@ -906,8 +1003,13 @@
     if (variant == 64 && wide_ok && refine_wide) variant = 464;
     const bool wide = (wide_var && wide_ok) || variant == 464;
     const int nit_last = !wide ? 4 : rows_last <= 0 ? 0 : rows_last <= 32 ? 1 : rows_last <= 64 ? 2 : 4;
+    int nfull = nit_last == 4 ? NR : NR - 1, nit = nit_last == 4 ? 0 : nit_last;
+    LmmRagged rg;
+    const bool ragged = ragA && wide && variant != 464 && !nlimit && lmm_ragged_shape((NR - 1) * 128 + rows_last, L, &rg);
+    if (ragged) { nfull = rg.nf; nit = 0; }
     if (macs_per_variant)
-        *macs_per_variant = (int64_t)L * ((int64_t)(NR - 1) * NR * 128 * 64 + (int64_t)2 * NR * 32 * nit_last * 64);
+        *macs_per_variant = (int64_t)L * ((int64_t)nfull * (nfull + 1) * 128 * 64 + (int64_t)2 * (nfull + 1) * 32 * nit * 64)
+                            + (ragged ? (int64_t)rg.mt * 32 * rg.nsb * 64 : 0);
     const dim3 g((unsigned)(Vpad / QF_BN * lsplit)), b(wide ? 256 : 64 * QF_WAVES);
     const size_t lds = QF_NST * QF_STAGE_BYTES;
     static bool attr_set = false;
@@ -949,19 +1051,32 @@
     case 158: hipLaunchKernelGGL(k_lmm_quadform_i8<128>, g, b, lds, st, G, T, Vpad, NR, L, lsplit, q, nlimit); break;
     case 286: hipLaunchKernelGGL(k_lmm_quadform_i8<256>, g, b, lds, st, G, T, Vpad, NR, L, lsplit, q, nlimit); break;
     case 414: hipLaunchKernelGGL(k_lmm_quadform_i8<384>, g, b, lds, st, G, T, Vpad, NR, L, lsplit, q, nlimit); break;
-    case 464: hipLaunchKernelGGL((k_lmm_quadform_i8w<0, 3>), g, b, lds, st, G, T, Vpad, NR, L, lsplit, q, nlimit, nit_last); break;
-    case 4: hipLaunchKernelGGL(k_lmm_quadform_i8w<0>, g, b, lds, st, G, T, Vpad, NR, L, lsplit, q, nlimit, nit_last); break;
-    case 6: hipLaunchKernelGGL((k_lmm_quadform_i8w<0, 0, 1>), g, b, lds, st, G, T, Vpad, NR, L, lsplit, q, nlimit, nit_last); break;
-    case 7: hipLaunchKernelGGL((k_lmm_quadform_i8w<0, 0, 2>), g, b, lds, st, G, T, Vpad, NR, L, lsplit, q, nlimit, nit_last); break;
-    case 8: hipLaunchKernelGGL((k_lmm_quadform_i8w<16, 0, 1>), g, b, lds, st, G, T, Vpad, NR, L, lsplit, q, nlimit, nit_last); break;
-    case 9: hipLaunchKernelGGL((k_lmm_quadform_i8w<1, 0, 1>), g, b, lds, st, G, T, Vpad, NR, L, lsplit, q, nlimit, nit_last); break;
-    case 50: hipLaunchKernelGGL(k_lmm_quadform_i8w<16>, g, b, lds, st, G, T, Vpad, NR, L, lsplit, q, nlimit, nit_last); break;
-    case 35: hipLaunchKernelGGL(k_lmm_quadform_i8w<1>, g, b, lds, st, G, T, Vpad, NR, L, lsplit, q, nlimit, nit_last); break;
-    case 162: hipLaunchKernelGGL(k_lmm_quadform_i8w<128>, g, b, lds, st, G, T, Vpad, NR, L, lsplit, q, nlimit, nit_last); break;
-    case 441: hipLaunchKernelGGL(k_lmm_quadform_i8w<407>, g, b, lds, st, G, T, Vpad, NR, L, lsplit, q, nlimit, nit_last); break;
+    case 464: hipLaunchKernelGGL((k_lmm_quadform_i8w<0, 3>), g, b, lds, st, G, T, Vpad, NR, L, lsplit, q, nlimit, nit, nfull); break;
+    case 4: hipLaunchKernelGGL(k_lmm_quadform_i8w<0>, g, b, lds, st, G, T, Vpad, NR, L, lsplit, q, nlimit, nit, nfull); break;
+    case 6: hipLaunchKernelGGL((k_lmm_quadform_i8w<0, 0, 1>), g, b, lds, st, G, T, Vpad, NR, L, lsplit, q, nlimit, nit, nfull); break;
+    case 7: hipLaunchKernelGGL((k_lmm_quadform_i8w<0, 0, 2>), g, b, lds, st, G, T, Vpad, NR, L, lsplit, q, nlimit, nit, nfull); break;
+    case 8: hipLaunchKernelGGL((k_lmm_quadform_i8w<16, 0, 1>), g, b, lds, st, G, T, Vpad, NR, L, lsplit, q, nlimit, nit, nfull); break;
+    case 9: hipLaunchKernelGGL((k_lmm_quadform_i8w<1, 0, 1>), g, b, lds, st, G, T, Vpad, NR, L, lsplit, q, nlimit, nit, nfull); break;
+    case 50: hipLaunchKernelGGL(k_lmm_quadform_i8w<16>, g, b, lds, st, G, T, Vpad, NR, L, lsplit, q, nlimit, nit, nfull); break;
+    case 35: hipLaunchKernelGGL(k_lmm_quadform_i8w<1>, g, b, lds, st, G, T, Vpad, NR, L, lsplit, q, nlimit, nit, nfull); break;
+    case 162: hipLaunchKernelGGL(k_lmm_quadform_i8w<128>, g, b, lds, st, G, T, Vpad, NR, L, lsplit, q, nlimit, nit, nfull); break;
+    case 441: hipLaunchKernelGGL(k_lmm_quadform_i8w<407>, g, b, lds, st, G, T, Vpad, NR, L, lsplit, q, nlimit, nit, nfull); break;
     case 437: hipLaunchKernelGGL(k_lmm_quadform_i8<407>, g, b, lds, st, G, T, Vpad, NR, L, lsplit, q, nlimit); break;
     default: hipLaunchKernelGGL(k_lmm_quadform_i8<0>, g, b, lds, st, G, T, Vpad, NR, L, lsplit, q, nlimit); break;
     }
+    if (ragged) {
+        const dim3 gr((unsigned)(Vpad / QF_BN)), br(256);
+        if (rg.mt == 1) hipLaunchKernelGGL(k_lmm_ragged_i8<1>, gr, br, 0, st, ragA, T, Vpad, rg.nsb, rg.nf, rg.rp, rg.mt, L, q);
+        else hipLaunchKernelGGL(k_lmm_ragged_i8<2>, gr, br, 0, st, ragA, T, Vpad, rg.nsb, rg.nf, rg.rp, rg.mt, L, q);
+    }
+    return hipGetLastError();
+}
+
+hipError_t shk_lmm_ragged_image(hipStream_t st, const int8_t *G, int N, int NR, int L, int8_t *ragA)
+{
+    LmmRagged rg;
+    if (!lmm_ragged_shape(N, L, &rg)) return hipErrorInvalidValue;
+    hipLaunchKernelGGL(k_lmm_ragged_image, dim3((unsigned)rg.nsb, (unsigned)rg.mt), dim3(128), 0, st, G, NR, L, rg.nf, rg.rp, rg.nsb, ragA);
     return hipGetLastError();
 }
 
@@ -976,7 +1091,7 @@
                           uint64_t *T3, double *q3, LmmLinOut li, const double *q, LmmFinParams P, double *out, uint32_t *flags, LmmRefine R)
 {
     hipLaunchKernelGGL(k_gather_T_list, dim3(64, (unsigned)NB64p), dim3(256), 0, st, T, Vpad, T3, R);
-    hipError_t e = shk_lmm_quadform(st, 64, Glow, T3, Vpad, NR, E, E, q3, R.count, 128, nullptr);
+    hipError_t e = shk_lmm_quadform(st, 64, Glow, T3, Vpad, NR, E, E, q3, R.count, 128, nullptr, nullptr);
     if (e != hipSuccess) return e;
     hipLaunchKernelGGL(k_lmm_refine_fix, dim3(64), dim3(256), 0, st, V, Vpad, nq, E, li, q, q3, P, out, flags, R);
     return hipGetLastError();
diff --git a/pyseer_amd/csrc/lmm_params.h b/pyseer_amd/csrc/lmm_params.h
--- a/pyseer_amd/csrc/lmm_params.h
+++ b/pyseer_amd/csrc/lmm_params.h
@@ -23,3 +23,15 @@
     int *list, *count;
     unsigned long long *bound_max;
 };
+
+#ifndef LMM_RAGGED_MAX
+#define LMM_RAGGED_MAX 8
+#endif
+struct LmmRagged { int nf, r, rp, mt, nsb; };
+static inline bool lmm_ragged_shape(int N, int L, LmmRagged *g)
+{
+    g->nf = N / 128; g->r = N % 128; g->rp = (g->r + 7) & ~7; g->nsb = 2 * g->nf + 1;
+    g->mt = (L * g->rp + 31) / 32; if (g->mt > 1) g->mt = (g->mt + 1) & ~1;
+    return g->r >= 1 && g->r <= LMM_RAGGED_MAX && g->nf >= 3;
+}
+static inline size_t lmm_ragged_bytes(const LmmRagged &g) { return (size_t)g.mt * g.nsb * 2048; }
diff --git a/pyseer_amd/csrc/lmm_quadform_wide.inc b/pyseer_amd/csrc/lmm_quadform_wide.inc
--- a/pyseer_amd/csrc/lmm_quadform_wide.inc
+++ b/pyseer_amd/csrc/lmm_quadform_wide.inc
@@ -16,7 +16,7 @@
 template <int ABL, int DM = 0, int PROF = 0>
 __global__ __launch_bounds__(256, 1) void k_lmm_quadform_i8w(const int8_t *__restrict__ G, const uint64_t *__restrict__ T,
                                                               int64_t Vpad, int NR, int L, int lsplit, double *__restrict__ qout,
-                                                              const int *__restrict__ nlimit, int nit_last)
+                                                              const int *__restrict__ nlimit, int nit_last, int nfull)
 {
     constexpr int JT = 4, DMA_PER_WAVE = 6;
     extern __shared__ __attribute__((aligned(16))) char smem[];
@@ -216,12 +216,11 @@
         }
         QW_STAMP(pt_epi)
     };
-    const int NRfull = (nit_last == 4) ? NR : NR - 1;
 #pragma unroll 1
-    for (int cI = 0; cI < NRfull; ++cI) segment(std::integral_constant<int, 4>{}, cI, scale0);
-    if (nit_last == 2) segment(std::integral_constant<int, 2>{}, NR - 1, scale0);
-    else if (nit_last == 1) segment(std::integral_constant<int, 1>{}, NR - 1, scale0);
-    const int total = nl * (NR * (NR + 1) / 2);
+    for (int cI = 0; cI < nfull; ++cI) segment(std::integral_constant<int, 4>{}, cI, scale0);
+    if (nit_last == 2) segment(std::integral_constant<int, 2>{}, nfull, scale0);
+    else if (nit_last == 1) segment(std::integral_constant<int, 1>{}, nfull, scale0);
+    const int nseg = nfull + (nit_last == 1 || nit_last == 2 ? 1 : 0), total = nl * (nseg * (nseg + 1) / 2);
     asm volatile("s_waitcnt vmcnt(0) lgkmcnt(0)" ::: "memory");
     if (PROF && blockIdx.x == 0 && tid == 0)
         printf("wide prof (block 0, wave 0): stages %d  wait %llu  sub0 %llu  sub1 %llu  sub2 %llu  sub3 %llu  tail %llu  epilogue %llu  (cycles)\n", total,
diff --git a/pyseer_amd/csrc/route.h b/pyseer_amd/csrc/route.h
--- a/pyseer_amd/csrc/route.h
+++ b/pyseer_amd/csrc/route.h
@@ -7,7 +7,7 @@
 {
     static const char *const keys[] = {"chord", "chord_n32", "chord_enter", "bitdot", "first_bordered", "pk", "warm", "fin_rounds", "ll_first", "newton",
                                        "firth_last", "firth_first32", "afcompact", "complement", "reader_slab", "reader_pad", "reader_chunk", "reader_workers", "reader_depth", "reader_helpers", "reader_target",
-                                       "firth_literal", "firth_strict", "firth_fast", "firth_w", "lmm_limbs", "lmm_tol", "qf", "lanes", "reader", "reader_threads", "wait", "job", "dma", "procs", "dma_window", nullptr};
+                                       "firth_literal", "firth_strict", "firth_fast", "firth_w", "lmm_limbs", "lmm_tol", "qf", "ragged", "lanes", "reader", "reader_threads", "wait", "job", "dma", "procs", "dma_window", nullptr};
     return keys;
 }
 static inline const char *&sh_route_override() { static thread_local const char *p = nullptr; return p; }
```
